# dhansmair/flamingo-mini

Measured on AMD Instinct MI355X. Metric: images/sec (fwd+bwd) flamingo-mini bs=32, higher is better.
Workload: dtype bf16

## Files before the change

flamingo-mini_amd/csrc/ff_api.hip:

```cpp
#include <stdarg.h>
#include <stdio.h>
#include <math.h>
#include <stdlib.h>
#include "ff_common.h"
#include "ff_internal.h"

namespace ff {

static thread_local char g_err[512] = "";
void set_error(const char* fmt, ...) {
    va_list ap;
    va_start(ap, fmt);
    vsnprintf(g_err, sizeof(g_err), fmt, ap);
    va_end(ap);
}
#ifdef FF_DEBUG
int dbg_switch(const char* name, int dflt) {
    const char* e = getenv(name);
    return e ? atoi(e) : dflt;
}
#endif
int check_launch(const char* what) {
    hipError_t e = hipGetLastError();
    if (e != hipSuccess) {
        set_error("%s: launch failed: %s", what, hipGetErrorString(e));
        return FF_ERR_LAUNCH;
    }
    return FF_OK;
}


static LnArgs ln_args(int dtype, int rows, int cols, RowMap x, RowMap y, RowMap dx) {
    LnArgs a;
    a.dtype = dtype; a.rows = rows; a.cols = cols;
    a.x_map = x; a.y_map = y; a.dx_map = dx;
    a.add_rows_per_seg = 0; a.add_div = 0; a.eps = 1e-5f; a.stats_given = 0;
    return a;
}

struct RsDims {
    int dt, Bn, T, v, D, F, q, H, dh, inner, ffi, R, depth, nte, act;
    int Mq, Mkv, Mf;
    size_t es, attn_ws;
    float scale;
    RowMap pD, pI, pF;
    RowMap lat_bcast;
    RowMap kv_media, kv_lat;
    explicit RsDims(const ff_resampler_desc& d) {
        dt = d.dtype; Bn = d.batch; T = d.n_frames; v = d.n_tokens; D = d.dim; F = T * v; q = d.num_latents;
        H = d.heads; dh = d.dim_head; inner = H * dh; ffi = d.ff_mult * D; R = F + q; depth = d.depth;
        nte = d.num_time_embeds; act = d.act; es = dtype_size(dt); scale = 1.0f / sqrtf((float)dh);
        Mq = Bn * q; Mkv = Bn * R; Mf = Bn * F; attn_ws = (size_t)Bn * H * q * 4;
        pD = plain_rows(D); pI = plain_rows(inner); pF = plain_rows(ffi);
        lat_bcast = RowMap{D, 0, q};
        kv_media = RowMap{D, (long long)R * D, F};
        kv_lat = RowMap{D, (long long)R * D, q};
    }
    LnArgs ln_latents() const { return ln_args(dt, Mq, D, pD, pD, pD); }
    LnArgs ln_media(RowMap y) const {
        LnArgs a = ln_args(dt, Mf, D, pD, y, pD);
        a.add_rows_per_seg = F; a.add_div = v;
        return a;
    }
    template <typename P> P* kv_latent_rows(P* kv) const { return (P*)((char*)kv + (size_t)F * D * es); }
};
struct RsLayerSaved {
    void *x_in, *kv_in, *Qs, *K, *V, *O, *x_mid, *xn_f, *Hpre, *Aact;
    float *mean_l, *rstd_l, *lse, *mean_f, *rstd_f;
};
constexpr int kMaxDepth = 64;
struct RsSaved {
    float *mean_m, *rstd_m, *mean_o, *rstd_o;
    void* x_last;
    RsLayerSaved L[kMaxDepth];
};
static void rs_take_layer_saved(const RsDims& s, Arena& a, RsLayerSaved& L) {
    const size_t rows_q = s.Mq, rows_kv = s.Mkv;
    L.mean_l = a.take<float>(rows_q * 4);
    L.rstd_l = a.take<float>(rows_q * 4);
    L.kv_in = a.take(rows_kv * s.D * s.es);
    L.Qs = a.take(rows_q * s.inner * s.es);
    L.K = a.take(rows_kv * s.inner * s.es);
    L.V = a.take(rows_kv * s.inner * s.es);
    L.lse = a.take<float>((size_t)s.Bn * s.H * s.q * 4);
    L.O = a.take(rows_q * s.inner * s.es);
    L.x_mid = a.take(rows_q * s.D * s.es);
    L.mean_f = a.take<float>(rows_q * 4);
    L.rstd_f = a.take<float>(rows_q * 4);
    L.xn_f = a.take(rows_q * s.D * s.es);
    L.Hpre = a.take(rows_q * s.ffi * s.es);
    L.Aact = a.take(rows_q * s.ffi * s.es);
}
static size_t rs_saved_layout(const RsDims& s, void* base, size_t cap, RsSaved& o) {
    Arena a(base, cap);
    const size_t rows_q = s.Mq;
    o.mean_m = a.take<float>((size_t)s.Mf * 4);
    o.rstd_m = a.take<float>((size_t)s.Mf * 4);
    for (int l = 0; l < s.depth; l++) {
        o.L[l].x_in = l == 0 ? nullptr : a.take(rows_q * s.D * s.es);
        rs_take_layer_saved(s, a, o.L[l]);
    }
    o.x_last = a.take(rows_q * s.D * s.es);
    o.mean_o = a.take<float>(rows_q * 4);
    o.rstd_o = a.take<float>(rows_q * 4);
    return align_up(a.used);
}

static size_t rs_ws_bytes(const RsDims& s) {
    size_t w = 0;
    auto g = [&](int M, int N, int K, int nz) { w = std::max(w, gemm_workspace_bytes(s.dt, M, N, K, nz, 0)); };
    g(s.Mq, s.inner, s.D, 1); g(s.Mkv, s.inner, s.D, 2); g(s.Mq, s.D, s.inner, 1); g(s.Mq, s.ffi, s.D, 1); g(s.Mq, s.D, s.ffi, 1);
    for (int nz = 1; nz <= 4; nz++) {
        g(s.D, s.ffi, s.Mq, nz); g(s.ffi, s.D, s.Mq, nz); g(s.D, s.inner, s.Mq, nz); g(s.inner, s.D, s.Mq, nz); g(s.inner, s.D, s.Mkv, nz);
    }
    g(s.Mkv, s.D, s.inner, 1);
    w = std::max(w, layernorm_bwd_workspace(s.Mf, s.D));
    w = std::max(w, layernorm_bwd_workspace(s.Mq, s.D));
    w = std::max(w, rows_reduce_workspace(s.Mq, s.D, s.q, 1));
    w = std::max(w, rows_reduce_workspace(s.Mf, s.D, s.F, s.v));
    return align_up(w) + align_up(s.attn_ws);
}
struct RsChain {
    void *ws, *dxn, *dO, *dkv, *dln;
    size_t ws_bytes, gws;
    float* attn_ws;
};
struct RsLayerGrads {
    void *dx_mid, *dH, *dQs, *dK, *dV;
};
static void rs_take_ws(const RsDims& s, Arena& a, RsChain& c) {
    c.ws_bytes = rs_ws_bytes(s);
    c.ws = a.take(c.ws_bytes);
    c.gws = c.ws_bytes - align_up(s.attn_ws);
    c.attn_ws = c.ws ? (float*)((char*)c.ws + c.gws) : nullptr;
}
static void rs_take_chain(const RsDims& s, Arena& a, RsChain& c) {
    c.dxn = a.take((size_t)s.Mq * s.D * s.es);
    c.dO = a.take((size_t)s.Mq * s.inner * s.es);
    c.dkv = a.take((size_t)s.Mkv * s.D * s.es);
    c.dln = a.take((size_t)s.Mq * s.D * s.es);
}
static void rs_take_layer_grads(const RsDims& s, Arena& a, RsLayerGrads& g) {
    g.dx_mid = a.take((size_t)s.Mq * s.D * s.es);
    g.dH = a.take((size_t)s.Mq * s.ffi * s.es);
    g.dQs = a.take((size_t)s.Mq * s.inner * s.es);
    g.dK = a.take((size_t)s.Mkv * s.inner * s.es);
    g.dV = a.take((size_t)s.Mkv * s.inner * s.es);
}
static void rs_take_ln_partials(const RsDims& s, Arena& a, bool deferrable, float** lnp) {
    for (int i = 0; i < 3; i++) lnp[i] = deferrable ? a.take<float>(layernorm_bwd_partial_bytes(i == 2 ? s.Mf : s.Mq, s.D)) : nullptr;
}

struct RsScratch {
    RsChain c;
    void *dx0, *dxf;
    void* dx_out[kMaxDepth];
    RsLayerGrads L[kMaxDepth];
    float* lnp[3 * kMaxDepth + 1];
};
static size_t rs_scratch_layout(const RsDims& s, void* base, size_t cap, bool bwd, RsScratch& o) {
    Arena a(base, cap);
    rs_take_ws(s, a, o.c);
    if (bwd) {
        o.dx0 = a.take((size_t)s.Mq * s.D * s.es);
        rs_take_chain(s, a, o.c);
        o.dxf = a.take((size_t)s.Mf * s.D * s.es);
        for (int l = 0; l < s.depth; l++) {
            o.dx_out[l] = a.take((size_t)s.Mq * s.D * s.es);
            rs_take_layer_grads(s, a, o.L[l]);
        }
        static const int defer_ln = dbg_switch("FF_DEFER_LN", 1);
        const bool lnd = defer_ln != 0 && layernorm_bwd_deferrable(s.dt, s.D);
        for (int l = 0; l < s.depth; l++) rs_take_ln_partials(s, a, lnd, o.lnp + 3 * l);
        o.lnp[3 * s.depth] = lnd ? a.take<float>(layernorm_bwd_partial_bytes(s.Mq, s.D)) : nullptr;
    }
    return align_up(a.used);
}

static int rs_check(const ff_resampler_desc* d) {
    FF_CHECK(d, FF_ERR_SHAPE, "resampler: null descriptor");
    FF_CHECK(d->dtype == FF_DTYPE_F32 || d->dtype == FF_DTYPE_BF16, FF_ERR_UNSUPPORTED, "resampler: dtype %d", d->dtype);
    FF_CHECK(d->batch > 0 && d->n_frames > 0 && d->n_tokens > 0 && d->dim > 0 && d->depth > 0 && d->depth <= kMaxDepth && d->heads > 0 &&
                 d->dim_head > 0 && d->num_latents > 0 && d->ff_mult > 0,
             FF_ERR_SHAPE, "resampler: bad dimensions");
    FF_CHECK(d->n_frames <= d->num_time_embeds, FF_ERR_SHAPE, "resampler: %d frames > num_time_embeds %d (perceiver_resampler.py:166)",
             d->n_frames, d->num_time_embeds);
    FF_CHECK(d->act >= FF_ACT_GELU && d->act <= FF_ACT_RELU, FF_ERR_SHAPE, "resampler: act %d", d->act);
    return FF_OK;
}

static ff_attn_desc rs_attn_desc(const RsDims& s) {
    ff_attn_desc a = {};
    a.dtype = s.dt; a.batch = s.Bn; a.heads = s.H; a.dim_head = s.dh; a.n_q = s.q; a.n_kv = s.R; a.mode = FF_ATTN_DENSE;
    const ff_strides sq = {(long long)s.q * s.inner, s.inner, s.dh}, sk = {(long long)s.R * s.inner, s.inner, s.dh};
    a.q = sq; a.o = sq; a.dq = sq; a.dout = sq;
    a.k = sk; a.v = sk; a.dk = sk; a.dv = sk;
    return a;
}

static int rs_media_stats(const RsDims& s, const void* x_f, const void* tpe, float* mean_m, float* rstd_m, hipStream_t st) {
    return layernorm_fwd(s.ln_media(s.pD), x_f, tpe, nullptr, nullptr, nullptr, mean_m, rstd_m, st);
}

static int rs_layer_forward(const RsDims& s, const void* const* p, const void* x_f, const void* tpe, float* mean_m, float* rstd_m, const void* x_in,
                            RowMap x_map, void* x_out, const RsLayerSaved& L, void* ws, size_t ws_bytes, hipStream_t st) {
    const RowMap pD = s.pD, pI = s.pI, pF = s.pF;
    void* kv_lat_base = s.kv_latent_rows(L.kv_in);
    {
        LnArgs a = s.ln_media(s.kv_media);
        a.stats_given = 1;
        FF_TRY(layernorm_fwd(a, x_f, tpe, p[0], p[1], L.kv_in, mean_m, rstd_m, st));
    }
    FF_TRY(layernorm_fwd(ln_args(s.dt, s.Mq, s.D, x_map, s.kv_lat, pD), x_in, nullptr, p[2], p[3], kv_lat_base, L.mean_l, L.rstd_l, st));
    FF_TRY(Gemm(s.dt, s.Mq, s.inner, s.D).a(0, s.kv_lat).b(0, pD).c(pI).scale(s.scale).problem(kv_lat_base, p[4], L.Qs).run(ws, ws_bytes, st));
    FF_TRY(Gemm(s.dt, s.Mkv, s.inner, s.D).a(0, pD).b(0, pD).c(pI).problem(L.kv_in, p[5], L.K).problem(L.kv_in, p[6], L.V).run(ws, ws_bytes, st));
    FF_TRY(attention_fwd(rs_attn_desc(s), L.Qs, L.K, L.V, nullptr, L.O, L.lse, st));
    FF_TRY(Gemm(s.dt, s.Mq, s.D, s.inner).a(0, pI).b(0, pI).c(pD).res_map(x_map).problem(L.O, p[7], L.x_mid, nullptr, nullptr, x_in).run(ws, ws_bytes, st));
    FF_TRY(layernorm_fwd(s.ln_latents(), L.x_mid, nullptr, p[8], p[9], L.xn_f, L.mean_f, L.rstd_f, st));
    FF_TRY(Gemm(s.dt, s.Mq, s.ffi, s.D).a(0, pD).b(0, pD).c(pF).act(s.act).problem(L.xn_f, p[10], L.Aact, L.Hpre).run(ws, ws_bytes, st));
    return Gemm(s.dt, s.Mq, s.D, s.ffi).a(0, pF).b(0, pF).c(pD).problem(L.Aact, p[11], x_out, nullptr, nullptr, L.x_mid).run(ws, ws_bytes, st);
}

static int rs_final_norm(const RsDims& s, const void* x_last, const void* gamma, const void* beta, void* out, float* mean, float* rstd, hipStream_t st) {
    return layernorm_fwd(s.ln_latents(), x_last, nullptr, gamma, beta, out, mean, rstd, st);
}

static int rs_ln_bwd(const RsChain& W, float* partial, LnPending* pending, const LnArgs& a, const void* dy, const void* x, const void* add,
                     const void* gamma, const float* mean, const float* rstd, void* dx, const void* dx_res, void* dg, void* db, hipStream_t st) {
    if (partial)
        return layernorm_bwd(a, dy, x, add, gamma, mean, rstd, dx, dx_res, dg, db, partial, layernorm_bwd_partial_bytes(a.rows, a.cols), st, nullptr, pending);
    return layernorm_bwd(a, dy, x, add, gamma, mean, rstd, dx, dx_res, dg, db, W.ws, W.gws, st);
}

static int rs_layer_backward(const RsDims& s, const void* const* p, void* const* g, const void* x_f, const void* tpe, const float* mean_m,
                             const float* rstd_m, const void* x_in, RowMap x_map, const RsLayerSaved& L, const void* dx_out, void* dx_in,
                             void* dx_f, const void* dx_f_res, const RsChain& W, const RsLayerGrads& T, float* const* lnp, LnPending* ln_sets,
                             hipStream_t st) {
    const RowMap pD = s.pD, pI = s.pI, pF = s.pF;
    FF_TRY(Gemm(s.dt, s.Mq, s.ffi, s.D).a(0, pD).b(1, pF).c(pF).act_bwd(s.act).problem(dx_out, p[11], T.dH, nullptr, L.Hpre).run(W.ws, W.gws, st));
    FF_TRY(Gemm(s.dt, s.Mq, s.D, s.ffi).a(0, pF).b(1, pD).c(pD).problem(T.dH, p[10], W.dxn).run(W.ws, W.gws, st));
    FF_TRY(rs_ln_bwd(W, lnp[0], &ln_sets[0], s.ln_latents(), W.dxn, L.x_mid, nullptr, p[8], L.mean_f, L.rstd_f, T.dx_mid, dx_out, g[8], g[9], st));
    FF_TRY(Gemm(s.dt, s.Mq, s.inner, s.D).a(0, pD).b(1, pI).c(pI).problem(T.dx_mid, p[7], W.dO).run(W.ws, W.gws, st));
    FF_TRY(attention_bwd(rs_attn_desc(s), L.Qs, L.K, L.V, nullptr, L.O, W.dO, L.lse, T.dQs, T.dK, T.dV, W.attn_ws, s.attn_ws, st));
    FF_TRY(Gemm(s.dt, s.Mkv, s.D, s.inner).a(0, pI).b(1, pD).c(pD).problem(T.dK, p[5], W.dkv).run(W.ws, W.gws, st));
    FF_TRY(Gemm(s.dt, s.Mkv, s.D, s.inner).a(0, pI).b(1, pD).c(pD).problem(T.dV, p[6], W.dkv, nullptr, nullptr, W.dkv).run(W.ws, W.gws, st));
    FF_TRY(Gemm(s.dt, s.Mq, s.D, s.inner).a(0, pI).b(1, pD).c(pD).res_map(s.kv_lat).scale(s.scale)
               .problem(T.dQs, p[4], W.dln, nullptr, nullptr, s.kv_latent_rows(W.dkv)).run(W.ws, W.gws, st));
    FF_TRY(rs_ln_bwd(W, lnp[1], &ln_sets[1], ln_args(s.dt, s.Mq, s.D, x_map, pD, pD), W.dln, x_in, nullptr, p[2], L.mean_l, L.rstd_l, dx_in, T.dx_mid, g[2],
                     g[3], st));
    return rs_ln_bwd(W, lnp[2], &ln_sets[2], s.ln_media(s.kv_media), W.dkv, x_f, tpe, p[0], mean_m, rstd_m, dx_f, dx_f_res, g[0], g[1], st);
}

static int rs_input_grads(const RsDims& s, const void* dx0, const void* dxf, void* d_latents, void* d_tpe, void* ws, size_t ws_bytes, hipStream_t st) {
    FF_TRY(rows_reduce(s.dt, s.Mq, s.D, s.pD, s.q, 1, dx0, d_latents, ws, ws_bytes, st));
    if (s.nte > s.T) FF_TRY(zero_bytes((char*)d_tpe + (size_t)s.T * s.D * s.es, (size_t)(s.nte - s.T) * s.D * s.es, st));
    return rows_reduce(s.dt, s.Mf, s.D, s.pD, s.F, s.v, dxf, d_tpe, ws, ws_bytes, st);
}

static int resampler_fwd(const ff_resampler_desc* d, const void* x_f, const void* const* P, void* out, void* saved, size_t saved_bytes,
                         void* scratch, size_t scratch_bytes, hipStream_t st) {
    FF_TRY(rs_check(d));
    FF_CHECK(x_f && P && out && saved && scratch, FF_ERR_SHAPE, "resampler_fwd: null argument");
    const RsDims s(*d);
    RsSaved S;
    RsScratch W;
    FF_CHECK(rs_saved_layout(s, saved, saved_bytes, S) <= saved_bytes, FF_ERR_WORKSPACE, "resampler_fwd: saved buffer too small");
    FF_CHECK(rs_scratch_layout(s, scratch, scratch_bytes, false, W) <= scratch_bytes, FF_ERR_WORKSPACE, "resampler_fwd: scratch too small");
    const void *latents = P[0], *tpe = P[1];
    FF_TRY(rs_media_stats(s, x_f, tpe, S.mean_m, S.rstd_m, st));
    for (int l = 0; l < s.depth; l++) {
        const void* const* p = P + FF_RESAMPLER_GLOBAL_PARAMS + FF_RESAMPLER_LAYER_PARAMS * l;
        void* x_next = l + 1 < s.depth ? S.L[l + 1].x_in : S.x_last;
        FF_TRY(rs_layer_forward(s, p, x_f, tpe, S.mean_m, S.rstd_m, l == 0 ? latents : S.L[l].x_in, l == 0 ? s.lat_bcast : s.pD, x_next, S.L[l], W.c.ws,
                                W.c.ws_bytes, st));
    }
    return rs_final_norm(s, S.x_last, P[2], P[3], out, S.mean_o, S.rstd_o, st);
}

static int resampler_bwd(const ff_resampler_desc* d, const void* x_f, const void* const* P, const void* dout, const void* saved,
                         size_t saved_bytes, void* const* G, void* dx_f, void* scratch, size_t scratch_bytes, hipStream_t st) {
    FF_TRY(rs_check(d));
    FF_CHECK(x_f && P && dout && saved && G && scratch, FF_ERR_SHAPE, "resampler_bwd: null argument");
    const RsDims s(*d);
    RsSaved S;
    RsScratch W;
    FF_CHECK(rs_saved_layout(s, (void*)saved, saved_bytes, S) <= saved_bytes, FF_ERR_WORKSPACE, "resampler_bwd: saved buffer too small");
    FF_CHECK(rs_scratch_layout(s, scratch, scratch_bytes, true, W) <= scratch_bytes, FF_ERR_WORKSPACE, "resampler_bwd: scratch too small");
    const RowMap pD = s.pD, pI = s.pI, pF = s.pF;
    const void *latents = P[0], *tpe = P[1];
    void* dxf = dx_f ? dx_f : W.dxf;
    void* const ws = W.c.ws;
    const size_t gws = W.c.gws;

    LnPending ln_sets[3 * kMaxDepth + 1];
    FF_TRY(rs_ln_bwd(W.c, W.lnp[3 * s.depth], &ln_sets[3 * s.depth], s.ln_latents(), dout, S.x_last, nullptr, P[2], S.mean_o, S.rstd_o,
                     W.dx_out[s.depth - 1], nullptr, G[2], G[3], st));
    for (int l = s.depth - 1; l >= 0; l--) {
        const void* const* p = P + FF_RESAMPLER_GLOBAL_PARAMS + FF_RESAMPLER_LAYER_PARAMS * l;
        void* const* g = G + FF_RESAMPLER_GLOBAL_PARAMS + FF_RESAMPLER_LAYER_PARAMS * l;
        void* dx_below = l == 0 ? W.dx0 : W.dx_out[l - 1];
        FF_TRY(rs_layer_backward(s, p, g, x_f, tpe, S.mean_m, S.rstd_m, l == 0 ? latents : S.L[l].x_in, l == 0 ? s.lat_bcast : pD, S.L[l], W.dx_out[l],
                                 dx_below, dxf, l == s.depth - 1 ? nullptr : dxf, W.c, W.L[l], W.lnp + 3 * l, ln_sets + 3 * l, st));
    }
    FF_TRY(layernorm_bwd_finish(s.dt, ln_sets, 3 * s.depth + 1, st));
    constexpr int kRsGroup = 4;
    for (int l0 = 0; l0 < s.depth; l0 += kRsGroup) {
        const int l1 = std::min(s.depth, l0 + kRsGroup);
        Gemm g3(s.dt, s.D, s.ffi, s.Mq), g1(s.dt, s.ffi, s.D, s.Mq), go(s.dt, s.D, s.inner, s.Mq), gq(s.dt, s.inner, s.D, s.Mq);
        g3.a(1, pD).b(1, pF).c(pF);
        g1.a(1, pF).b(1, pD).c(pD);
        go.a(1, pD).b(1, pI).c(pI);
        gq.a(1, pI).b(1, s.kv_lat).c(pD).scale(s.scale);
        for (int l = l0; l < l1; l++) {
            void* const* g = G + FF_RESAMPLER_GLOBAL_PARAMS + FF_RESAMPLER_LAYER_PARAMS * l;
            const RsLayerSaved& L = S.L[l];
            const RsLayerGrads& T = W.L[l];
            g3.problem(W.dx_out[l], L.Aact, g[11]);
            g1.problem(T.dH, L.xn_f, g[10]);
            go.problem(T.dx_mid, L.O, g[7]);
            gq.problem(T.dQs, s.kv_latent_rows(L.kv_in), g[4]);
        }
        FF_TRY(g3.run(ws, gws, st));
        FF_TRY(g1.run(ws, gws, st));
        FF_TRY(go.run(ws, gws, st));
        FF_TRY(gq.run(ws, gws, st));
    }
    {
        Gemm gkv(s.dt, s.inner, s.D, s.Mkv);
        gkv.a(1, pI).b(1, pD).c(pD);
        for (int l = 0; l < s.depth; l++) {
            void* const* g = G + FF_RESAMPLER_GLOBAL_PARAMS + FF_RESAMPLER_LAYER_PARAMS * l;
            gkv.problem(W.L[l].dK, S.L[l].kv_in, g[5]);
            gkv.problem(W.L[l].dV, S.L[l].kv_in, g[6]);
            if (gkv.P.nz == kRsGroup || l == s.depth - 1) {
                FF_TRY(gkv.run(ws, gws, st));
                gkv.P.nz = 0;
            }
        }
    }
    return rs_input_grads(s, W.dx0, dxf, G[0], G[1], ws, gws, st);
}

struct RsProSaved { float *mean_m, *rstd_m; };
static size_t rs_pro_layout(const RsDims& s, void* base, size_t cap, RsProSaved& o) {
    Arena a(base, cap);
    o.mean_m = a.take<float>((size_t)s.Mf * 4);
    o.rstd_m = a.take<float>((size_t)s.Mf * 4);
    return align_up(a.used);
}
static size_t rs_layer_saved_layout(const RsDims& s, void* base, size_t cap, RsLayerSaved& L) {
    Arena a(base, cap);
    L.x_in = nullptr;
    rs_take_layer_saved(s, a, L);
    return align_up(a.used);
}
struct RsLayerScratch {
    RsChain c;
    RsLayerGrads g;
    float* lnp[3];
};
static size_t rs_layer_scratch_layout(const RsDims& s, void* base, size_t cap, RsLayerScratch& o) {
    Arena a(base, cap);
    rs_take_ws(s, a, o.c);
    rs_take_chain(s, a, o.c);
    rs_take_layer_grads(s, a, o.g);
    rs_take_ln_partials(s, a, layernorm_bwd_deferrable(s.dt, s.D), o.lnp);
    return align_up(a.used);
}

static int rs_prologue_fwd(const ff_resampler_desc* d, const void* x_f, const void* tpe, void* pro, size_t pro_bytes, hipStream_t st) {
    FF_TRY(rs_check(d));
    FF_CHECK(x_f && tpe && pro, FF_ERR_SHAPE, "resampler_prologue_fwd: null argument");
    const RsDims s(*d);
    RsProSaved S;
    FF_CHECK(rs_pro_layout(s, pro, pro_bytes, S) <= pro_bytes, FF_ERR_WORKSPACE, "resampler_prologue_fwd: saved buffer too small");
    return rs_media_stats(s, x_f, tpe, S.mean_m, S.rstd_m, st);
}

static int rs_layer_fwd(const ff_resampler_desc* d, const void* x_f, const void* tpe, const void* pro, size_t pro_bytes, const void* x_in,
                        int x_is_latents, const void* const* p, void* x_out, void* saved, size_t saved_bytes, void* scratch, size_t scratch_bytes,
                        hipStream_t st) {
    FF_TRY(rs_check(d));
    FF_CHECK(x_f && tpe && pro && x_in && p && x_out && saved && scratch, FF_ERR_SHAPE, "resampler_layer_fwd: null argument");
    const RsDims s(*d);
    RsProSaved Pr;
    RsLayerSaved L;
    RsLayerScratch W;
    FF_CHECK(rs_pro_layout(s, (void*)pro, pro_bytes, Pr) <= pro_bytes, FF_ERR_WORKSPACE, "resampler_layer_fwd: prologue buffer too small");
    FF_CHECK(rs_layer_saved_layout(s, saved, saved_bytes, L) <= saved_bytes, FF_ERR_WORKSPACE, "resampler_layer_fwd: saved buffer too small");
    FF_CHECK(rs_layer_scratch_layout(s, scratch, scratch_bytes, W) <= scratch_bytes, FF_ERR_WORKSPACE, "resampler_layer_fwd: scratch too small");
    return rs_layer_forward(s, p, x_f, tpe, Pr.mean_m, Pr.rstd_m, x_in, x_is_latents ? s.lat_bcast : s.pD, x_out, L, W.c.ws, W.c.ws_bytes, st);
}

static int rs_layer_bwd(const ff_resampler_desc* d, const void* x_f, const void* tpe, const void* pro, size_t pro_bytes, const void* x_in,
                        int x_is_latents, const void* const* p, const void* dx_out, const void* saved, size_t saved_bytes, void* const* g,
                        void* dx_in, void* dx_f, int dx_f_accumulate, void* scratch, size_t scratch_bytes, hipStream_t st) {
    FF_TRY(rs_check(d));
    FF_CHECK(x_f && tpe && pro && x_in && p && dx_out && saved && g && dx_in && dx_f && scratch, FF_ERR_SHAPE, "resampler_layer_bwd: null argument");
    const RsDims s(*d);
    RsProSaved Pr;
    RsLayerSaved L;
    RsLayerScratch W;
    FF_CHECK(rs_pro_layout(s, (void*)pro, pro_bytes, Pr) <= pro_bytes, FF_ERR_WORKSPACE, "resampler_layer_bwd: prologue buffer too small");
    FF_CHECK(rs_layer_saved_layout(s, (void*)saved, saved_bytes, L) <= saved_bytes, FF_ERR_WORKSPACE, "resampler_layer_bwd: saved buffer too small");
    FF_CHECK(rs_layer_scratch_layout(s, scratch, scratch_bytes, W) <= scratch_bytes, FF_ERR_WORKSPACE, "resampler_layer_bwd: scratch too small");
    const RowMap pD = s.pD, pI = s.pI, pF = s.pF;
    void* const ws = W.c.ws;
    const size_t gws = W.c.gws;
    LnPending ln_sets[3];
    FF_TRY(rs_layer_backward(s, p, g, x_f, tpe, Pr.mean_m, Pr.rstd_m, x_in, x_is_latents ? s.lat_bcast : pD, L, dx_out, dx_in, dx_f,
                             dx_f_accumulate ? dx_f : nullptr, W.c, W.g, W.lnp, ln_sets, st));
    FF_TRY(layernorm_bwd_finish(s.dt, ln_sets, 3, st));
    FF_TRY(Gemm(s.dt, s.D, s.ffi, s.Mq).a(1, pD).b(1, pF).c(pF).problem(dx_out, L.Aact, g[11]).run(ws, gws, st));
    FF_TRY(Gemm(s.dt, s.ffi, s.D, s.Mq).a(1, pF).b(1, pD).c(pD).problem(W.g.dH, L.xn_f, g[10]).run(ws, gws, st));
    FF_TRY(Gemm(s.dt, s.D, s.inner, s.Mq).a(1, pD).b(1, pI).c(pI).problem(W.g.dx_mid, L.O, g[7]).run(ws, gws, st));
    FF_TRY(Gemm(s.dt, s.inner, s.D, s.Mq).a(1, pI).b(1, s.kv_lat).c(pD).scale(s.scale).problem(W.g.dQs, s.kv_latent_rows(L.kv_in), g[4]).run(ws, gws, st));
    return Gemm(s.dt, s.inner, s.D, s.Mkv).a(1, pI).b(1, pD).c(pD).problem(W.g.dK, L.kv_in, g[5]).problem(W.g.dV, L.kv_in, g[6]).run(ws, gws, st);
}

static int rs_prologue_bwd(const ff_resampler_desc* d, const void* dx0, const void* dx_f, void* d_latents, void* d_tpe, void* scratch,
                           size_t scratch_bytes, hipStream_t st) {
    FF_TRY(rs_check(d));
    FF_CHECK(dx0 && dx_f && d_latents && d_tpe && scratch, FF_ERR_SHAPE, "resampler_prologue_bwd: null argument");
    const RsDims s(*d);
    RsLayerScratch W;
    FF_CHECK(rs_layer_scratch_layout(s, scratch, scratch_bytes, W) <= scratch_bytes, FF_ERR_WORKSPACE, "resampler_prologue_bwd: scratch too small");
    return rs_input_grads(s, dx0, dx_f, d_latents, d_tpe, W.c.ws, W.c.ws_bytes, st);
}

static int rs_epilogue_fwd(const ff_resampler_desc* d, const void* x_last, const void* gamma, const void* beta, void* out, void* epi, size_t epi_bytes,
                           hipStream_t st) {
    FF_TRY(rs_check(d));
    FF_CHECK(x_last && gamma && beta && out && epi, FF_ERR_SHAPE, "resampler_epilogue_fwd: null argument");
    const RsDims s(*d);
    const size_t rows_q = s.Mq;
    FF_CHECK(epi_bytes >= 2 * align_up(rows_q * 4), FF_ERR_WORKSPACE, "resampler_epilogue_fwd: saved buffer too small");
    return rs_final_norm(s, x_last, gamma, beta, out, (float*)epi, (float*)((char*)epi + align_up(rows_q * 4)), st);
}
static int rs_epilogue_bwd(const ff_resampler_desc* d, const void* dout, const void* x_last, const void* gamma, const void* epi, size_t epi_bytes,
                           void* dx_last, void* dgamma, void* dbeta, void* scratch, size_t scratch_bytes, hipStream_t st) {
    FF_TRY(rs_check(d));
    FF_CHECK(dout && x_last && gamma && epi && dx_last && dgamma && dbeta && scratch, FF_ERR_SHAPE, "resampler_epilogue_bwd: null argument");
    const RsDims s(*d);
    const size_t rows_q = s.Mq;
    FF_CHECK(epi_bytes >= 2 * align_up(rows_q * 4), FF_ERR_WORKSPACE, "resampler_epilogue_bwd: saved buffer too small");
    RsLayerScratch W;
    FF_CHECK(rs_layer_scratch_layout(s, scratch, scratch_bytes, W) <= scratch_bytes, FF_ERR_WORKSPACE, "resampler_epilogue_bwd: scratch too small");
    const float* mean = (const float*)epi;
    const float* rstd = (const float*)((const char*)epi + align_up(rows_q * 4));
    return layernorm_bwd(s.ln_latents(), dout, x_last, nullptr, gamma, mean, rstd, dx_last, nullptr, dgamma, dbeta, W.c.ws, W.c.ws_bytes, st);
}

struct XaDims {
    int dt, b, L, d, dv, Nm, nv, Nk, H, dh, inner, ffi, act;
    size_t es;
    float scale;
    bool ext_kv;
    explicit XaDims(const ff_xattn_desc& x) {
        ext_kv = x.cached_k.sr != 0;
        dt = x.dtype; b = x.batch; L = x.n_tokens; d = x.dim; dv = x.dim_visual; Nm = x.n_media; nv = x.n_visual; Nk = Nm * nv;
        H = x.heads; dh = x.dim_head; inner = H * dh; ffi = x.ff_mult * d; act = x.act; es = dtype_size(dt);
        scale = 1.0f / sqrtf((float)dh);
    }
};
struct XaSaved {
    float *mean_a, *rstd_a, *lse, *mean_f, *rstd_f;
    void *yn, *Qs, *KV, *O, *attn_out, *y1, *xn_f, *Hpre, *Aact, *ffw_out;
    size_t kv_offset;
};
static size_t xa_saved_layout(const XaDims& s, void* base, size_t cap, XaSaved& o) {
    Arena a(base, cap);
    const size_t M = (size_t)s.b * s.L;
    o.KV = s.ext_kv ? nullptr : a.take((size_t)s.b * s.Nk * 2 * s.inner * s.es);
    o.kv_offset = 0;
    o.mean_a = a.take<float>(M * 4);
    o.rstd_a = a.take<float>(M * 4);
    o.yn = a.take(M * s.d * s.es);
    o.Qs = a.take(M * s.inner * s.es);
    o.lse = a.take<float>((size_t)s.b * s.H * s.L * 4);
    o.O = a.take(M * s.inner * s.es);
    o.attn_out = a.take(M * s.d * s.es);
    o.y1 = a.take(M * s.d * s.es);
    o.mean_f = a.take<float>(M * 4);
    o.rstd_f = a.take<float>(M * 4);
    o.xn_f = a.take(M * s.d * s.es);
    o.Hpre = a.take(M * s.ffi * s.es);
    o.Aact = a.take(M * s.ffi * s.es);
    o.ffw_out = a.take(M * s.d * s.es);
    return align_up(a.used);
}
struct XaScratch {
    void *dy1, *dH, *dxn, *dO, *dQs, *dKV, *dyn, *ws;
    size_t ws_bytes;
    float* lnx;
};
struct XaStash {
    void *dy1, *dH, *dQs;
    float *lnp_f = nullptr, *lnp_a = nullptr;
};
static bool xa_ln_deferrable(const XaDims& s) {
    static const int on = dbg_switch("FF_DEFER_LN", 1);
    return on != 0 && layernorm_bwd_deferrable(s.dt, s.d);
}
static size_t xa_stash_layout(const XaDims& s, void* base, size_t cap, XaStash& o) {
    Arena a(base, cap);
    const size_t M = (size_t)s.b * s.L;
    o.dy1 = a.take(M * s.d * s.es);
    o.dH = a.take(M * s.ffi * s.es);
    o.dQs = a.take(M * s.inner * s.es);
    if (xa_ln_deferrable(s)) {
        o.lnp_f = a.take<float>(layernorm_bwd_partial_bytes((int)M, s.d));
        o.lnp_a = a.take<float>(layernorm_bwd_partial_bytes((int)M, s.d));
    }
    return align_up(a.used);
}
static size_t xa_ws_bytes(const XaDims& s) {
    const int M = s.b * s.L, Mk = s.b * s.Nk;
    size_t w = 0;
    auto g = [&](int m, int n, int k) { w = std::max(w, gemm_workspace_bytes(s.dt, m, n, k, 1, 0)); };
    g(M, s.inner, s.d); g(Mk, 2 * s.inner, s.dv); g(M, s.d, s.inner); g(M, s.ffi, s.d); g(M, s.d, s.ffi);
    g(s.d, s.ffi, M); g(s.ffi, s.d, M); g(s.d, s.inner, M); g(s.inner, s.d, M); g(2 * s.inner, s.dv, Mk); g(Mk, s.dv, 2 * s.inner);
    w = std::max(w, layernorm_bwd_workspace(M, s.d));
    w = std::max(w, gate_grad_workspace(M, s.d));
    if (decode_ffw_supported(s.dt, M, s.d, s.ffi)) w = std::max(w, decode_ffw_workspace_bytes(s.d, s.ffi));
    return align_up(w) + align_up((size_t)s.b * s.H * s.L * 4);
}
static size_t xa_scratch_layout(const XaDims& s, void* base, size_t cap, bool bwd, XaScratch& o) {
    Arena a(base, cap);
    const size_t M = (size_t)s.b * s.L;
    o.ws_bytes = xa_ws_bytes(s);
    o.ws = a.take(o.ws_bytes);
    o.lnx = a.take<float>(xa_ln3_part_bytes(s.b, s.H));
    if (bwd) {
        o.dy1 = a.take(M * s.d * s.es);
        o.dH = a.take(M * s.ffi * s.es);
        o.dxn = a.take(M * s.d * s.es);
        o.dO = a.take(M * s.inner * s.es);
        o.dQs = a.take(M * s.inner * s.es);
        o.dKV = s.ext_kv ? nullptr : a.take((size_t)s.b * s.Nk * 2 * s.inner * s.es);
        o.dyn = a.take(M * s.d * s.es);
    }
    return align_up(a.used);
}
static int xa_check(const ff_xattn_desc* d) {
    FF_CHECK(d, FF_ERR_SHAPE, "xattn: null descriptor");
    FF_CHECK(d->dtype == FF_DTYPE_F32 || d->dtype == FF_DTYPE_BF16, FF_ERR_UNSUPPORTED, "xattn: dtype %d", d->dtype);
    FF_CHECK(d->batch > 0 && d->n_tokens > 0 && d->dim > 0 && d->dim_visual > 0 && d->n_media > 0 && d->n_visual > 0 && d->heads > 0 &&
                 d->dim_head > 0 && d->ff_mult > 0,
             FF_ERR_SHAPE, "xattn: bad dimensions");
    FF_CHECK(d->act >= FF_ACT_GELU && d->act <= FF_ACT_RELU, FF_ERR_SHAPE, "xattn: act %d", d->act);
    return FF_OK;
}
static ff_attn_desc xa_attn_desc(const ff_xattn_desc& x, const XaDims& s, bool cached) {
    ff_attn_desc a = {};
    a.dtype = s.dt; a.batch = s.b; a.heads = s.H; a.dim_head = s.dh; a.n_q = s.L; a.n_kv = s.Nk;
    a.mode = FF_ATTN_MEDIA; a.n_visual = s.nv; a.tt_stride = x.tt_stride; a.tt_offset = x.tt_offset;
    const ff_strides sq = {(long long)s.L * s.inner, s.inner, s.dh};
    const ff_strides sk = {(long long)s.Nk * 2 * s.inner, 2LL * s.inner, s.dh};
    a.q = sq; a.o = sq; a.dq = sq; a.dout = sq;
    a.k = cached ? x.cached_k : sk;
    a.v = cached ? x.cached_v : sk;
    a.dk = sk; a.dv = sk;
    return a;
}

static bool xa_fused_enabled() {
    static const int v = dbg_switch("FF_XATTN_FUSED", 1);
    return v != 0;
}
static bool xa_ln3_enabled() {
    static const int v = dbg_switch("FF_XATTN_LN3", 1);
    return v != 0;
}
static XaFusedArgs xa_fused_args(const ff_xattn_desc& x, const XaDims& s, bool ext_kv) {
    XaFusedArgs a = {};
    a.batch = s.b; a.heads = s.H; a.n_q = s.L; a.n_kv = s.Nk; a.n_visual = s.nv; a.tt_stride = x.tt_stride; a.tt_offset = x.tt_offset;
    a.dim = s.d; a.inner = s.inner; a.scale = s.scale; a.eps = 1e-5f;
    static const int xcd_split = dbg_switch("FF_XATTN_XCD_SPLIT", 0);
    a.xcd_split = xcd_split;
    const ff_strides sk = {(long long)s.Nk * 2 * s.inner, 2LL * s.inner, s.dh};
    a.k = ext_kv ? x.cached_k : sk;
    a.v = ext_kv ? x.cached_v : sk;
    a.dk = sk; a.dv = sk;
    return a;
}

static bool xa_ln3_in_bwd(const ff_xattn_desc& x, const XaDims& s) {
    if (!xa_ln3_enabled() || !xa_fused_enabled() || !xa_fused_supported(s.dt, s.dh, s.d, s.inner) || x.sync == nullptr) return false;
    const XaFusedArgs fa = xa_fused_args(x, s, s.ext_kv);
    const int M = s.b * s.L;
    return xa_out_fusable(fa, s.dt, s.dh) && s.b <= layernorm_bwd_partial_blocks(M) && (size_t)s.b * (2 * (size_t)s.d + 2) * sizeof(float) <= layernorm_bwd_workspace(M, s.d);
}
static int xattn_fwd(const ff_xattn_desc* d, const void* y, const void* vf, const int* tt, const void* const* P, const void* ck,
                     const void* cv, void* y_out, void* saved, size_t saved_bytes, void* scratch, size_t scratch_bytes, hipStream_t st) {
    FF_TRY(xa_check(d));
    const bool cached = ck != nullptr;
    FF_CHECK(y && tt && P && y_out && saved && scratch && (cached ? cv != nullptr : vf != nullptr), FF_ERR_SHAPE, "xattn_fwd: null argument");
    const XaDims s(*d);
    FF_CHECK(s.ext_kv == cached, FF_ERR_SHAPE, "xattn_fwd: external K / V need their strides in the descriptor (cached_k / cached_v) and vice versa");
    XaSaved S;
    XaScratch W;
    FF_CHECK(xa_saved_layout(s, saved, saved_bytes, S) <= saved_bytes, FF_ERR_WORKSPACE, "xattn_fwd: saved buffer too small");
    FF_CHECK(xa_scratch_layout(s, scratch, scratch_bytes, false, W) <= scratch_bytes, FF_ERR_WORKSPACE, "xattn_fwd: scratch too small");
    const int M = s.b * s.L, Mk = s.b * s.Nk;
    const RowMap pd = plain_rows(s.d), pI = plain_rows(s.inner), pF = plain_rows(s.ffi), pV = plain_rows(s.dv), pKV = plain_rows(2 * s.inner);
    const void *Kp, *Vp;
    if (!cached) {
        FF_TRY(Gemm(s.dt, Mk, 2 * s.inner, s.dv).a(0, pV).b(0, pV).c(pKV).problem(vf, P[5], S.KV).run(W.ws, W.ws_bytes, st));
        Kp = S.KV;
        Vp = (const char*)S.KV + (size_t)s.inner * s.es;
    } else {
        Kp = ck; Vp = cv;
    }
    bool out_fused = false, ln_fused = false;
    if (xa_fused_enabled() && xa_fused_supported(s.dt, s.dh, s.d, s.inner)) {
        const XaFusedArgs fa = xa_fused_args(*d, s, cached);
        XaOutArgs oa = {(const bf16*)P[6], (const bf16*)P[0], (bf16*)S.y1, (bf16*)S.attn_out, (unsigned*)d->sync};
        out_fused = d->sync != nullptr && xa_out_fusable(fa, s.dt, s.dh) && !decode_ffw_supported(s.dt, M, s.d, s.ffi);
        if (out_fused && xa_ln3_enabled()) {
            oa.ln_g = (const bf16*)P[7]; oa.ln_b = (const bf16*)P[8]; oa.ln_out = (bf16*)S.xn_f; oa.ln_mean = S.mean_f; oa.ln_rstd = S.rstd_f;
            oa.ln_part = W.lnx;
            ln_fused = true;
        }
        FF_TRY(xa_qattn_fwd(fa, s.dt, s.dh, y, P[2], P[3], P[4], Kp, Vp, tt, S.yn, S.Qs, S.O, S.mean_a, S.rstd_a, S.lse, st, out_fused ? &oa : nullptr));
    } else {
        FF_TRY(layernorm_fwd(ln_args(s.dt, M, s.d, pd, pd, pd), y, nullptr, P[2], P[3], S.yn, S.mean_a, S.rstd_a, st));
        FF_TRY(Gemm(s.dt, M, s.inner, s.d).a(0, pd).b(0, pd).c(pI).scale(s.scale).problem(S.yn, P[4], S.Qs).run(W.ws, W.ws_bytes, st));
        FF_TRY(attention_fwd(xa_attn_desc(*d, s, cached), S.Qs, Kp, Vp, tt, S.O, S.lse, st));
    }
    if (!out_fused) FF_TRY(Gemm(s.dt, M, s.d, s.inner).a(0, pI).b(0, pI).c(pd).problem(S.O, P[6], S.y1, S.attn_out, nullptr, y, P[0]).run(W.ws, W.ws_bytes, st));
    if (decode_ffw_supported(s.dt, M, s.d, s.ffi))
        return decode_ffw(M, s.d, s.ffi, s.act, 1e-5f, S.y1, P[7], P[8], P[9], P[10], P[1], S.xn_f, S.mean_f, S.rstd_f, S.Hpre, S.Aact, S.ffw_out, y_out,
                          W.ws, W.ws_bytes, st);
    if (!ln_fused) FF_TRY(layernorm_fwd(ln_args(s.dt, M, s.d, pd, pd, pd), S.y1, nullptr, P[7], P[8], S.xn_f, S.mean_f, S.rstd_f, st));
    FF_TRY(Gemm(s.dt, M, s.ffi, s.d).a(0, pd).b(0, pd).c(pF).act(s.act).problem(S.xn_f, P[9], S.Aact, S.Hpre).run(W.ws, W.ws_bytes, st));
    return Gemm(s.dt, M, s.d, s.ffi).a(0, pF).b(0, pF).c(pd).problem(S.Aact, P[10], y_out, S.ffw_out, nullptr, S.y1, P[1]).run(W.ws, W.ws_bytes, st);
}

static int xattn_bwd(const ff_xattn_desc* d, const void* y, const void* vf, const int* tt, const void* const* P, const void* dy2,
                     const void* saved, size_t saved_bytes, void* const* G, void* dy, void* dvf, void* scratch, size_t scratch_bytes,
                     hipStream_t st, const void* ext_k = nullptr, const void* ext_v = nullptr, void* dkv_out = nullptr,
                     void* stash = nullptr, size_t stash_bytes = 0) {
    FF_TRY(xa_check(d));
    const bool hoisted = ext_k != nullptr;
    FF_CHECK(y && tt && P && dy2 && saved && G && dy && scratch && (hoisted ? (ext_v && dkv_out) : vf != nullptr), FF_ERR_SHAPE,
             "xattn_bwd: null argument");
    const XaDims s(*d);
    FF_CHECK(s.ext_kv == hoisted, FF_ERR_SHAPE, "xattn_bwd: external K / V need their strides in the descriptor (cached_k / cached_v) and vice versa");
    XaSaved S;
    XaScratch W;
    FF_CHECK(xa_saved_layout(s, (void*)saved, saved_bytes, S) <= saved_bytes, FF_ERR_WORKSPACE, "xattn_bwd: saved buffer too small");
    FF_CHECK(xa_scratch_layout(s, scratch, scratch_bytes, true, W) <= scratch_bytes, FF_ERR_WORKSPACE, "xattn_bwd: scratch too small");
    XaStash T{W.dy1, W.dH, W.dQs};
    const bool defer = stash != nullptr;
    if (defer) FF_CHECK(xa_stash_layout(s, stash, stash_bytes, T) <= stash_bytes, FF_ERR_WORKSPACE, "xattn_bwd: stash too small");
    const bool defer_ln = defer && xa_ln_deferrable(s);
    if (defer_ln)
        FF_CHECK(((uintptr_t)y | (uintptr_t)dy | (uintptr_t)dy2 | (uintptr_t)P[2] | (uintptr_t)P[7]) % 16 == 0, FF_ERR_SHAPE,
                 "xattn_bwd (deferred weight gradients): y, d y_out, d y and the LayerNorm weights must be 16-byte aligned");
    LnPending pend_f, pend_a;
    const int M = s.b * s.L, Mk = s.b * s.Nk;
    const RowMap pd = plain_rows(s.d), pI = plain_rows(s.inner), pF = plain_rows(s.ffi), pV = plain_rows(s.dv), pKV = plain_rows(2 * s.inner);
    const size_t attn_ws_bytes = align_up((size_t)s.b * s.H * s.L * 4);
    const size_t gws = W.ws_bytes - attn_ws_bytes;
    float* attn_ws = (float*)((char*)W.ws + gws);

    if (!defer) FF_TRY(Gemm(s.dt, s.d, s.ffi, M).a(1, pd).b(1, pF).c(pF).problem(dy2, S.Aact, G[10], nullptr, nullptr, nullptr, P[1]).run(W.ws, gws, st));
    FF_TRY(Gemm(s.dt, M, s.ffi, s.d).a(0, pd).b(1, pF).c(pF).act_bwd(s.act).problem(dy2, P[10], T.dH, nullptr, S.Hpre, nullptr, P[1]).run(W.ws, gws, st));
    if (!defer) FF_TRY(Gemm(s.dt, s.ffi, s.d, M).a(1, pF).b(1, pd).c(pd).problem(T.dH, S.xn_f, G[9]).run(W.ws, gws, st));
// ... 339 lines not shown
```

flamingo-mini_amd/csrc/ff_gemm.hip:

```cpp
#include <atomic>
#include <type_traits>
#include "ff_common.h"
#include <stdlib.h>
#include "ff_internal.h"
#include "ff_gemm_tiles.h"

namespace ff {

template <typename T>
FF_DEV void epilogue4(const GemmParams& P, const GemmProblem& pr, int m, int n, float (&v)[4]) {
    typedef __attribute__((ext_vector_type(4))) T vec4;
    const long long off = P.c_map.off(m) + n;
    const bool full = (n + 3 < P.N);
#pragma unroll
    for (int r = 0; r < 4; r++) v[r] *= P.scale;
    auto load4 = [&](const void* base, long long at, float (&o)[4]) {
        const T* p = (const T*)base + at;
        if (full) {
            vec4 t = *(const vec4*)p;
#pragma unroll
            for (int r = 0; r < 4; r++) o[r] = to_f32(t[r]);
        } else {
#pragma unroll
            for (int r = 0; r < 4; r++) o[r] = (n + r < P.N) ? to_f32(p[r]) : 0.f;
// ... 55 lines not shown
                for (int e = 0; e < VN; e++) { o[e] = a[e]; o[e + 4] = b[e]; }
            }
        } else {
#pragma unroll
            for (int e = 0; e < 8; e++) o[e] = e < nv ? to_f32(p[e]) : 0.f;
        }
    };
    auto store8 = [&](void* base, long long at, const float (&o)[8]) {
        T* p = (T*)base + at;
        if (vec) {
            if constexpr (VN == 8) Vec<T>::store(p, o);
            else {
                float a[VN], b[VN];
#pragma unroll
                for (int e = 0; e < VN; e++) { a[e] = o[e]; b[e] = o[e + 4]; }
                Vec<T>::store(p, a); Vec<T>::store(p + VN, b);
            }
        } else {
#pragma unroll
            for (int e = 0; e < 8; e++)
                if (e < nv) p[e] = from_f32<T>(o[e]);
        }
    };
#pragma unroll
    for (int e = 0; e < 8; e++) v[e] *= P.scale;
    const long long off = P.c_map.off(m) + n;
    if (has_aux) store8(pr.aux_out, off, v);
    if (has_gate) {
#pragma unroll
        for (int e = 0; e < 8; e++) v[e] *= gate;
    }
    if (has_act) {
#pragma unroll
        for (int e = 0; e < 8; e++) v[e] = act_fwd_t<T>(v[e], P.act);
    }
    if (has_act_bwd) {
        float h[8];
        load8(pr.aux_in, off, h);
#pragma unroll
        for (int e = 0; e < 8; e++) v[e] *= act_grad_t<T>(h[e], P.act_bwd);
    }
    if (has_res) {
        float q[8];
        load8(pr.residual, P.r_map.off(m) + n, q);
#pragma unroll
        for (int e = 0; e < 8; e++) v[e] += q[e];
    }
    store8(pr.C, off, v);
}

template <int BN> struct CtSwz { static constexpr int kMask = (BN / 4) % 16 == 0 ? 15 : 7; };
template <int BM, int BN, int NTHR = 256>
FF_DEV void tile_epilogue_bf16(const GemmParams& P, const GemmProblem& pr, const float* ct, int m_base, int n_base) {
    constexpr int TPR = BN / 8, RPP = NTHR / TPR;
    const int t = threadIdx.x, tr = t / TPR, col = (t % TPR) * 8, n = n_base + col;
    if (t >= TPR * RPP || n >= P.N) return;
    const int nv = min(8, P.N - n);
    const bool vec = P.c_vec8 && nv == 8;
    const float gate = pr.gate ? tanhf(to_f32(*(const bf16*)pr.gate)) : 1.f;
    auto rows = [&](auto feat) {
        constexpr int F = decltype(feat)::value;
        constexpr int UNROLL = (F < 0 || (F & (kEpiAct | kEpiActBwd))) ? 2 : 4;
        const int nrows = min(BM, P.M - m_base);
#pragma unroll UNROLL
        for (int r = tr; r < nrows; r += RPP) {
            const int m = m_base + r;
            const int ch = col >> 2, sw = r & CtSwz<BN>::kMask;
            const f32x4 lo = *(const f32x4*)(ct + r * BN + ((ch ^ sw) << 2)), hi = *(const f32x4*)(ct + r * BN + (((ch + 1) ^ sw) << 2));
            float v[8] = {lo[0], lo[1], lo[2], lo[3], hi[0], hi[1], hi[2], hi[3]};
            epilogue8<bf16, F>(P, pr, m, n, nv, vec, gate, v);
        }
    };
    const int feat = (pr.aux_out ? kEpiAux : 0) | (pr.gate ? kEpiGate : 0) | (P.act >= 0 ? kEpiAct : 0) | (P.act_bwd >= 0 ? kEpiActBwd : 0) |
                     (pr.residual ? kEpiRes : 0);
    if (feat == 0) rows(std::integral_constant<int, 0>());
    else if (feat == kEpiRes) rows(std::integral_constant<int, kEpiRes>());
    else if (feat == (kEpiRes | kEpiGate)) rows(std::integral_constant<int, kEpiRes | kEpiGate>());
    else if (feat == (kEpiAux | kEpiAct)) rows(std::integral_constant<int, kEpiAux | kEpiAct>());
    else if (feat == kEpiActBwd) rows(std::integral_constant<int, kEpiActBwd>());
    else if (feat == (kEpiActBwd | kEpiGate)) rows(std::integral_constant<int, kEpiActBwd | kEpiGate>());
    else rows(std::integral_constant<int, -1>());
}

#define FF_PIN(x) asm volatile("" : "+s"(x))
#define FF_GEMM_ARGS(Q, pr, P)                                                                                                        \
    GemmParams Q;                                                                                                                     \
    Q.M = P.M; Q.N = P.N; Q.K = P.K; Q.split_k = P.split_k; Q.k_per_split = P.k_per_split; Q.nz = P.nz;                              \
    Q.xcd_ms = P.xcd_ms; Q.xcd_ns = P.xcd_ns; Q.a_map = P.a_map; Q.b_map = P.b_map; Q.c_map = P.c_map; Q.r_map = P.r_map;             \
    Q.scale = P.scale; Q.act = P.act; Q.act_bwd = P.act_bwd; Q.c_vec8 = P.c_vec8; Q.partial = P.partial;                              \
    GemmProblem pr = P.p[0];                                                                                                          \
    FF_PIN(Q.M); FF_PIN(Q.N); FF_PIN(Q.K); FF_PIN(Q.split_k); FF_PIN(Q.k_per_split); FF_PIN(Q.nz); FF_PIN(Q.xcd_ms); FF_PIN(Q.xcd_ns); \
    FF_PIN(Q.a_map.ld); FF_PIN(Q.a_map.seg_stride); FF_PIN(Q.a_map.rows_per_seg);                                                     \
    FF_PIN(Q.b_map.ld); FF_PIN(Q.b_map.seg_stride); FF_PIN(Q.b_map.rows_per_seg);                                                     \
    FF_PIN(Q.c_map.ld); FF_PIN(Q.c_map.seg_stride); FF_PIN(Q.c_map.rows_per_seg);                                                     \
    FF_PIN(Q.r_map.ld); FF_PIN(Q.r_map.seg_stride); FF_PIN(Q.r_map.rows_per_seg);                                                     \
    FF_PIN(Q.scale); FF_PIN(Q.act); FF_PIN(Q.act_bwd); FF_PIN(Q.c_vec8); FF_PIN(Q.partial);                                           \
    FF_PIN(pr.A); FF_PIN(pr.B); FF_PIN(pr.C); FF_PIN(pr.aux_out); FF_PIN(pr.aux_in); FF_PIN(pr.residual); FF_PIN(pr.gate)


struct TileCoord {
    int z, split, tm, tn;
};
FF_DEV int fast_div(int a, int b) {
    int q = (int)(__fdividef((float)a, (float)b));
    if (q * b > a) q--;
    else if ((q + 1) * b <= a) q++;
    return q;
}
FF_DEV TileCoord tile_coord(int nz, int split_k, int ms, int ns, int tiles_m, int tiles_n) {
    const int per_z = tiles_m * tiles_n;
    int bid = xcd_remap(blockIdx.x, per_z * split_k * nz);
    TileCoord c;
    c.z = 0; c.split = 0;
    if (nz > 1) { c.z = fast_div(bid, per_z * split_k); bid -= c.z * per_z * split_k; }
    if (split_k > 1) { c.split = fast_div(bid, per_z); bid -= c.split * per_z; }
    int p = bid;
    const int lm = __builtin_ctz(ms), ln = __builtin_ctz(ns);
    c.tm = 0; c.tn = 0;
    for (int sgrid = 0; sgrid < ms * ns; sgrid++) {
        const int sm = sgrid >> ln, sn = sgrid & (ns - 1);
        const int r0 = (sm * tiles_m) >> lm, r1 = ((sm + 1) * tiles_m) >> lm;
        const int c0 = (sn * tiles_n) >> ln, c1 = ((sn + 1) * tiles_n) >> ln;
        const int cw = c1 - c0, cnt = (r1 - r0) * cw;
        if (p < cnt) {
            const int q = fast_div(p, cw);
            c.tm = r0 + q;
            c.tn = c0 + p - q * cw;
            break;
        }
        p -= cnt;
    }
    return c;
}

#ifdef FF_GEMM_TIMELINE
__device__ unsigned long long g_timeline[16384 * 8];
#define FF_TL(i) do { if (threadIdx.x == 0 && blockIdx.x < 16384) g_timeline[blockIdx.x * 8 + (i)] = __builtin_amdgcn_s_memrealtime(); } while (0)
#else
#define FF_TL(i) do { } while (0)
#endif


template <int BM, int BN, int AL, int BL, int NS>
__global__ __launch_bounds__(256) void gemm_bf16_dma_kernel(const void* hA, const void* hB, int hM, int hN, int hK, int h_split, int h_kps,
                                                            int h_nz, int h_xcd, int h_ald, int h_bld, int h_seg, const GemmParams P) {
    extern __shared__ __attribute__((aligned(16))) unsigned char smem_raw[];
    bf16* smem = (bf16*)smem_raw;
    FF_TL(0);
    constexpr int A_ELEMS = BM * kBK, B_ELEMS = BN * kBK, STAGE = A_ELEMS + B_ELEMS;
    constexpr int WM = BM / 2, WN = BN / 2, MT = WM / 16, NT = WN / 16;
    constexpr int PER_TILE = BM / 32 + BN / 32;
    static_assert(PER_TILE * (NS - 1) <= 63, "vmcnt overflow");

    RowMap a_map{h_ald, 0, 0}, b_map{h_bld, 0, 0};
    if (h_seg) { a_map = P.a_map; b_map = P.b_map; }
    const void* opA = hA;
    const void* opB = hB;
    const int tiles_m = (hM + BM - 1) / BM, tiles_n = (hN + BN - 1) / BN;
    const TileCoord tc = tile_coord(h_nz, h_split, h_xcd & 255, h_xcd >> 8, tiles_m, tiles_n);
    if (tc.z > 0) { opA = P.p[tc.z].A; opB = P.p[tc.z].B; }
    const int m_base = tc.tm * BM, n_base = tc.tn * BN;
    const int k_begin = tc.split * h_kps;
    const int k_end = min(hK, k_begin + h_kps);
    const int t = threadIdx.x, l = t & 63;
    const int w = __builtin_amdgcn_readfirstlane(t >> 6);
    const int wm = w >> 1, wn = w & 1;
    const __amdgpu_buffer_rsrc_t ra = __builtin_amdgcn_make_buffer_rsrc((void*)opA, 0, 0x7fffffff, 0x00020000);
    const __amdgpu_buffer_rsrc_t rb = __builtin_amdgcn_make_buffer_rsrc((void*)opB, 0, 0x7fffffff, 0x00020000);

    f32x4 acc[MT][NT];
#pragma unroll
    for (int i = 0; i < MT; i++)
#pragma unroll
        for (int j = 0; j < NT; j++) acc[i][j] = f32x4{0.f, 0.f, 0.f, 0.f};

    const int nk = (k_end - k_begin + kBK - 1) / kBK;
    unsigned va[BM / 32], vb[BN / 32];
    dma_prepare<BM, AL>(a_map, m_base, hM, w, l, va);
    dma_prepare<BN, BL>(b_map, n_base, hN, w, l, vb);
    const bool a_plain = AL == 0 || a_map.rows_per_seg <= 0, b_plain = BL == 0 || b_map.rows_per_seg <= 0;
    const unsigned a_step = AL == 0 ? 2u : (unsigned)a_map.ld * 2u, b_step = BL == 0 ? 2u : (unsigned)b_map.ld * 2u;
    auto issue = [&](int tile) {
        bf16* st = smem + (tile % NS) * STAGE;
        const int k0 = k_begin + tile * kBK;
        const bool full = k0 + kBK <= k_end;
        if (full && a_plain) dma_tile_fast<BM, AL>(ra, st, va, (unsigned)k0 * a_step, w);
        else dma_tile<BM, AL>(ra, st, a_map, m_base, hM, k0, k_end, w, l);
        if (full && b_plain) dma_tile_fast<BN, BL>(rb, st + A_ELEMS, vb, (unsigned)k0 * b_step, w);
        else dma_tile<BN, BL>(rb, st + A_ELEMS, b_map, n_base, hN, k0, k_end, w, l);
    };
    FF_TL(1);
#pragma unroll
    for (int s = 0; s < NS - 1; s++)
        if (s < nk) issue(s);
    FF_GEMM_ARGS(Q, pr, P);
    if (tc.z > 0) pr = P.p[tc.z];

    for (int kt = 0; kt < nk; kt++) {
        const int younger = min(nk - 1 - kt, NS - 2);
        if (NS >= 4 && younger == 2) wait_vmcnt<2 * PER_TILE>();
        else if (NS >= 3 && younger >= 1) wait_vmcnt<PER_TILE>();
        else wait_vmcnt<0>();
        __builtin_amdgcn_s_barrier();
#ifdef FF_GEMM_TIMELINE
        if (kt == 0) FF_TL(2);
#endif
        if (kt + NS - 1 < nk) issue(kt + NS - 1);
        const bf16* sA = smem + (kt % NS) * STAGE;
        const bf16* sB = sA + A_ELEMS;
#pragma unroll
        for (int ks = 0; ks < kBK / 32; ks++) {
            bf16x8 fa[MT], fb[NT];
#pragma unroll
            for (int i = 0; i < MT; i++) fa[i] = frag_read2<BM, AL>(sA, wm * WM + i * 16, ks);
#pragma unroll
            for (int j = 0; j < NT; j++) fb[j] = frag_read2<BN, BL>(sB, wn * WN + j * 16, ks);
#pragma unroll
            for (int i = 0; i < MT; i++)
#pragma unroll
                for (int j = 0; j < NT; j++) acc[i][j] = mfma_bf16(fb[j], fa[i], acc[i][j]);
        }
    }

    FF_TL(3);
    const int c = l & 15, g = l >> 4;
    if (Q.split_k > 1) {
#pragma unroll
        for (int i = 0; i < MT; i++) {
            const int m = m_base + wm * WM + i * 16 + c;
            if (m >= Q.M) continue;
#pragma unroll
            for (int j = 0; j < NT; j++) {
                const int n = n_base + wn * WN + j * 16 + g * 4;
                if (n >= Q.N) continue;
                *(f32x4*)(Q.partial + ((long long)(tc.z * Q.split_k + tc.split) * Q.M + m) * Q.N + n) = acc[i][j];
            }
        }
        return;
    }
    static_assert(BM * BN * 4 <= NS * STAGE * 2, "fp32 tile must fit the operand ring");
    __syncthreads();
    float* ct = (float*)smem_raw;
#pragma unroll
    for (int i = 0; i < MT; i++) {
        const int ml = wm * WM + i * 16 + c;
#pragma unroll
        for (int j = 0; j < NT; j++) {
            const int ch = ((wn * WN + j * 16) >> 2) + g;
            *(f32x4*)(ct + ml * BN + ((ch ^ (c & CtSwz<BN>::kMask)) << 2)) = acc[i][j];
        }
    }
    __syncthreads();
    FF_TL(4);
    tile_epilogue_bf16<BM, BN>(Q, pr, ct, m_base, n_base);
    FF_TL(5);
}

template <int BN, int BL, int NW = 4> struct BStage {
    static constexpr bool SPLIT = BN == 160 && (BL == 1 || NW == 8);
    static constexpr int N128 = 128 / (NW * 8);
    static constexpr int PER_WAVE = SPLIT ? N128 + 1 : BN / (NW * 8);
    static FF_DEV void prepare(const RowMap& map, int n_base, int n_lim, int w, int l, unsigned* v) {
        if constexpr (SPLIT) {
            dma_prepare<128, BL, NW>(map, n_base, n_lim, w, l, v);
            dma_prepare<32, BL, 4>(map, n_base + 128, n_lim, w & 3, l, v + N128);
            if (NW == 8 && w >= 4) v[N128] = kOobOffset;
        } else dma_prepare<BN, BL, NW>(map, n_base, n_lim, w, l, v);
    }
    static FF_DEV void fast(__amdgpu_buffer_rsrc_t r, bf16* st, const unsigned* v, unsigned soff, int w, bf16* dummy = nullptr) {
        if constexpr (SPLIT) {
            dma_tile_fast<128, BL, NW>(r, st, v, soff, w);
            if (NW == 8 && w >= 4) dma_tile_fast<32, BL, 4>(r, dummy, v + N128, soff, 0);
            else dma_tile_fast<32, BL, 4>(r, st + 128 * kBK, v + N128, soff, w & 3);
        } else dma_tile_fast<BN, BL, NW>(r, st, v, soff, w);
    }
    static FF_DEV void slow(__amdgpu_buffer_rsrc_t r, bf16* st, const RowMap& map, int n_base, int n_lim, int k0, int k_end, int w, int l, bf16* dummy = nullptr) {
        if constexpr (SPLIT) {
            dma_tile<128, BL, NW>(r, st, map, n_base, n_lim, k0, k_end, w, l);
            if (NW == 8 && w >= 4) dma_tile<32, BL, 4>(r, dummy, map, n_base + 128, 0, k0, k_end, 0, l);
            else dma_tile<32, BL, 4>(r, st + 128 * kBK, map, n_base + 128, n_lim, k0, k_end, w & 3, l);
        } else dma_tile<BN, BL, NW>(r, st, map, n_base, n_lim, k0, k_end, w, l);
    }
    static FF_DEV bf16x8 frag(const bf16* s, int col0, int ks) {
        if constexpr (SPLIT && BL == 1) return col0 < 128 ? frag_read2<128, 1>(s, col0, ks) : frag_read2<32, 1>(s + 128 * kBK, col0 - 128, ks);
        else return frag_read2<BN, BL>(s, col0, ks);
    }
};

template <int BM, int BN, int AL, int BL, int NS, int WPC, int NPW = 4, int NCW = 4>
__global__ __launch_bounds__((NCW + NPW) * 64, WPC * (NCW + NPW) / 4) void gemm_bf16_pc_kernel(const void* hA, const void* hB, int hM, int hN, int hK, int h_split, int h_kps,
                                                           int h_nz, int h_xcd, int h_ald, int h_bld, int h_seg, const GemmParams P) {
    extern __shared__ __attribute__((aligned(16))) unsigned char smem_raw[];
    bf16* smem = (bf16*)smem_raw;
    constexpr int A_ELEMS = BM * kBK, B_ELEMS = BN * kBK, STAGE = A_ELEMS + B_ELEMS;
    constexpr int CM = NCW / 2;
    constexpr int WM = BM / CM, WN = BN / 2, MT = WM / 16, NT = WN / 16;
    static_assert((NCW == 4 || NCW == 8) && WM % 16 == 0, "consumer layout");
    typedef BStage<BN, BL, NPW> BS;
    constexpr int PER_TILE = BM / (NPW * 8) + BS::PER_WAVE;
    static_assert(WN % 16 == 0 && BM % 32 == 0 && BN % 32 == 0, "tile shape");
    static_assert((AL == 0 || BM == 256 || BM == 128 || BM == 64) && (BL == 0 || BN == 128 || BN == 64 || BN == 160), "M-major staging exists for 64 / 128 / 256-wide A tiles and 64 / 128 / 160-wide B tiles only");
    static_assert(PER_TILE * (NS - 1) <= 63, "vmcnt overflow");

    RowMap a_map{h_ald, 0, 0}, b_map{h_bld, 0, 0};
    if (h_seg) { a_map = P.a_map; b_map = P.b_map; }
    const void* opA = hA;
    const void* opB = hB;
    const int tiles_m = (hM + BM - 1) / BM, tiles_n = (hN + BN - 1) / BN;
    const TileCoord tc = tile_coord(h_nz, h_split, h_xcd & 255, h_xcd >> 8, tiles_m, tiles_n);
    if (tc.z > 0) { opA = P.p[tc.z].A; opB = P.p[tc.z].B; }
    const int m_base = tc.tm * BM, n_base = tc.tn * BN;
    const int k_begin = tc.split * h_kps;
    const int k_end = min(hK, k_begin + h_kps);
    const int t = threadIdx.x, l = t & 63;
    const int w = __builtin_amdgcn_readfirstlane(t >> 6);
    const bool producer = w >= NCW;
    const int pw = producer ? w - NCW : w;
    const int wm = (w & (NCW - 1)) >> 1, wn = w & 1;
    bf16* dummy = smem + NS * STAGE + (pw & 3) * 512;
    const __amdgpu_buffer_rsrc_t ra = __builtin_amdgcn_make_buffer_rsrc((void*)opA, 0, 0x7fffffff, 0x00020000);
    const __amdgpu_buffer_rsrc_t rb = __builtin_amdgcn_make_buffer_rsrc((void*)opB, 0, 0x7fffffff, 0x00020000);
    const int nk = (k_end - k_begin + kBK - 1) / kBK;

    f32x4 acc[MT][NT];
#pragma unroll
    for (int i = 0; i < MT; i++)
#pragma unroll
        for (int j = 0; j < NT; j++) acc[i][j] = f32x4{0.f, 0.f, 0.f, 0.f};

    unsigned va[BM / (NPW * 8)], vb[BS::PER_WAVE];
    const bool a_plain = AL == 0 || a_map.rows_per_seg <= 0, b_plain = BL == 0 || b_map.rows_per_seg <= 0;
    const unsigned a_step = AL == 0 ? 2u : (unsigned)a_map.ld * 2u, b_step = BL == 0 ? 2u : (unsigned)b_map.ld * 2u;
    auto issue = [&](int tile) {
        bf16* st = smem + (tile % NS) * STAGE;
        const int k0 = k_begin + tile * kBK;
        const bool full = k0 + kBK <= k_end;
        if (full && a_plain) dma_tile_fast<BM, AL, NPW>(ra, st, va, (unsigned)k0 * a_step, pw);
        else dma_tile<BM, AL, NPW>(ra, st, a_map, m_base, hM, k0, k_end, pw, l);
        if (full && b_plain) BS::fast(rb, st + A_ELEMS, vb, (unsigned)k0 * b_step, pw, dummy);
        else BS::slow(rb, st + A_ELEMS, b_map, n_base, hN, k0, k_end, pw, l, dummy);
    };
    if (producer) {
        dma_prepare<BM, AL, NPW>(a_map, m_base, hM, pw, l, va);
        BS::prepare(b_map, n_base, hN, pw, l, vb);
#pragma unroll
        for (int s = 0; s < NS - 1; s++)
            if (s < nk) issue(s);
    }
    FF_GEMM_ARGS(Q, pr, P);
    if (tc.z > 0) pr = P.p[tc.z];
#ifdef FF_GEMM_PCMODE
    constexpr int pcmode = FF_GEMM_PCMODE;
#else
    constexpr int pcmode = 0;
#endif
    if (producer) {
        for (int kt = 0; kt < nk; kt++) {
            if (pcmode == 2) { __builtin_amdgcn_s_barrier(); continue; }
            const int younger = min(nk - 1 - kt, NS - 2);
            if (NS >= 4 && younger == 2) wait_vmcnt<2 * PER_TILE>();
            else if (NS >= 3 && younger >= 1) wait_vmcnt<PER_TILE>();
            else wait_vmcnt<0>();
            __builtin_amdgcn_s_barrier();
            if (kt + NS - 1 < nk) issue(kt + NS - 1);
        }
    } else {
        for (int kt = 0; kt < nk; kt++) {
            __builtin_amdgcn_s_barrier();
            if (pcmode == 1) continue;
            const bf16* sA = smem + (kt % NS) * STAGE;
            const bf16* sB = sA + A_ELEMS;
#pragma unroll
            for (int ks = 0; ks < kBK / 32; ks++) {
                bf16x8 fa[MT], fb[NT];
                if (pcmode != 4) {
#pragma unroll
                    for (int i = 0; i < MT; i++) fa[i] = frag_read2<BM, AL>(sA, wm * WM + i * 16, ks);
#pragma unroll
                    for (int j = 0; j < NT; j++) fb[j] = BS::frag(sB, wn * WN + j * 16, ks);
                } else {
                    const bf16x8 fixed = __builtin_bit_cast(bf16x8, f32x4{(float)l, 1.f, 2.f, (float)kt});
#pragma unroll
                    for (int i = 0; i < MT; i++) fa[i] = fixed;
#pragma unroll
                    for (int j = 0; j < NT; j++) fb[j] = fixed;
                }
                if (pcmode == 3) {
#pragma unroll
                    for (int i = 0; i < MT; i++) acc[i][0] += __builtin_bit_cast(f32x4, fa[i]);
#pragma unroll
                    for (int j = 0; j < NT; j++) acc[0][j] += __builtin_bit_cast(f32x4, fb[j]);
                    continue;
                }
#pragma unroll
                for (int i = 0; i < MT; i++)
#pragma unroll
                    for (int j = 0; j < NT; j++) acc[i][j] = mfma_bf16(fb[j], fa[i], acc[i][j]);
            }
        }
    }
    const int c = l & 15, g = l >> 4;
    if (Q.split_k > 1) {
        if (producer) return;
#pragma unroll
        for (int i = 0; i < MT; i++) {
            const int m = m_base + wm * WM + i * 16 + c;
            if (m >= Q.M) continue;
#pragma unroll
            for (int j = 0; j < NT; j++) {
                const int n = n_base + wn * WN + j * 16 + g * 4;
                if (n >= Q.N) continue;
                *(f32x4*)(Q.partial + ((long long)(tc.z * Q.split_k + tc.split) * Q.M + m) * Q.N + n) = acc[i][j];
            }
        }
        return;
    }
    static_assert(BM * BN * 4 <= NS * STAGE * 2, "fp32 tile must fit the operand ring");
    __syncthreads();
    float* ct = (float*)smem_raw;
    if (!producer) {
#pragma unroll
        for (int i = 0; i < MT; i++) {
            const int ml = wm * WM + i * 16 + c;
#pragma unroll
            for (int j = 0; j < NT; j++) {
                const int ch = ((wn * WN + j * 16) >> 2) + g;
                *(f32x4*)(ct + ml * BN + ((ch ^ (c & CtSwz<BN>::kMask)) << 2)) = acc[i][j];
            }
        }
    }
    __syncthreads();
    tile_epilogue_bf16<BM, BN, (NCW + NPW) * 64>(Q, pr, ct, m_base, n_base);
}

template <int AL, int BL>
__global__ __launch_bounds__(1024, 4) void gemm_bf16_u16_kernel(const void* hA, const void* hB, int hM, int hN, int hK, int h_split, int h_kps,
                                                                int h_nz, int h_xcd, int h_ald, int h_bld, int h_seg, const GemmParams P) {
    extern __shared__ __attribute__((aligned(16))) unsigned char smem_raw[];
    bf16* smem = (bf16*)smem_raw;
    constexpr int BM = 256, BN = 256, NW = 16;
    constexpr int UNIT = BM * kBK, NU = 5;
    static_assert(BM == BN, "the ring's units hold either operand");
    constexpr int WM = 64, WN = 64, MT = WM / 16, NT = WN / 16;
    constexpr int PA = BM / (NW * 8), PB = BN / (NW * 8);

    RowMap a_map{h_ald, 0, 0}, b_map{h_bld, 0, 0};
    if (h_seg) { a_map = P.a_map; b_map = P.b_map; }
    const void* opA = hA;
    const void* opB = hB;
    const int tiles_m = (hM + BM - 1) / BM, tiles_n = (hN + BN - 1) / BN;
    const TileCoord tc = tile_coord(h_nz, h_split, h_xcd & 255, h_xcd >> 8, tiles_m, tiles_n);
    if (tc.z > 0) { opA = P.p[tc.z].A; opB = P.p[tc.z].B; }
    const int m_base = tc.tm * BM, n_base = tc.tn * BN;
    const int k_begin = tc.split * h_kps;
    const int k_end = min(hK, k_begin + h_kps);
    const int t = threadIdx.x, l = t & 63;
    const int w = __builtin_amdgcn_readfirstlane(t >> 6);
    const int wm = w >> 2, wn = w & 3;
    const __amdgpu_buffer_rsrc_t ra = __builtin_amdgcn_make_buffer_rsrc((void*)opA, 0, 0x7fffffff, 0x00020000);
    const __amdgpu_buffer_rsrc_t rb = __builtin_amdgcn_make_buffer_rsrc((void*)opB, 0, 0x7fffffff, 0x00020000);

    f32x4 acc[MT][NT];
#pragma unroll
    for (int i = 0; i < MT; i++)
#pragma unroll
        for (int j = 0; j < NT; j++) acc[i][j] = f32x4{0.f, 0.f, 0.f, 0.f};

    const int nk = (k_end - k_begin + kBK - 1) / kBK;
    unsigned va[PA], vb[PB];
    dma_prepare<BM, AL, NW>(a_map, m_base, hM, w, l, va);
    dma_prepare<BN, BL, NW>(b_map, n_base, hN, w, l, vb);
    const bool a_plain = AL == 0 || a_map.rows_per_seg <= 0, b_plain = BL == 0 || b_map.rows_per_seg <= 0;
    const unsigned a_step = AL == 0 ? 2u : (unsigned)a_map.ld * 2u, b_step = BL == 0 ? 2u : (unsigned)b_map.ld * 2u;
    auto unit = [&](int kt, int op) { return smem + ((2 * kt + op) % NU) * UNIT; };
    auto issue_a = [&](int tile) {
        const int k0 = k_begin + tile * kBK;
        if (k0 + kBK <= k_end && a_plain) dma_tile_fast<BM, AL, NW>(ra, unit(tile, 0), va, (unsigned)k0 * a_step, w);
        else dma_tile<BM, AL, NW>(ra, unit(tile, 0), a_map, m_base, hM, k0, k_end, w, l);
    };
    auto issue_b = [&](int tile) {
        const int k0 = k_begin + tile * kBK;
        if (k0 + kBK <= k_end && b_plain) dma_tile_fast<BN, BL, NW>(rb, unit(tile, 1), vb, (unsigned)k0 * b_step, w);
        else dma_tile<BN, BL, NW>(rb, unit(tile, 1), b_map, n_base, hN, k0, k_end, w, l);
    };
    if (nk > 0) { issue_a(0); issue_b(0); }
    if (nk > 1) issue_a(1);
    FF_GEMM_ARGS(Q, pr, P);
    if (tc.z > 0) pr = P.p[tc.z];

    auto sync = [&](int kt) {
        if (kt + 1 < nk) wait_vmcnt<PA>();
        else wait_vmcnt<0>();
        __builtin_amdgcn_s_barrier();
        if (kt + 1 < nk) issue_b(kt + 1);
        if (kt + 2 < nk) issue_a(kt + 2);
    };
    bf16x8 fa[MT], fb[NT];
    auto read = [&](int kt, int ks) {
        const bf16* sA = unit(kt, 0);
        const bf16* sB = unit(kt, 1);
#pragma unroll
        for (int i = 0; i < MT; i++) fa[i] = frag_read2<BM, AL>(sA, wm * WM + i * 16, ks);
#pragma unroll
        for (int j = 0; j < NT; j++) fb[j] = frag_read2<BN, BL>(sB, wn * WN + j * 16, ks);
    };
    auto mma = [&]() {
#pragma unroll
        for (int i = 0; i < MT; i++)
#pragma unroll
            for (int j = 0; j < NT; j++) acc[i][j] = mfma_bf16(fb[j], fa[i], acc[i][j]);
    };
    for (int kt = 0; kt < nk; kt++) {
        sync(kt);
        read(kt, 0);
        mma();
        read(kt, 1);
        mma();
    }

    const int c = l & 15, g = l >> 4;
    if (Q.split_k > 1) {
#pragma unroll
        for (int i = 0; i < MT; i++) {
            const int m = m_base + wm * WM + i * 16 + c;
            if (m >= Q.M) continue;
#pragma unroll
            for (int j = 0; j < NT; j++) {
                const int n = n_base + wn * WN + j * 16 + g * 4;
                if (n >= Q.N) continue;
                *(f32x4*)(Q.partial + ((long long)(tc.z * Q.split_k + tc.split) * Q.M + m) * Q.N + n) = acc[i][j];
            }
        }
        return;
    }
    static_assert((BM / 2) * BN * 4 <= NU * UNIT * 2, "half of the fp32 tile must fit the operand ring");
    float* ct = (float*)smem_raw;
    __syncthreads();
#pragma unroll
    for (int half = 0; half < 2; half++) {
        if ((wm >> 1) == half) {
#pragma unroll
            for (int i = 0; i < MT; i++) {
                const int ml = (wm & 1) * WM + i * 16 + c;
#pragma unroll
                for (int j = 0; j < NT; j++) {
                    const int ch = ((wn * WN + j * 16) >> 2) + g;
                    *(f32x4*)(ct + ml * BN + ((ch ^ (c & CtSwz<BN>::kMask)) << 2)) = acc[i][j];
                }
            }
        }
        __syncthreads();
        tile_epilogue_bf16<BM / 2, BN, NW * 64>(Q, pr, ct, m_base + half * (BM / 2), n_base);
        if (half == 0) __syncthreads();
    }
}
template <int AL, int BL> static int launch_bf16_u16(const GemmParams& P, hipStream_t st) {
    constexpr size_t lds = (size_t)5 * 256 * kBK * sizeof(bf16);
    static bool attr_done[64] = {};
    int dev = 0;
    (void)hipGetDevice(&dev);
    if (dev < 0 || dev >= 64 || !attr_done[dev]) {
        hipError_t e = hipFuncSetAttribute((const void*)gemm_bf16_u16_kernel<AL, BL>, hipFuncAttributeMaxDynamicSharedMemorySize, (int)lds);
        FF_CHECK(e == hipSuccess, FF_ERR_LAUNCH, "hipFuncSetAttribute(gemm u16 lds=%zu): %s", lds, hipGetErrorString(e));
        if (dev >= 0 && dev < 64) attr_done[dev] = true;
    }
    const int grid = cdiv(P.M, 256) * cdiv(P.N, 256) * P.split_k * P.nz;
    const int seg = P.a_map.rows_per_seg > 0 || P.b_map.rows_per_seg > 0 || P.a_map.ld >= (1LL << 31) || P.b_map.ld >= (1LL << 31);
    gemm_bf16_u16_kernel<AL, BL><<<dim3(grid), dim3(1024), lds, st>>>(P.p[0].A, P.p[0].B, P.M, P.N, P.K, P.split_k, P.k_per_split, P.nz,
                                                                      P.xcd_ms | (P.xcd_ns << 8), (int)P.a_map.ld, (int)P.b_map.ld, seg, P);
    return check_launch("gemm_bf16_u16");
}

template <int NW>
__global__ __launch_bounds__(NW * 64) void gemm_bf16_rows32_kernel(const GemmParams P) {
    __shared__ f32x4 red[NW][2][64];
    const int t = threadIdx.x, l = t & 63, c = l & 15, g = l >> 4;
    const int w = __builtin_amdgcn_readfirstlane(t >> 6);
    const int n0 = blockIdx.x * 16;
    const GemmProblem& pr = P.p[0];
    const int steps = P.K / 32, spw = (steps + NW - 1) / NW;
    const int s_begin = w * spw, s_end = min(steps, s_begin + spw);
    const __amdgpu_buffer_rsrc_t ra = __builtin_amdgcn_make_buffer_rsrc((void*)pr.A, 0, 0x7fffffff, 0x00020000);
    const __amdgpu_buffer_rsrc_t rb = __builtin_amdgcn_make_buffer_rsrc((void*)pr.B, 0, 0x7fffffff, 0x00020000);
    const int gk = g * 8;
    const unsigned b_off = n0 + c < P.N ? (unsigned)(P.b_map.off(n0 + c) + gk) * 2u : kOobOffset;
    const unsigned a0_off = c < P.M ? (unsigned)(P.a_map.off(c) + gk) * 2u : kOobOffset;
    const unsigned a1_off = 16 + c < P.M ? (unsigned)(P.a_map.off(16 + c) + gk) * 2u : kOobOffset;
    constexpr int SB = 4;
    bf16x8 fb0[SB], fa00[SB], fa10[SB], fb1[SB], fa01[SB], fa11[SB];
    f32x4 acc0 = {0.f, 0.f, 0.f, 0.f}, acc1 = {0.f, 0.f, 0.f, 0.f};
    auto ld = [&](__amdgpu_buffer_rsrc_t r, unsigned off, unsigned soff, bool in) {
        return __builtin_bit_cast(bf16x8, __builtin_amdgcn_raw_buffer_load_b128(r, in ? off : kOobOffset, soff, 0));
    };
    auto load = [&](bf16x8* fb, bf16x8* fa0, bf16x8* fa1, int s0) {
#pragma unroll
        for (int i = 0; i < SB; i++) {
            const bool in = s0 + i < s_end;
            const int st = s0 + i;
            const unsigned soff = in ? (unsigned)st * 64u : 0u;
            fb[i] = ld(rb, b_off, soff, in);
            fa0[i] = ld(ra, a0_off, soff, in);
            fa1[i] = ld(ra, a1_off, soff, in);
        }
    };
    auto mma = [&](const bf16x8* fb, const bf16x8* fa0, const bf16x8* fa1, int s0) {
#pragma unroll
        for (int i = 0; i < SB; i++)
            if (s0 + i < s_end) {
                acc0 = mfma_bf16(fb[i], fa0[i], acc0);
                acc1 = mfma_bf16(fb[i], fa1[i], acc1);
            }
    };
    load(fb0, fa00, fa10, s_begin);
    for (int s0 = s_begin; s0 < s_end; s0 += 2 * SB) {
        load(fb1, fa01, fa11, s0 + SB);
        mma(fb0, fa00, fa10, s0);
        load(fb0, fa00, fa10, s0 + 2 * SB);
        mma(fb1, fa01, fa11, s0 + SB);
    }
    red[w][0][l] = acc0;
    red[w][1][l] = acc1;
    __syncthreads();
    if (t < 128) {
        const int i = t >> 6;
        f32x4 sum = red[0][i][l];
#pragma unroll
        for (int ww = 1; ww < NW; ww++) sum += red[ww][i][l];
        const int m = i * 16 + c, n = n0 + g * 4;
        if (m < P.M && n < P.N) {
            float v[4] = {sum[0], sum[1], sum[2], sum[3]};
            epilogue4<bf16>(P, pr, m, n, v);
        }
    }
}
static int launch_bf16_rows32(const GemmParams& P, hipStream_t st) {
    const int steps = P.K / 32, grid = cdiv(P.N, 16);
    if (steps <= 40) hipLaunchKernelGGL(gemm_bf16_rows32_kernel<4>, dim3(grid), dim3(256), 0, st, P);
    else if (steps <= 80) hipLaunchKernelGGL(gemm_bf16_rows32_kernel<8>, dim3(grid), dim3(512), 0, st, P);
    else hipLaunchKernelGGL(gemm_bf16_rows32_kernel<16>, dim3(grid), dim3(1024), 0, st, P);
    return check_launch("gemm_bf16_rows32");
}

constexpr int kFBM = 64, kFBK = 16, kFLd = 80;
// ... 4 lines not shown
    const int t = threadIdx.x;
    if (LAYOUT == 0) {
        const int row = row_base + (t >> 2), k = k0 + (t & 3) * 4;
        reg[0] = reg[1] = reg[2] = reg[3] = 0.f;
        if (row < row_lim) {
            const float* p = base + map.off(row) + k;
            if (vec_ok && k + 3 < k_end) {
                f32x4 v = *(const f32x4*)p;
                reg[0] = v[0]; reg[1] = v[1]; reg[2] = v[2]; reg[3] = v[3];
            } else {
#pragma unroll
                for (int j = 0; j < 4; j++)
                    if (k + j < k_end) reg[j] = p[j];
            }
        }
    } else {
        const int k = k0 + (t >> 4), row = row_base + (t & 15) * 4;
        reg[0] = reg[1] = reg[2] = reg[3] = 0.f;
        if (k < k_end) {
            const float* p = base + map.off(k) + row;
            if (vec_ok && row + 3 < row_lim) {
                f32x4 v = *(const f32x4*)p;
                reg[0] = v[0]; reg[1] = v[1]; reg[2] = v[2]; reg[3] = v[3];
            } else {
#pragma unroll
                for (int j = 0; j < 4; j++)
                    if (row + j < row_lim) reg[j] = p[j];
            }
        }
    }
}
template <int LAYOUT> FF_DEV void f32_tile_store(float* s, const float (&reg)[4]) {
    const int t = threadIdx.x;
    if (LAYOUT == 0) {
        const int row = t >> 2, k = (t & 3) * 4;
#pragma unroll
        for (int j = 0; j < 4; j++) s[(k + j) * kFLd + row] = reg[j];
    } else {
        const int k = t >> 4, row = (t & 15) * 4;
        *(f32x4*)(s + k * kFLd + row) = f32x4{reg[0], reg[1], reg[2], reg[3]};
    }
}

template <int AL, int BL> __global__ __launch_bounds__(256) void gemm_f32_kernel(const GemmParams P) {
    __shared__ __attribute__((aligned(16))) float sA[kFBK * kFLd];
    __shared__ __attribute__((aligned(16))) float sB[kFBK * kFLd];
    const int tiles_m = (P.M + kFBM - 1) / kFBM, tiles_n = (P.N + kFBM - 1) / kFBM;
    const TileCoord tc = tile_coord(P.nz, P.split_k, P.xcd_ms, P.xcd_ns, tiles_m, tiles_n);
    const GemmProblem& pr = P.p[tc.z];
    const int m_base = tc.tm * kFBM, n_base = tc.tn * kFBM;
    const int k_begin = tc.split * P.k_per_split;
    const int k_end = min(P.K, k_begin + P.k_per_split);
    const float* A = (const float*)pr.A;
    const float* B = (const float*)pr.B;
    const int t = threadIdx.x, w = t >> 6, l = t & 63, c = l & 15, g = l >> 4;
    const int wm = w >> 1, wn = w & 1;
    const bool a_vec = P.a_vec_ok, b_vec = P.b_vec_ok;

    f32x4 acc[2][2];
#pragma unroll
    for (int i = 0; i < 2; i++)
#pragma unroll
        for (int j = 0; j < 2; j++) acc[i][j] = f32x4{0.f, 0.f, 0.f, 0.f};

    for (int k0 = k_begin; k0 < k_end; k0 += kFBK) {
        float ra[4], rb[4];
        f32_tile_load<AL>(A, P.a_map, m_base, P.M, k0, k_end, a_vec, ra);
        f32_tile_load<BL>(B, P.b_map, n_base, P.N, k0, k_end, b_vec, rb);
        __syncthreads();
        f32_tile_store<AL>(sA, ra);
        f32_tile_store<BL>(sB, rb);
        __syncthreads();
#pragma unroll
        for (int ks = 0; ks < kFBK / 4; ks++) {
            float fa[2], fb[2];
#pragma unroll
            for (int i = 0; i < 2; i++) fa[i] = sA[(ks * 4 + g) * kFLd + wm * 32 + i * 16 + c];
#pragma unroll
            for (int j = 0; j < 2; j++) fb[j] = sB[(ks * 4 + g) * kFLd + wn * 32 + j * 16 + c];
#pragma unroll
            for (int i = 0; i < 2; i++)
#pragma unroll
                for (int j = 0; j < 2; j++) acc[i][j] = mfma_f32(fb[j], fa[i], acc[i][j]);
        }
    }
#pragma unroll
    for (int i = 0; i < 2; i++) {
        const int m = m_base + wm * 32 + i * 16 + c;
        if (m >= P.M) continue;
#pragma unroll
        for (int j = 0; j < 2; j++) {
            const int n = n_base + wn * 32 + j * 16 + g * 4;
            if (n >= P.N) continue;
            float v[4] = {acc[i][j][0], acc[i][j][1], acc[i][j][2], acc[i][j][3]};
            if (P.split_k > 1) {
                float* dst = P.partial + ((long long)(tc.z * P.split_k + tc.split) * P.M + m) * P.N + n;
#pragma unroll
                for (int r = 0; r < 4; r++)
                    if (n + r < P.N) dst[r] = v[r];
            } else {
                epilogue4<float>(P, pr, m, n, v);
            }
        }
    }
}

template <typename T> __global__ __launch_bounds__(256) void gemm_splitk_epilogue_kernel(const GemmParams P) {
    FF_GEMM_ARGS(Q, pr, P);
    const unsigned n8 = (unsigned)(Q.N + 7) / 8u;
    const unsigned idx = blockIdx.x * 256u + threadIdx.x;
    const unsigned row = idx / n8, nq = idx - row * n8;
    if (row >= (unsigned)(Q.nz * Q.M)) return;
    const int z = Q.nz > 1 ? (int)(row / (unsigned)Q.M) : 0, m = (int)row - z * Q.M, n = (int)nq * 8;
    if (z > 0) pr = P.p[z];
    const int nv = min(8, Q.N - n);
    float v[8] = {0.f, 0.f, 0.f, 0.f, 0.f, 0.f, 0.f, 0.f};
    const float* src = Q.partial + ((long long)z * Q.split_k * Q.M + m) * Q.N + n;
    const long long slab = (long long)Q.M * Q.N;
    int sp = 0;
    for (; sp + 3 < Q.split_k; sp += 4) {
        f32x4 lo[4], hi[4];
#pragma unroll
        for (int u = 0; u < 4; u++) {
            lo[u] = *(const f32x4*)(src + (sp + u) * slab);
            hi[u] = f32x4{0.f, 0.f, 0.f, 0.f};
            if (nv == 8) hi[u] = *(const f32x4*)(src + (sp + u) * slab + 4);
        }
#pragma unroll
        for (int u = 0; u < 4; u++)
#pragma unroll
            for (int e = 0; e < 4; e++) { v[e] += lo[u][e]; v[e + 4] += hi[u][e]; }
    }
    for (; sp + 1 < Q.split_k; sp += 2) {
        const f32x4 a0 = *(const f32x4*)(src + sp * slab), b0 = *(const f32x4*)(src + (sp + 1) * slab);
        f32x4 a1 = {0.f, 0.f, 0.f, 0.f}, b1 = a1;
        if (nv == 8) { a1 = *(const f32x4*)(src + sp * slab + 4); b1 = *(const f32x4*)(src + (sp + 1) * slab + 4); }
#pragma unroll
        for (int e = 0; e < 4; e++) { v[e] += a0[e]; v[e + 4] += a1[e]; }
#pragma unroll
        for (int e = 0; e < 4; e++) { v[e] += b0[e]; v[e + 4] += b1[e]; }
    }
    if (sp < Q.split_k) {
        const f32x4 a0 = *(const f32x4*)(src + sp * slab);
        f32x4 a1 = {0.f, 0.f, 0.f, 0.f};
        if (nv == 8) a1 = *(const f32x4*)(src + sp * slab + 4);
#pragma unroll
        for (int e = 0; e < 4; e++) { v[e] += a0[e]; v[e + 4] += a1[e]; }
    }
    const float gate = pr.gate ? tanhf(to_f32(*(const T*)pr.gate)) : 1.f;
    epilogue8<T>(Q, pr, m, n, nv, Q.c_vec8 && nv == 8, gate, v);
}

static int dispatch_f32(const GemmParams& P, hipStream_t st) {
    const int grid = cdiv(P.M, kFBM) * cdiv(P.N, kFBM) * P.split_k * P.nz;
#define FF_F32_LAUNCH(AL, BL) hipLaunchKernelGGL((gemm_f32_kernel<AL, BL>), dim3(grid), dim3(256), 0, st, P)
    if (P.a_layout == 0 && P.b_layout == 0) FF_F32_LAUNCH(0, 0);
    else if (P.a_layout == 0 && P.b_layout == 1) FF_F32_LAUNCH(0, 1);
    else if (P.a_layout == 1 && P.b_layout == 0) FF_F32_LAUNCH(1, 0);
    else FF_F32_LAUNCH(1, 1);
#undef FF_F32_LAUNCH
    return check_launch("gemm_f32");
}


namespace {
struct ProfState {
    std::atomic<bool> on{false};
    int cap = 0;
    std::atomic<int> n{0};
    hipEvent_t* ev = nullptr;
    ff_gemm_profile_record* rec = nullptr;
} g_prof;
}
int profile_begin(int dtype, int tile, int a_layout, int b_layout, int M, int N, int K, int nz, int split_k, hipStream_t st) {
    if (!g_prof.on.load(std::memory_order_relaxed)) return -1;
    const int i = g_prof.n.fetch_add(1);
    if (i >= g_prof.cap) return -1;
    ff_gemm_profile_record& r = g_prof.rec[i];
    r.dtype = dtype; r.tile = tile; r.a_layout = a_layout; r.b_layout = b_layout;
    r.M = M; r.N = N; r.K = K; r.nz = nz; r.split_k = split_k; r.ms = 0.f;
    hipEventRecord(g_prof.ev[2 * i], st);
    return i;
}
void profile_end(int i, hipStream_t st) {
    if (i >= 0) hipEventRecord(g_prof.ev[2 * i + 1], st);
}
static int prof_begin(const GemmParams& P, int dtype, int bm, hipStream_t st) {
    return profile_begin(dtype, bm, P.a_layout, P.b_layout, P.M, P.N, P.K, P.nz, P.split_k, st);
}
static void prof_end(int i, hipStream_t st) { profile_end(i, st); }

static int env_int(const char* name, int dflt) { return dbg_switch(name, dflt); }

struct TilePlan { int tile, split; };
static TilePlan plan_bf16(int M, int N, int K, int nz, int want_split, int a_layout = 0, int b_layout = 0, int ft = 0) {
    const long long t128 = (long long)cdiv(M, 128) * cdiv(N, 128) * nz, t64 = (long long)cdiv(M, 64) * cdiv(N, 64) * nz;
    TilePlan p;
    static const int env_tile = env_int("FF_GEMM_TILE", 0);
    if (ft == 0) ft = env_tile;
    static const int pc_bl1 = env_int("FF_GEMM_PC_BL1", 1);
    const bool pc_ok = a_layout == 0 && (b_layout == 0 || (pc_bl1 && N % 8 == 0));
    const bool skinny_ok = a_layout == 0 && b_layout == 0;
    const bool rows_ok = skinny_ok && M <= 32 && nz == 1 && K % 32 == 0;
    if (ft == 3216 && rows_ok) return TilePlan{3216, 1};
    if (ft == 128168) ft = 128160;
    const long long t256 = (long long)cdiv(M, 256) * cdiv(N, 128) * nz;
    if (ft == 128 || ft == 64 || ft == 64002 || ft == 6412 || ft == 128002 || (ft == 128160 && pc_ok) || (ft == 3264 && skinny_ok) || ft == 256128 || (ft == 256256 && skinny_ok)) {
        p.tile = ft;
        if (want_split > 0) { p.split = want_split; return p; }
        const long long t = ft == 128 || ft == 128002 ? t128 : ft == 64 || ft == 64002 ? t64 : ft == 128160 ? (long long)cdiv(M, 128) * cdiv(N, 160) * nz
                            : ft == 3264 ? (long long)cdiv(M, 32) * cdiv(N, 64) * nz : ft == 256128 ? t256 : ft == 256256 ? (long long)cdiv(M, 256) * cdiv(N, 256) * nz
                            : (long long)cdiv(M, 64) * cdiv(N, 128) * nz;
        p.split = (t >= 128 || K < 1024) ? 1 : std::max(1, std::min(std::min((int)(256 / t), K / 512), 16));
        return p;
    }
    static const int pc_on = env_int("FF_GEMM_PC", 1);
    static const int skinny_on = env_int("FF_GEMM_SKINNY", 1);
    static const int rows_on = env_int("FF_GEMM_ROWS32", 1);
    if (rows_on && rows_ok && K <= 1024 && want_split <= 1) return TilePlan{3216, 1};
    if (skinny_on && skinny_ok && M <= 32 && nz == 1) {
        const int t = cdiv(N, 64);
        int sp = 1;
        if (K >= 2048) {
            sp = std::min(8, std::max(1, 160 / t));
            while (sp > 1 && K / (64 * sp) < 8) sp--;
        }
        p = TilePlan{3264, want_split > 0 ? want_split : sp};
        return p;
    }
    static const int u16_on = env_int("FF_GEMM_U16", 1);
    const long long t256sq = (long long)cdiv(M, 256) * cdiv(N, 256) * nz;
    if (u16_on && a_layout == 0 && b_layout == 0 && M >= 4096 && K >= 2048 && t256sq >= 256 && want_split <= 1) return TilePlan{256256, 1};
    static const int t256_on = env_int("FF_GEMM_T256", 1);
    if (t256_on && a_layout == 0 && M >= 4096 && N >= 1024 && K >= 1024 && t256 >= 256 && N % 8 == 0 && want_split <= 1) return TilePlan{256128, 1};
    const long long t160 = (long long)cdiv(M, 128) * cdiv(N, 160) * nz;
    int pc_split = 0;
    if (pc_on && pc_ok && N % 160 == 0 && K % 64 == 0 && t160 <= 256)
        for (int sp = 1; sp <= 8 && !pc_split; sp++)
            if (t160 * sp >= 224 && t160 * sp <= 256 && K / sp >= 1024 && K % (64 * sp) == 0) pc_split = sp;
    if (pc_split) p = TilePlan{128160, pc_split};
    else if (t128 >= 200 && t128 < 450 && a_layout == 0 && (long long)cdiv(M, 64) * cdiv(N, 128) * nz >= 400) p = TilePlan{6412, 1};
    else if (t128 >= 200) p = TilePlan{128, 1};
    else if (K >= 2048) {
        int s = (int)std::min<long long>(8, std::max<long long>(2, cdiv(384, t128)));
        while (s > 1 && K / (64 * s) < 8) s--;
        p = TilePlan{128, s};
    } else if (t64 >= 200) p = TilePlan{64, 1};
    else {
        int s = (int)std::min<long long>(4, cdiv(256, t64));
        while (s > 1 && K / (64 * s) < 4) s--;
        p = TilePlan{64, s};
    }
    if (want_split > 0) p.split = want_split;
    static const int pc128 = env_int("FF_GEMM_PC128", 2);
    if (pc128 && p.tile == 128) p.tile = 128002;
    if (pc128 >= 2 && p.tile == 6412) p.tile = 128002;
    static const int pc64 = env_int("FF_GEMM_PC64", 1);
    if (pc64 && p.tile == 64) p.tile = 64002;
    return p;
}

template <int BM, int BN, int AL, int BL, int NS> static int launch_bf16_dma(const GemmParams& P, hipStream_t st) {
    constexpr size_t lds = (size_t)NS * (BM + BN) * kBK * sizeof(bf16);
    if (lds > 64 * 1024) {
        static bool attr_done[64] = {};
        int dev = 0;
        (void)hipGetDevice(&dev);
        if (dev < 0 || dev >= 64 || !attr_done[dev]) {
            hipError_t e = hipFuncSetAttribute((const void*)gemm_bf16_dma_kernel<BM, BN, AL, BL, NS>,
                                               hipFuncAttributeMaxDynamicSharedMemorySize, (int)lds);
            FF_CHECK(e == hipSuccess, FF_ERR_LAUNCH, "hipFuncSetAttribute(gemm dma lds=%zu): %s", lds, hipGetErrorString(e));
            if (dev >= 0 && dev < 64) attr_done[dev] = true;
        }
    }
    const int grid = cdiv(P.M, BM) * cdiv(P.N, BN) * P.split_k * P.nz;
    const int seg = P.a_map.rows_per_seg > 0 || P.b_map.rows_per_seg > 0 || P.a_map.ld >= (1LL << 31) || P.b_map.ld >= (1LL << 31);
    gemm_bf16_dma_kernel<BM, BN, AL, BL, NS><<<dim3(grid), dim3(256), lds, st>>>(P.p[0].A, P.p[0].B, P.M, P.N, P.K, P.split_k, P.k_per_split, P.nz,
                                                                           P.xcd_ms | (P.xcd_ns << 8), (int)P.a_map.ld, (int)P.b_map.ld, seg, P);
    return check_launch("gemm_bf16_dma");
}
template <int BM, int BN, int NS> static int dispatch_bf16_dma(const GemmParams& P, hipStream_t st) {
    if (P.a_layout == 0 && P.b_layout == 0) return launch_bf16_dma<BM, BN, 0, 0, NS>(P, st);
    if (P.a_layout == 0 && P.b_layout == 1) return launch_bf16_dma<BM, BN, 0, 1, NS>(P, st);
    if (P.a_layout == 1 && P.b_layout == 0) return launch_bf16_dma<BM, BN, 1, 0, NS>(P, st);
    return launch_bf16_dma<BM, BN, 1, 1, NS>(P, st);
}
template <int BM, int BN> static int run_bf16_dma_tile(const GemmParams& P, int ns, hipStream_t st) {
    return ns == 2 ? dispatch_bf16_dma<BM, BN, 2>(P, st) : ns == 4 ? dispatch_bf16_dma<BM, BN, 4>(P, st) : dispatch_bf16_dma<BM, BN, 3>(P, st);
}
template <int BM, int BN, int AL, int BL, int NS, int WPC, int NPW = 4, int NCW = 4> static int launch_bf16_pc(const GemmParams& P, hipStream_t st) {
    constexpr size_t lds = (size_t)NS * (BM + BN) * kBK * sizeof(bf16) + (NPW == 8 && BN == 160 ? 4096 : 0);
    static bool attr_done[64] = {};
    int dev = 0;
    (void)hipGetDevice(&dev);
    if (dev < 0 || dev >= 64 || !attr_done[dev]) {
        hipError_t e = hipFuncSetAttribute((const void*)gemm_bf16_pc_kernel<BM, BN, AL, BL, NS, WPC, NPW, NCW>, hipFuncAttributeMaxDynamicSharedMemorySize, (int)lds);
        FF_CHECK(e == hipSuccess, FF_ERR_LAUNCH, "hipFuncSetAttribute(gemm pc lds=%zu): %s", lds, hipGetErrorString(e));
        if (dev >= 0 && dev < 64) attr_done[dev] = true;
    }
    const int grid = cdiv(P.M, BM) * cdiv(P.N, BN) * P.split_k * P.nz;
    const int seg = P.a_map.rows_per_seg > 0 || P.b_map.rows_per_seg > 0 || P.a_map.ld >= (1LL << 31) || P.b_map.ld >= (1LL << 31);
    gemm_bf16_pc_kernel<BM, BN, AL, BL, NS, WPC, NPW, NCW><<<dim3(grid), dim3((NCW + NPW) * 64), lds, st>>>(P.p[0].A, P.p[0].B, P.M, P.N, P.K, P.split_k, P.k_per_split,
                                                                                 P.nz, P.xcd_ms | (P.xcd_ns << 8), (int)P.a_map.ld,
                                                                                 (int)P.b_map.ld, seg, P);
    return check_launch("gemm_bf16_pc");
}
template <int NS> static int dispatch_bf16_pc128(const GemmParams& P, hipStream_t st) {
    if (P.a_layout == 0 && P.b_layout == 0) return launch_bf16_pc<128, 128, 0, 0, NS, 2>(P, st);
    if (P.a_layout == 0 && P.b_layout == 1) return launch_bf16_pc<128, 128, 0, 1, NS, 2>(P, st);
    if (P.a_layout == 1 && P.b_layout == 0) return launch_bf16_pc<128, 128, 1, 0, NS, 2>(P, st);
    return launch_bf16_pc<128, 128, 1, 1, NS, 2>(P, st);
}
static int run_bf16_dma(const GemmParams& P, hipStream_t st) {
    static const int ns_env = env_int("FF_GEMM_STAGES", 0);
    const int ns = P.force_stages > 0 ? P.force_stages : ns_env > 0 ? ns_env : 2;
    if (P.tile == 128160) {
        static const int npw_full = env_int("FF_GEMM_NPW", 8), npw_split = env_int("FF_GEMM_NPW_SPLIT", 4);
        const int npw = P.split_k > 1 ? npw_split : npw_full;
        const int pns = P.force_stages > 0 ? P.force_stages : ns_env > 0 ? ns_env : npw == 8 ? 4 : 3;
        static const int ncw_env = env_int("FF_GEMM_NCW", 4), ncw_split_env = env_int("FF_GEMM_NCW_SPLIT", 4);
        const int ncw = P.force_tile == 128168 ? 8 : (P.split_k > 1 ? ncw_split_env : ncw_env);
        if (ncw == 8) {
            if (P.b_layout == 0) return pns == 3 ? launch_bf16_pc<128, 160, 0, 0, 3, 1, 4, 8>(P, st) : launch_bf16_pc<128, 160, 0, 0, 4, 1, 4, 8>(P, st);
            return pns == 3 ? launch_bf16_pc<128, 160, 0, 1, 3, 1, 4, 8>(P, st) : launch_bf16_pc<128, 160, 0, 1, 4, 1, 4, 8>(P, st);
        }
        if (npw == 8) {
            if (P.b_layout == 0) return pns == 4 ? launch_bf16_pc<128, 160, 0, 0, 4, 1, 8>(P, st) : launch_bf16_pc<128, 160, 0, 0, 3, 1, 8>(P, st);
            return pns == 4 ? launch_bf16_pc<128, 160, 0, 1, 4, 1, 8>(P, st) : launch_bf16_pc<128, 160, 0, 1, 3, 1, 8>(P, st);
        }
        if (P.b_layout == 0) return pns == 4 ? launch_bf16_pc<128, 160, 0, 0, 4, 1>(P, st) : launch_bf16_pc<128, 160, 0, 0, 3, 1>(P, st);
        return pns == 4 ? launch_bf16_pc<128, 160, 0, 1, 4, 1>(P, st) : launch_bf16_pc<128, 160, 0, 1, 3, 1>(P, st);
    }
    if (P.tile == 128002) return dispatch_bf16_pc128<2>(P, st);
    if (P.tile == 256128) {
        static const int npw256 = env_int("FF_GEMM_NPW256", 8);
        if (P.a_layout == 1)
            return P.b_layout == 0 ? launch_bf16_pc<256, 128, 1, 0, 3, 1, 4, 8>(P, st) : launch_bf16_pc<256, 128, 1, 1, 3, 1, 4, 8>(P, st);
        if (npw256 == 8) return P.b_layout == 0 ? launch_bf16_pc<256, 128, 0, 0, 3, 1, 8, 8>(P, st) : launch_bf16_pc<256, 128, 0, 1, 3, 1, 8, 8>(P, st);
        return P.b_layout == 0 ? launch_bf16_pc<256, 128, 0, 0, 3, 1, 4, 8>(P, st) : launch_bf16_pc<256, 128, 0, 1, 3, 1, 4, 8>(P, st);
    }
    if (P.tile == 256256) return launch_bf16_u16<0, 0>(P, st);
    if (P.tile == 3216) return launch_bf16_rows32(P, st);
    if (P.tile == 3264) return launch_bf16_pc<32, 64, 0, 0, 4, 2>(P, st);
    if (P.tile == 128) return run_bf16_dma_tile<128, 128>(P, ns, st);
    if (P.tile == 6412) return run_bf16_dma_tile<64, 128>(P, ns, st);
    if (P.tile == 64002) {
        if (P.a_layout == 0 && P.b_layout == 0) return launch_bf16_pc<64, 64, 0, 0, 3, 2>(P, st);
        if (P.a_layout == 0 && P.b_layout == 1) return launch_bf16_pc<64, 64, 0, 1, 3, 2>(P, st);
        if (P.a_layout == 1 && P.b_layout == 0) return launch_bf16_pc<64, 64, 1, 0, 3, 2>(P, st);
        return launch_bf16_pc<64, 64, 1, 1, 3, 2>(P, st);
    }
    return run_bf16_dma_tile<64, 64>(P, P.force_stages > 0 ? P.force_stages : ns_env > 0 ? ns_env : 3, st);
}

int gemm_pick_split(int dtype, int M, int N, int K, int nz) {
    if (dtype == FF_DTYPE_BF16)
        return std::max(plan_bf16(M, N, K, nz, 0, 0, 0).split, plan_bf16(M, N, K, nz, 0, 0, 1).split);
    const long long tiles = (long long)cdiv(M, kFBM) * cdiv(N, kFBM) * nz;
    if (tiles >= 128 || K < 1024) return 1;
    int s = (int)(256 / tiles);
    s = std::min(s, K / 512);
    s = std::min(s, 16);
    return std::max(s, 1);
}

size_t gemm_workspace_bytes(int dtype, int M, int N, int K, int nz, int split_k) {
    if (split_k <= 0) split_k = gemm_pick_split(dtype, M, N, K, nz);
    return split_k > 1 ? (size_t)split_k * nz * M * N * sizeof(float) : 0;
}

int gemm_launch(GemmParams P, int dtype, void* workspace, size_t ws_bytes, hipStream_t st, int* leave_partial) {
    if (leave_partial) *leave_partial = 1;
    FF_CHECK(P.M > 0 && P.N > 0 && P.K > 0 && P.nz >= 1 && P.nz <= kGemmMaxZ, FF_ERR_SHAPE, "gemm: bad shape M=%d N=%d K=%d nz=%d",
             P.M, P.N, P.K, P.nz);
    P.tile = kFBM;
    if (dtype == FF_DTYPE_BF16) {
        const TilePlan plan = plan_bf16(P.M, P.N, P.K, P.nz, P.split_k, P.a_layout, P.b_layout, P.force_tile);
        P.tile = plan.tile;
        P.split_k = plan.split;
    } else if (P.split_k <= 0) P.split_k = gemm_pick_split(dtype, P.M, P.N, P.K, P.nz);
    const int kq = dtype == FF_DTYPE_BF16 ? kBK : kFBK;
    P.k_per_split = cdiv(cdiv(P.K, P.split_k), kq) * kq;
    P.split_k = cdiv(P.K, P.k_per_split);
    P.partial = nullptr;
    if (P.split_k > 1) {
        const size_t need = gemm_workspace_bytes(dtype, P.M, P.N, P.K, P.nz, P.split_k);
        FF_CHECK(workspace && ws_bytes >= need, FF_ERR_WORKSPACE, "gemm split-K workspace: need %zu have %zu", need, ws_bytes);
        FF_CHECK(P.N % 4 == 0, FF_ERR_UNSUPPORTED, "gemm split-K needs N %% 4 == 0 (N=%d)", P.N);
        P.partial = (float*)workspace;
    }
    {
        const int tm_edge = dtype == FF_DTYPE_BF16 ? (P.tile == 256128 || P.tile == 256256 ? 256 : P.tile == 128 || P.tile == 128160 || P.tile == 128002 ? 128 : P.tile == 3264 || P.tile == 3216 ? 32 : 64) : kFBM;
        const int tn_edge = dtype == FF_DTYPE_BF16 ? (P.tile == 3216 ? 16 : P.tile == 64 || P.tile == 64002 || P.tile == 3264 ? 64 : P.tile == 128160 ? 160 : P.tile == 256256 ? 256 : 128) : kFBM;
        const int tiles_m = cdiv(P.M, tm_edge), tiles_n = cdiv(P.N, tn_edge);
        double best = 1e300;
        P.xcd_ms = 1; P.xcd_ns = 1;
        for (int ms = 1; ms <= 8; ms *= 2) {
            const int ns = 8 / ms;
            if (ms > tiles_m || ns > tiles_n) continue;
            const double cost = (double)P.M / ms + (double)P.N / ns;
            if (cost < best) { best = cost; P.xcd_ms = ms; P.xcd_ns = ns; }
        }
        static const int disable = env_int("FF_GEMM_XCD2D", 1) == 0;
        if (disable) { P.xcd_ms = 1; P.xcd_ns = 1; }
    }
    const int vec = dtype == FF_DTYPE_BF16 ? 8 : 4;
    auto map_ok = [&](const RowMap& m) { return m.ld % vec == 0 && (m.rows_per_seg <= 0 || m.seg_stride % vec == 0); };
    const int a_contig = P.a_layout == 0 ? P.K : P.M, b_contig = P.b_layout == 0 ? P.K : P.N;
    P.a_vec_ok = map_ok(P.a_map) && a_contig % vec == 0;
    P.b_vec_ok = map_ok(P.b_map) && b_contig % vec == 0;
    for (int z = 0; z < P.nz; z++) {
        P.a_vec_ok = P.a_vec_ok && ((uintptr_t)P.p[z].A % 16 == 0);
        P.b_vec_ok = P.b_vec_ok && ((uintptr_t)P.p[z].B % 16 == 0);
    }
    P.c_vec8 = P.N % vec == 0 && map_ok(P.c_map) && map_ok(P.r_map);
    for (int z = 0; z < P.nz; z++)
        P.c_vec8 = P.c_vec8 && ((uintptr_t)P.p[z].C | (uintptr_t)P.p[z].aux_out | (uintptr_t)P.p[z].aux_in | (uintptr_t)P.p[z].residual) % 16 == 0;
    int rc;
    const int prof_id = prof_begin(P, dtype, P.tile, st);
    if (dtype == FF_DTYPE_BF16) {
        FF_CHECK(P.a_vec_ok && P.b_vec_ok, FF_ERR_UNSUPPORTED,
                 "bf16 gemm needs 16-byte aligned operands with contiguous dims %% 8 == 0 (M=%d N=%d K=%d)", P.M, P.N, P.K);
        FF_CHECK(P.N % 4 == 0 && P.c_map.ld % 4 == 0, FF_ERR_UNSUPPORTED, "bf16 gemm needs N %% 4 == 0 (N=%d)", P.N);
        auto span_ok = [&](const RowMap& m, int rows, int contig) {
            const long long last = (m.rows_per_seg > 0 ? (long long)((rows - 1) / m.rows_per_seg) * m.seg_stride + (long long)((rows - 1) % m.rows_per_seg) * m.ld
                                                      : (long long)(rows - 1) * m.ld) + contig;
            return last < (1LL << 30);
        };
        FF_CHECK(span_ok(P.a_map, P.a_layout == 0 ? P.M : P.K, a_contig) && span_ok(P.b_map, P.b_layout == 0 ? P.N : P.K, b_contig),
                 FF_ERR_UNSUPPORTED, "bf16 gemm operands must span < 2^30 elements (M=%d N=%d K=%d)", P.M, P.N, P.K);
        rc = run_bf16_dma(P, st);
    } else {
        rc = dispatch_f32(P, st);
    }
    prof_end(prof_id, st);
    FF_TRY(rc);
    if (P.split_k > 1 && leave_partial && P.nz == 1 && P.scale == 1.f && P.act < 0 && P.act_bwd < 0 && !P.p[0].aux_out && !P.p[0].gate &&
        !P.p[0].residual) {
        *leave_partial = P.split_k;
        return FF_OK;
    }
    if (P.split_k > 1) {
        const long long total = (long long)P.nz * P.M * ((P.N + 7) / 8);
        FF_CHECK(total < (1LL << 31), FF_ERR_UNSUPPORTED, "gemm split-K output too large (M=%d N=%d nz=%d)", P.M, P.N, P.nz);
        const int grid = (int)((total + 255) / 256);
        if (dtype == FF_DTYPE_BF16) hipLaunchKernelGGL(gemm_splitk_epilogue_kernel<bf16>, dim3(grid), dim3(256), 0, st, P);
        else hipLaunchKernelGGL(gemm_splitk_epilogue_kernel<float>, dim3(grid), dim3(256), 0, st, P);
        FF_TRY(check_launch("gemm_splitk_epilogue"));
    }
    return FF_OK;
}

}

#ifdef FF_GEMM_TIMELINE
extern "C" int ff_debug_timeline_read(unsigned long long* out, int n_blocks) {
    return (int)hipMemcpyFromSymbol(out, HIP_SYMBOL(ff::g_timeline), sizeof(unsigned long long) * 8 * n_blocks);
}
#endif

extern "C" size_t ff_gemm_workspace_bytes(const ff_gemm_desc* d) {
    int split = d->split_k;
    if (split <= 0 && d->tile > 0 && d->dtype == FF_DTYPE_BF16) split = ff::plan_bf16(d->M, d->N, d->K, 1, 0, d->a_layout, d->b_layout, d->tile).split;
    return ff::gemm_workspace_bytes(d->dtype, d->M, d->N, d->K, 1, split);
}

extern "C" int ff_gemm(const ff_gemm_desc* d, const void* A, const void* B, void* C, void* aux_out, const void* aux_in,
                       const void* residual, const void* gate, void* workspace, size_t workspace_bytes, ff_stream_t stream) {
    using namespace ff;
    FF_CHECK(d && A && B && C, FF_ERR_SHAPE, "ff_gemm: null argument");
    FF_CHECK(d->dtype == FF_DTYPE_F32 || d->dtype == FF_DTYPE_BF16, FF_ERR_UNSUPPORTED, "ff_gemm: dtype %d", d->dtype);
    FF_CHECK(d->act_bwd < 0 || aux_in, FF_ERR_SHAPE, "ff_gemm: act_bwd needs aux_in");
    GemmParams P = {};
    P.M = d->M; P.N = d->N; P.K = d->K;
    P.a_layout = d->a_layout; P.b_layout = d->b_layout;
    P.a_map = make_rowmap(d->a_map); P.b_map = make_rowmap(d->b_map); P.c_map = make_rowmap(d->c_map); P.r_map = P.c_map;
    P.scale = d->scale; P.act = d->act; P.act_bwd = d->act_bwd; P.split_k = d->split_k;
    P.force_tile = d->tile; P.force_stages = d->stages;
    P.nz = 1;
    P.p[0] = GemmProblem{A, B, C, aux_out, aux_in, residual, gate};
    return gemm_launch(P, d->dtype, workspace, workspace_bytes, (hipStream_t)stream);
}

extern "C" int ff_gemm_profile_enable(int max_records) {
    using namespace ff;
    if (max_records <= 0) { g_prof.on = false; return FF_OK; }
    g_prof.on = false;
    if (max_records > g_prof.cap) {
        hipEvent_t* ev = (hipEvent_t*)realloc(g_prof.ev, sizeof(hipEvent_t) * 2 * max_records);
        ff_gemm_profile_record* rec = (ff_gemm_profile_record*)realloc(g_prof.rec, sizeof(ff_gemm_profile_record) * max_records);
        FF_CHECK(ev && rec, FF_ERR_WORKSPACE, "gemm profile: out of host memory");
        g_prof.ev = ev; g_prof.rec = rec;
        for (int i = 2 * g_prof.cap; i < 2 * max_records; i++) {
            hipError_t e = hipEventCreate(&g_prof.ev[i]);
            FF_CHECK(e == hipSuccess, FF_ERR_LAUNCH, "hipEventCreate: %s", hipGetErrorString(e));
        }
        g_prof.cap = max_records;
    }
    g_prof.n = 0;
    g_prof.on = true;
    return FF_OK;
}
extern "C" int ff_gemm_profile_read(ff_gemm_profile_record* out, int max_records) {
    using namespace ff;
    const int n = std::min(std::min(g_prof.n.load(), g_prof.cap), max_records);
    for (int i = 0; i < n; i++) {
        hipEventSynchronize(g_prof.ev[2 * i + 1]);
        float ms = 0.f;
        hipEventElapsedTime(&ms, g_prof.ev[2 * i], g_prof.ev[2 * i + 1]);
        g_prof.rec[i].ms = ms;
        out[i] = g_prof.rec[i];
    }
    g_prof.n = 0;
    return n;
}

extern "C" int ff_gemm_plan(const ff_gemm_desc* d, int* bm, int* bn, int* split_k) {
    using namespace ff;
    FF_CHECK(d && bm && bn && split_k, FF_ERR_SHAPE, "ff_gemm_plan: null argument");
    if (d->dtype == FF_DTYPE_BF16) {
        const TilePlan p = plan_bf16(d->M, d->N, d->K, 1, d->split_k, d->a_layout, d->b_layout, d->tile);
        *bm = p.tile == 256128 || p.tile == 256256 ? 256 : p.tile == 128 || p.tile == 128160 || p.tile == 128002 ? 128 : p.tile == 3264 || p.tile == 3216 ? 32 : 64;
        *bn = p.tile == 3216 ? 16 : p.tile == 64 || p.tile == 64002 || p.tile == 3264 ? 64 : p.tile == 128160 ? 160 : p.tile == 256256 ? 256 : 128;
        *split_k = p.split;
    } else {
        *bm = *bn = kFBM;
        *split_k = d->split_k > 0 ? d->split_k : gemm_pick_split(d->dtype, d->M, d->N, d->K, 1);
    }
    return FF_OK;
}
```

flamingo-mini_amd/csrc/ff_internal.h:

```cpp
#pragma once
#include <algorithm>
#include "ff_common.h"

namespace ff {

constexpr int kGemmMaxZ = 12;
constexpr int kKvProjGroup = 4;
struct GemmProblem {
    const void* A;
    const void* B;
    void* C;
    void* aux_out;
    const void* aux_in;
    const void* residual;
    const void* gate;
};
struct GemmParams {
    int M, N, K;
    int a_layout, b_layout;
    RowMap a_map, b_map, c_map, r_map;
    float scale;
    int act, act_bwd;
    int split_k, k_per_split;
    int tile;
    int force_tile, force_stages;
    int xcd_ms, xcd_ns;
    float* partial;
    int a_vec_ok, b_vec_ok;
    int c_vec8;
    int nz;
    GemmProblem p[kGemmMaxZ];
};
int gemm_pick_split(int dtype, int M, int N, int K, int nz);
size_t gemm_workspace_bytes(int dtype, int M, int N, int K, int nz, int split_k);
int gemm_launch(GemmParams P, int dtype, void* workspace, size_t ws_bytes, hipStream_t st, int* leave_partial = nullptr);

struct Gemm {
    GemmParams P;
    int dtype;
    Gemm(int dtype_, int M, int N, int K) : dtype(dtype_) {
        P = GemmParams{};
        P.M = M; P.N = N; P.K = K;
        P.scale = 1.f; P.act = FF_ACT_NONE; P.act_bwd = FF_ACT_NONE; P.split_k = 0; P.nz = 0;
        P.a_map = plain_rows(K); P.b_map = plain_rows(K); P.c_map = plain_rows(N); P.r_map = P.c_map;
    }
    Gemm& a(int layout, RowMap m) { P.a_layout = layout; P.a_map = m; return *this; }
    Gemm& b(int layout, RowMap m) { P.b_layout = layout; P.b_map = m; return *this; }
    Gemm& c(RowMap m) { P.c_map = m; P.r_map = m; return *this; }
    Gemm& res_map(RowMap m) { P.r_map = m; return *this; }
    Gemm& scale(float s) { P.scale = s; return *this; }
    Gemm& act(int a) { P.act = a; return *this; }
    Gemm& act_bwd(int a) { P.act_bwd = a; return *this; }
    Gemm& problem(const void* A, const void* B, void* C, void* aux_out = nullptr, const void* aux_in = nullptr,
                  const void* residual = nullptr, const void* gate = nullptr) {
        P.p[P.nz++] = GemmProblem{A, B, C, aux_out, aux_in, residual, gate};
        return *this;
    }
    size_t workspace() const { return gemm_workspace_bytes(dtype, P.M, P.N, P.K, std::max(P.nz, 1), P.split_k); }
    int run(void* ws, size_t ws_bytes, hipStream_t st, int* leave_partial = nullptr) const { return gemm_launch(P, dtype, ws, ws_bytes, st, leave_partial); }
};

int profile_begin(int dtype, int tile, int a_layout, int b_layout, int M, int N, int K, int nz, int split_k, hipStream_t st);
void profile_end(int i, hipStream_t st);

struct LnArgs {
    int dtype;
    int rows, cols;
    RowMap x_map, y_map, dx_map;
    int add_rows_per_seg, add_div;
    float eps;
    int stats_given;
    int dy_splits = 0;
    long long dy_slab = 0;
};
int layernorm_fwd(const LnArgs& a, const void* x, const void* add, const void* gamma, const void* beta, void* y,
                  float* mean, float* rstd, hipStream_t st);
size_t layernorm_bwd_workspace(int rows, int cols);
struct LnDots {
    const void* a = nullptr; const void* alpha_a = nullptr; void* out_a = nullptr;
    const void* b = nullptr; const void* alpha_b = nullptr; void* out_b = nullptr;
};
struct LnPending {
    const float* partial = nullptr;
    int nblk = 0, cols = 0;
    void *dgamma = nullptr, *dbeta = nullptr;
    const void* alpha_a = nullptr; void* out_a = nullptr;
    const void* alpha_b = nullptr; void* out_b = nullptr;
};
constexpr int kLnFinishMax = 8;
bool layernorm_bwd_deferrable(int dtype, int cols);
size_t layernorm_bwd_partial_bytes(int rows, int cols);
int layernorm_bwd_partial_blocks(int rows);
int layernorm_bwd(const LnArgs& a, const void* dy, const void* x, const void* add, const void* gamma, const float* mean,
                  const float* rstd, void* dx, const void* dx_residual, void* dgamma, void* dbeta, void* ws,
                  size_t ws_bytes, hipStream_t st, const LnDots* dots = nullptr, LnPending* pending = nullptr);
int layernorm_bwd_finish(int dtype, const LnPending* sets, int n, hipStream_t st);
size_t rows_reduce_workspace(int rows, int cols, int rows_per_batch, int rows_per_group);
int zero_bytes(void* p, size_t bytes, hipStream_t st);
int rows_reduce(int dtype, int rows, int cols, RowMap x_map, int rows_per_batch, int rows_per_group, const void* x,
                void* out, void* ws, size_t ws_bytes, hipStream_t st);
size_t gate_grad_workspace(int rows, int cols);
int gate_grad(int dtype, int rows, int cols, const void* a, const void* b, const void* alpha, void* dalpha, void* ws,
              size_t ws_bytes, hipStream_t st);
int text_time(int batch, int n_tokens, const void* ml, int elem_bytes, int* out, hipStream_t st);

size_t attention_bwd_workspace(const ff_attn_desc& d);
int attention_fwd(const ff_attn_desc& d, const void* Q, const void* K, const void* V, const int* tt, void* O, float* lse,
                  hipStream_t st);
int attention_bwd(const ff_attn_desc& d, const void* Q, const void* K, const void* V, const int* tt, const void* O,
                  const void* dO, const float* lse, void* dQ, void* dK, void* dV, void* ws, size_t ws_bytes,
                  hipStream_t st);

int attention_bwd_dkv(const ff_attn_desc& d, const void* Q, const void* K, const void* V, const int* tt, const void* dO, const float* lse,
                      const float* Dsum, void* dK, void* dV, hipStream_t st);

struct XaFusedArgs {
    int batch, heads, n_q, n_kv, n_visual, tt_stride, tt_offset;
    int dim, inner;
    float scale, eps;
    int xcd_split;
    ff_strides k, v, dk, dv;
};
struct XaOutArgs {
    const bf16* W;
    const bf16* gate;
    bf16* out;
    bf16* aux;
    unsigned* sync;
    const bf16* ln_g;
    const bf16* ln_b;
    bf16* ln_out;
    float* ln_mean;
    float* ln_rstd;
    const bf16* ln_x;
    const bf16* ln_res;
    float* ln_part;
    float* ln_wpart;
};
size_t xa_ln3_part_bytes(int batch, int heads);
bool xa_out_fusable(const XaFusedArgs& a, int dtype, int dim_head);
bool xa_fused_supported(int dtype, int dim_head, int dim, int inner);
int xa_qattn_fwd(const XaFusedArgs& a, int dtype, int dim_head, const void* y, const void* gamma, const void* beta, const void* Wq, const void* K,
                 const void* V, const int* tt, void* yn, void* Qs, void* O, float* mean, float* rstd, float* lse, hipStream_t st,
                 const XaOutArgs* out = nullptr);
int xa_dattn_bwd(const XaFusedArgs& a, int dtype, int dim_head, const void* dy1, const void* Wo, const void* gate, const void* Qs, const void* K,
                 const void* V, const int* tt, const void* O, const float* lse, void* dO, void* dQ, void* dK, void* dV, float* Dsum,
                 int* single_tile, hipStream_t st, const XaOutArgs* out = nullptr);

bool decode_ffw_supported(int dtype, int M, int d, int ffi);
size_t decode_ffw_workspace_bytes(int d, int ffi);
int decode_ffw(int M, int d, int ffi, int act, float eps, const void* y1, const void* gamma, const void* beta, const void* W1, const void* W3,
               const void* alpha, void* xn, float* mean, float* rstd, void* Hpre, void* Aact, void* ffw_out, void* y_out, void* ws, size_t ws_bytes,
               hipStream_t st);

struct Arena {
    unsigned char* base;
    size_t cap, used;
    Arena(void* p, size_t c) : base((unsigned char*)p), cap(c), used(0) {}
    template <typename T = void> T* take(size_t bytes) {
        size_t at = align_up(used);
        used = at + bytes;
        return (T*)(base ? base + at : nullptr);
    }
    bool ok() const { return used <= cap; }
};

}
```

flamingo-mini_amd/csrc/ff_rowwise.hip:

```cpp
#include "ff_common.h"
#include "ff_internal.h"

namespace ff {

#ifdef FF_XA_TIMELINE
__device__ unsigned long long g_ln_timeline[4096 * 8];
#define FF_LTL(i) do { if (threadIdx.x == 0 && blockIdx.x < 4096) g_ln_timeline[blockIdx.x * 8 + (i)] = __builtin_amdgcn_s_memrealtime(); } while (0)
#else
#define FF_LTL(i) do { } while (0)
#endif

template <typename T, int VEC> FF_DEV void ld(const T* p, float (&o)[VEC]) {
    if constexpr (VEC == 1) o[0] = to_f32(p[0]);
    else Vec<T>::load(p, o);
}
template <typename T, int VEC> FF_DEV void st(T* p, const float (&o)[VEC]) {
    if constexpr (VEC == 1) p[0] = from_f32<T>(o[0]);
    else Vec<T>::store(p, o);
}

template <typename T, int VEC>
__global__ __launch_bounds__(256) void ln_fwd_kernel(const LnArgs a_in, const T* __restrict__ x, const T* __restrict__ add,
                                                     const T* __restrict__ gamma, const T* __restrict__ beta, T* __restrict__ y,
                                                     float* __restrict__ mean, float* __restrict__ rstd) {
    const LnArgs a = fetch_args(a_in);
    pin_args(x, add, gamma, beta, y, mean, rstd);
    const int lane = threadIdx.x & 63;
    const int row = blockIdx.x * 4 + (threadIdx.x >> 6);
    if (row >= a.rows) return;
    const T* xr = x + a.x_map.off(row);
    const T* ar = nullptr;
    if (add) ar = add + (long long)((row % a.add_rows_per_seg) / a.add_div) * a.cols;
    const int nchunk = a.cols / VEC;
    float mu, rs;
    if (nchunk <= 4 * 64 && VEC > 1) {
        float v[4][VEC];
#pragma unroll
        for (int u = 0; u < 4; u++) {
            const int c = lane + 64 * u;
            if (c < nchunk) {
                ld<T, VEC>(xr + c * VEC, v[u]);
                if (ar) {
                    float t[VEC];
                    ld<T, VEC>(ar + c * VEC, t);
#pragma unroll
                    for (int i = 0; i < VEC; i++) v[u][i] += t[i];
                }
            }
        }
        if (a.stats_given) {
            mu = mean[row];
            rs = rstd[row];
        } else {
            float s = 0.f;
#pragma unroll
            for (int u = 0; u < 4; u++)
                if (lane + 64 * u < nchunk)
#pragma unroll
                    for (int i = 0; i < VEC; i++) s += v[u][i];
            mu = wave_sum(s) / (float)a.cols;
            float q = 0.f;
#pragma unroll
            for (int u = 0; u < 4; u++)
                if (lane + 64 * u < nchunk)
#pragma unroll
                    for (int i = 0; i < VEC; i++) q += (v[u][i] - mu) * (v[u][i] - mu);
            rs = rsqrtf(wave_sum(q) / (float)a.cols + a.eps);
            if (lane == 0 && mean) {
                mean[row] = mu;
                rstd[row] = rs;
            }
        }
        if (!y) return;
        T* yr = y + a.y_map.off(row);
#pragma unroll
        for (int u = 0; u < 4; u++) {
            const int c = lane + 64 * u;
            if (c < nchunk) {
                float g[VEC], b[VEC], o[VEC];
                ld<T, VEC>(gamma + c * VEC, g);
                ld<T, VEC>(beta + c * VEC, b);
#pragma unroll
                for (int i = 0; i < VEC; i++) o[i] = (v[u][i] - mu) * rs * g[i] + b[i];
                st<T, VEC>(yr + c * VEC, o);
            }
        }
        return;
    }
    if (a.stats_given) {
        mu = mean[row];
        rs = rstd[row];
    } else {
        float s = 0.f;
        for (int c = lane; c < nchunk; c += 64) {
            float v[VEC];
            ld<T, VEC>(xr + c * VEC, v);
            if (ar) {
                float t[VEC];
                ld<T, VEC>(ar + c * VEC, t);
#pragma unroll
                for (int i = 0; i < VEC; i++) v[i] += t[i];
            }
#pragma unroll
            for (int i = 0; i < VEC; i++) s += v[i];
        }
        mu = wave_sum(s) / (float)a.cols;
        float q = 0.f;
        for (int c = lane; c < nchunk; c += 64) {
            float v[VEC];
            ld<T, VEC>(xr + c * VEC, v);
            if (ar) {
                float t[VEC];
                ld<T, VEC>(ar + c * VEC, t);
#pragma unroll
                for (int i = 0; i < VEC; i++) v[i] += t[i];
            }
#pragma unroll
            for (int i = 0; i < VEC; i++) q += (v[i] - mu) * (v[i] - mu);
        }
        rs = rsqrtf(wave_sum(q) / (float)a.cols + a.eps);
        if (lane == 0 && mean) {
            mean[row] = mu;
            rstd[row] = rs;
        }
    }
    if (!y) return;
    T* yr = y + a.y_map.off(row);
    for (int c = lane; c < nchunk; c += 64) {
        float v[VEC], g[VEC], b[VEC];
        ld<T, VEC>(xr + c * VEC, v);
        if (ar) {
            float t[VEC];
            ld<T, VEC>(ar + c * VEC, t);
#pragma unroll
            for (int i = 0; i < VEC; i++) v[i] += t[i];
        }
        ld<T, VEC>(gamma + c * VEC, g);
        ld<T, VEC>(beta + c * VEC, b);
#pragma unroll
        for (int i = 0; i < VEC; i++) v[i] = (v[i] - mu) * rs * g[i] + b[i];
        st<T, VEC>(yr + c * VEC, v);
    }
}

template <typename T, int VEC>
__global__ __launch_bounds__(256) void ln_bwd_dx_kernel(const LnArgs a_in, const T* __restrict__ dy, const T* __restrict__ x,
                                                        const T* __restrict__ add, const T* __restrict__ gamma,
                                                        const float* __restrict__ mean, const float* __restrict__ rstd, T* dx,
                                                        const T* dx_res) {
    const LnArgs a = fetch_args(a_in);
    pin_args(dy, x, add, gamma, mean, rstd, dx, dx_res);
    const int lane = threadIdx.x & 63;
    const int row = blockIdx.x * 4 + (threadIdx.x >> 6);
    if (row >= a.rows) return;
    const T* xr = x + a.x_map.off(row);
    const T* dyr = dy + a.y_map.off(row);
    const T* ar = nullptr;
    if (add) ar = add + (long long)((row % a.add_rows_per_seg) / a.add_div) * a.cols;
    const float mu = mean[row], rs = rstd[row];
    const int nchunk = a.cols / VEC;
    float s1 = 0.f, s2 = 0.f;
    for (int c = lane; c < nchunk; c += 64) {
        float v[VEC], d[VEC], g[VEC];
        ld<T, VEC>(xr + c * VEC, v);
        if (ar) {
            float t[VEC];
            ld<T, VEC>(ar + c * VEC, t);
#pragma unroll
            for (int i = 0; i < VEC; i++) v[i] += t[i];
        }
        ld<T, VEC>(dyr + c * VEC, d);
        ld<T, VEC>(gamma + c * VEC, g);
#pragma unroll
        for (int i = 0; i < VEC; i++) {
            const float dyh = d[i] * g[i];
            s1 += dyh;
            s2 += dyh * (v[i] - mu) * rs;
        }
    }
    const float m1 = wave_sum(s1) / (float)a.cols, m2 = wave_sum(s2) / (float)a.cols;
    const long long doff = a.dx_map.off(row);
    for (int c = lane; c < nchunk; c += 64) {
        float v[VEC], d[VEC], g[VEC], o[VEC];
        ld<T, VEC>(xr + c * VEC, v);
        if (ar) {
            float t[VEC];
            ld<T, VEC>(ar + c * VEC, t);
#pragma unroll
            for (int i = 0; i < VEC; i++) v[i] += t[i];
        }
        ld<T, VEC>(dyr + c * VEC, d);
        ld<T, VEC>(gamma + c * VEC, g);
#pragma unroll
        for (int i = 0; i < VEC; i++) o[i] = rs * (d[i] * g[i] - m1 - (v[i] - mu) * rs * m2);
        if (dx_res) {
            float q[VEC];
            ld<T, VEC>(dx_res + doff + c * VEC, q);
#pragma unroll
            for (int i = 0; i < VEC; i++) o[i] += q[i];
        }
        st<T, VEC>(dx + doff + c * VEC, o);
    }
}


template <typename T, int VEC, int NCH>
__global__ __launch_bounds__(256) void ln_bwd_fused_kernel(const LnArgs a_in, const T* __restrict__ dy, const T* __restrict__ x,
                                                           const T* __restrict__ add, const T* __restrict__ gamma,
                                                           const float* __restrict__ mean, const float* __restrict__ rstd, T* dx,
                                                           const T* dx_res, const T* __restrict__ dot_a, const T* __restrict__ dot_b,
                                                           float* __restrict__ partial, int rows_per_block) {
    FF_LTL(0);
    const LnArgs a = fetch_args(a_in);
    pin_args(dy, x, add, gamma, mean, rstd, dx, dx_res, dot_a, dot_b, partial, rows_per_block);
    extern __shared__ __attribute__((aligned(16))) float sacc[];
    FF_LTL(1);
    __shared__ float red[4];
    const int lane = threadIdx.x & 63, w = threadIdx.x >> 6;
    const int nchunk = a.cols / VEC;
    float accg[NCH][VEC], accb[NCH][VEC];
#pragma unroll
    for (int i = 0; i < NCH; i++)
#pragma unroll
        for (int e = 0; e < VEC; e++) accg[i][e] = accb[i][e] = 0.f;
    float da = 0.f, db = 0.f;
    const int row_end = min(a.rows, (int)(blockIdx.x + 1) * rows_per_block);
    auto load_dy = [&](int row, const T* dyr, int c, float (&d)[VEC]) {
        if (a.dy_splits > 0) {
            const float* pp = (const float*)dy + (long long)row * a.cols + c * VEC;
#pragma unroll
            for (int e = 0; e < VEC; e++) d[e] = 0.f;
            for (int sp = 0; sp < a.dy_splits; sp++) {
#pragma unroll
                for (int e = 0; e < VEC; e += 4) {
                    const f32x4 q = *(const f32x4*)(pp + (long long)sp * a.dy_slab + e);
                    d[e] += q[0]; d[e + 1] += q[1]; d[e + 2] += q[2]; d[e + 3] += q[3];
                }
            }
        } else ld<T, VEC>(dyr + c * VEC, d);
    };
    for (int row = blockIdx.x * rows_per_block + w; row < row_end; row += 4) {
        const T* xr = x + a.x_map.off(row);
        const T* dyr = a.dy_splits > 0 ? dy : dy + a.y_map.off(row);
        const T* ar = add ? add + (long long)((row % a.add_rows_per_seg) / a.add_div) * a.cols : nullptr;
        const float mu = mean[row], rs = rstd[row];
        float s1 = 0.f, s2 = 0.f;
        constexpr bool KEEP = NCH <= 4;
        constexpr bool HOIST = KEEP && VEC > 1;
        float xk[KEEP ? NCH : 1][VEC], dk[KEEP ? NCH : 1][VEC];
        uint4 rq[HOIST ? NCH : 1], ra[HOIST ? NCH : 1], rb[HOIST ? NCH : 1];
        const long long doff = a.dx_map.off(row);
#pragma unroll
        for (int i = 0; i < NCH; i++) {
            const int c = lane + 64 * i;
            if (c < nchunk) {
                float v[VEC], d[VEC], g[VEC];
                ld<T, VEC>(xr + c * VEC, v);
                if (ar) {
                    float t[VEC];
                    ld<T, VEC>(ar + c * VEC, t);
#pragma unroll
                    for (int e = 0; e < VEC; e++) v[e] += t[e];
                }
                load_dy(row, dyr, c, d);
                ld<T, VEC>(gamma + c * VEC, g);
                if constexpr (HOIST) {
                    if (dx_res) rq[i] = *(const uint4*)(dx_res + doff + c * VEC);
                    if (dot_a) ra[i] = *(const uint4*)(dot_a + doff + c * VEC);
                    if (dot_b) rb[i] = *(const uint4*)(dot_b + doff + c * VEC);
                }
#pragma unroll
                for (int e = 0; e < VEC; e++) {
                    const float dyh = d[e] * g[e], xh = (v[e] - mu) * rs;
                    s1 += dyh;
                    s2 += dyh * xh;
                    if (KEEP) { xk[i][e] = xh; dk[i][e] = d[e]; }
                }
            }
        }
        const float m1 = wave_sum(s1) / (float)a.cols, m2 = wave_sum(s2) / (float)a.cols;
        auto unpack = [](const uint4& r, float (&o)[VEC]) {
            if constexpr (VEC > 1) {
                typedef typename Vec<T>::raw raw_t;
                const raw_t x = __builtin_bit_cast(raw_t, r);
#pragma unroll
                for (int e = 0; e < VEC; e++) o[e] = to_f32(x[e]);
            }
        };
#pragma unroll
        for (int i = 0; i < NCH; i++) {
            const int c = lane + 64 * i;
            if (c < nchunk) {
                float xh[VEC], d[VEC], g[VEC], o[VEC];
                if (KEEP) {
#pragma unroll
                    for (int e = 0; e < VEC; e++) { xh[e] = xk[i][e]; d[e] = dk[i][e]; }
                } else {
                    float v[VEC];
                    ld<T, VEC>(xr + c * VEC, v);
                    if (ar) {
                        float t[VEC];
                        ld<T, VEC>(ar + c * VEC, t);
#pragma unroll
                        for (int e = 0; e < VEC; e++) v[e] += t[e];
                    }
                    load_dy(row, dyr, c, d);
#pragma unroll
                    for (int e = 0; e < VEC; e++) xh[e] = (v[e] - mu) * rs;
                }
                ld<T, VEC>(gamma + c * VEC, g);
#pragma unroll
                for (int e = 0; e < VEC; e++) {
                    o[e] = rs * (d[e] * g[e] - m1 - xh[e] * m2);
                    accg[i][e] += d[e] * xh[e];
                    accb[i][e] += d[e];
                }
                if (dx_res) {
                    float q[VEC];
                    if constexpr (HOIST) unpack(rq[i], q);
                    else ld<T, VEC>(dx_res + doff + c * VEC, q);
                    if (dot_a) {
                        float u[VEC];
                        if constexpr (HOIST) unpack(ra[i], u);
                        else ld<T, VEC>(dot_a + doff + c * VEC, u);
#pragma unroll
                        for (int e = 0; e < VEC; e++) da += q[e] * u[e];
                    }
#pragma unroll
                    for (int e = 0; e < VEC; e++) o[e] += q[e];
                }
                if (dx) {
                    float r[VEC];
#pragma unroll
                    for (int e = 0; e < VEC; e++) r[e] = to_f32(from_f32<T>(o[e]));
                    if (dot_b) {
                        float u[VEC];
                        if constexpr (HOIST) unpack(rb[i], u);
                        else ld<T, VEC>(dot_b + doff + c * VEC, u);
#pragma unroll
                        for (int e = 0; e < VEC; e++) db += r[e] * u[e];
                    }
                    st<T, VEC>(dx + doff + c * VEC, o);
                }
            }
        }
    }
    FF_LTL(2);
    {
        float* mine = sacc + (size_t)w * 2 * a.cols;
#pragma unroll
        for (int i = 0; i < NCH; i++) {
            const int c = lane + 64 * i;
            if (c < nchunk) {
#pragma unroll
                for (int e = 0; e < VEC; e += 4) {
                    *(f32x4*)(mine + c * VEC + e) = f32x4{accg[i][e], accg[i][e + 1], accg[i][e + 2], accg[i][e + 3]};
                    *(f32x4*)(mine + a.cols + c * VEC + e) = f32x4{accb[i][e], accb[i][e + 1], accb[i][e + 2], accb[i][e + 3]};
                }
            }
        }
    }
    __syncthreads();
    FF_LTL(3);
    const long long P = 2LL * a.cols + 2;
    float* out = partial + (long long)blockIdx.x * P;
    for (int i = threadIdx.x * 4; i < 2 * a.cols; i += 256 * 4) {
        const f32x4 s0 = *(const f32x4*)(sacc + i), s1 = *(const f32x4*)(sacc + 2 * a.cols + i);
        const f32x4 s2 = *(const f32x4*)(sacc + 4 * a.cols + i), s3 = *(const f32x4*)(sacc + 6 * a.cols + i);
        float* o = out + i;
        o[0] = (s0[0] + s1[0]) + (s2[0] + s3[0]); o[1] = (s0[1] + s1[1]) + (s2[1] + s3[1]);
        o[2] = (s0[2] + s1[2]) + (s2[2] + s3[2]); o[3] = (s0[3] + s1[3]) + (s2[3] + s3[3]);
    }
    da = block_sum<4>(da, red);
    db = block_sum<4>(db, red);
    if (threadIdx.x == 0) { out[2 * a.cols] = da; out[2 * a.cols + 1] = db; }
    FF_LTL(4);
}

template <typename T>
FF_DEV void ln_final_body(int nblk, int cols, const float* __restrict__ partial, T* dgamma, T* dbeta, const T* alpha_a, T* out_a, const T* alpha_b,
                          T* out_b) {
    __shared__ float red[16][17];
    const int P = 2 * cols + 2;
    const int tx = threadIdx.x & 15, ty = threadIdx.x >> 4;
    const int idx = blockIdx.x * 16 + tx;
    float v[8] = {0.f, 0.f, 0.f, 0.f, 0.f, 0.f, 0.f, 0.f};
    if (idx < P) {
        int b = ty;
        for (; b + 7 * 16 < nblk; b += 8 * 16) {
#pragma unroll
            for (int u = 0; u < 8; u++) v[u] += partial[(long long)(b + 16 * u) * P + idx];
        }
        for (; b < nblk; b += 16) v[0] += partial[(long long)b * P + idx];
    }
    red[ty][tx] = ((v[0] + v[1]) + (v[2] + v[3])) + ((v[4] + v[5]) + (v[6] + v[7]));
    __syncthreads();
    if (ty == 0 && idx < P) {
        float s = 0.f;
#pragma unroll
        for (int u = 0; u < 16; u++) s += red[u][tx];
        const float v = s;
        if (idx < cols) { if (dgamma) dgamma[idx] = from_f32<T>(v); }
        else if (idx < 2 * cols) { if (dbeta) dbeta[idx - cols] = from_f32<T>(v); }
        else if (idx == 2 * cols) {
            if (out_a) { const float t = tanhf(to_f32(alpha_a[0])); out_a[0] = from_f32<T>(v * (1.f - t * t)); }
        } else if (out_b) { const float t = tanhf(to_f32(alpha_b[0])); out_b[0] = from_f32<T>(v * (1.f - t * t)); }
    }
}
template <typename T>
__global__ __launch_bounds__(256) void ln_bwd_final_kernel(int nblk, int cols, const float* __restrict__ partial, T* dgamma, T* dbeta,
                                                           const T* alpha_a, T* out_a, const T* alpha_b, T* out_b) {
    pin_args(nblk, cols, partial, dgamma, dbeta, alpha_a, out_a, alpha_b, out_b);
    ln_final_body<T>(nblk, cols, partial, dgamma, dbeta, alpha_a, out_a, alpha_b, out_b);
}
struct LnFinishTable {
    LnPending s[kLnFinishMax];
};
template <typename T>
__global__ __launch_bounds__(256) void ln_bwd_final_multi_kernel(const LnFinishTable t) {
    const LnPending& e = t.s[blockIdx.y];
    if ((int)blockIdx.x * 16 >= 2 * e.cols + 2) return;
    ln_final_body<T>(e.nblk, e.cols, e.partial, (T*)e.dgamma, (T*)e.dbeta, (const T*)e.alpha_a, (T*)e.out_a, (const T*)e.alpha_b, (T*)e.out_b);
}

struct ColReduceArgs {
    int rows, cols;
    RowMap x_map, y_map;
    int rows_per_batch, rows_per_group, n_batch;
    int add_rows_per_seg, add_div;
    int rows_per_split, nsplit, ngroups;
};

template <typename T, int VEC, int MODE>
__global__ __launch_bounds__(256) void col_reduce_kernel(const ColReduceArgs a_in, const T* __restrict__ x, const T* __restrict__ dy,
                                                         const T* __restrict__ add, const float* __restrict__ mean,
                                                         const float* __restrict__ rstd, float* __restrict__ partial) {
    const ColReduceArgs a = fetch_args(a_in);
    pin_args(x, dy, add, mean, rstd, partial);
    constexpr int NS = MODE == 1 ? 2 : 1;
    __shared__ float red[4][NS][64 * VEC];
    const int tx = threadIdx.x & 63, ty = threadIdx.x >> 6;
    const int col = (blockIdx.x * 64 + tx) * VEC;
    const int g = blockIdx.y, split = blockIdx.z;
    float acc[NS][VEC];
#pragma unroll
    for (int s = 0; s < NS; s++)
#pragma unroll
        for (int i = 0; i < VEC; i++) acc[s][i] = 0.f;
    if (col < a.cols) {
        const int n_g = a.n_batch * a.rows_per_group;
        const int i_end = min(n_g, (split + 1) * a.rows_per_split);
        for (int i = split * a.rows_per_split + ty; i < i_end; i += 4) {
            const int bi = i / a.rows_per_group, j = i - bi * a.rows_per_group;
            const int row = bi * a.rows_per_batch + g * a.rows_per_group + j;
            if (row >= a.rows) continue;
            float v[VEC];
            ld<T, VEC>(x + a.x_map.off(row) + col, v);
            if (MODE == 0) {
#pragma unroll
                for (int e = 0; e < VEC; e++) acc[0][e] += v[e];
            } else {
                if (add) {
                    float t[VEC];
                    ld<T, VEC>(add + (long long)((row % a.add_rows_per_seg) / a.add_div) * a.cols + col, t);
#pragma unroll
                    for (int e = 0; e < VEC; e++) v[e] += t[e];
                }
                float d[VEC];
                ld<T, VEC>(dy + a.y_map.off(row) + col, d);
                const float mu = mean[row], rs = rstd[row];
#pragma unroll
                for (int e = 0; e < VEC; e++) {
                    acc[0][e] += d[e] * (v[e] - mu) * rs;
                    acc[1][e] += d[e];
                }
            }
        }
    }
#pragma unroll
    for (int s = 0; s < NS; s++)
#pragma unroll
        for (int e = 0; e < VEC; e++) red[ty][s][tx * VEC + e] = acc[s][e];
    __syncthreads();
    if (ty == 0 && col < a.cols) {
#pragma unroll
        for (int s = 0; s < NS; s++)
#pragma unroll
            for (int e = 0; e < VEC; e++) {
                const float v = red[0][s][tx * VEC + e] + red[1][s][tx * VEC + e] + red[2][s][tx * VEC + e] + red[3][s][tx * VEC + e];
                partial[(((long long)split * a.ngroups + g) * NS + s) * a.cols + col + e] = v;
            }
    }
}

template <typename T>
__global__ __launch_bounds__(256) void col_reduce_final_kernel(int nsplit, int ngroups, int nslots, int cols,
                                                               const float* __restrict__ partial, T* out0, T* out1) {
    pin_args(nsplit, ngroups, nslots, cols, partial, out0, out1);
    const long long total = (long long)ngroups * nslots * cols;
    for (long long idx = (long long)blockIdx.x * 256 + threadIdx.x; idx < total; idx += (long long)gridDim.x * 256) {
        float v0 = 0.f, v1 = 0.f, v2 = 0.f, v3 = 0.f;
        int s = 0;
        for (; s + 4 <= nsplit; s += 4) {
            v0 += partial[(long long)s * total + idx];
            v1 += partial[(long long)(s + 1) * total + idx];
            v2 += partial[(long long)(s + 2) * total + idx];
            v3 += partial[(long long)(s + 3) * total + idx];
        }
        for (; s < nsplit; s++) v0 += partial[(long long)s * total + idx];
        const float v = (v0 + v1) + (v2 + v3);
        const int c = (int)(idx % cols);
        const long long gs = idx / cols;
        const int slot = (int)(gs % nslots), g = (int)(gs / nslots);
        T* out = slot == 0 ? out0 : out1;
        out[(long long)g * cols + c] = from_f32<T>(v);
    }
}

template <typename T, int VEC>
__global__ __launch_bounds__(256) void dot_partial_kernel(long long n, const T* __restrict__ a, const T* __restrict__ b,
                                                          float* __restrict__ partial) {
    pin_args(n, a, b, partial);
    __shared__ float red[4];
    float s = 0.f;
    const long long nchunk = n / VEC;
    for (long long c = (long long)blockIdx.x * 256 + threadIdx.x; c < nchunk; c += (long long)gridDim.x * 256) {
        float u[VEC], v[VEC];
        ld<T, VEC>(a + c * VEC, u);
        ld<T, VEC>(b + c * VEC, v);
#pragma unroll
        for (int i = 0; i < VEC; i++) s += u[i] * v[i];
    }
    s = block_sum<4>(s, red);
    if (threadIdx.x == 0) partial[blockIdx.x] = s;
}
template <typename T>
__global__ __launch_bounds__(256) void gate_grad_final_kernel(int nblk, const float* __restrict__ partial, const T* alpha, T* dalpha) {
    pin_args(nblk, partial, alpha, dalpha);
    __shared__ float red[4];
    float s = 0.f;
    for (int i = threadIdx.x; i < nblk; i += 256) s += partial[i];
    s = block_sum<4>(s, red);
    if (threadIdx.x == 0) {
        const float t = tanhf(to_f32(alpha[0]));
        dalpha[0] = from_f32<T>(s * (1.f - t * t));
    }
}

template <typename I> __global__ void text_time_kernel(int batch, int n, const I* __restrict__ ml, int* __restrict__ out) {
    const int b = blockIdx.x * blockDim.x + threadIdx.x;
    if (b >= batch) return;
    int acc = 0;
    for (int i = 0; i < n; i++) {
        acc += (int)ml[(long long)b * n + i];
        out[(long long)b * n + i] = acc;
    }
}

int gate_grad(int dtype, int rows, int cols, const void* a, const void* b, const void* alpha, void* dalpha, void* ws,
              size_t ws_bytes, hipStream_t st_);

static bool vec_ok(int dtype, int cols, std::initializer_list<RowMap> maps, std::initializer_list<const void*> ptrs) {
    const int n = dtype == FF_DTYPE_BF16 ? 8 : 4;
    if (cols % n) return false;
    for (const RowMap& m : maps)
        if (m.ld % n || (m.rows_per_seg > 0 && m.seg_stride % n)) return false;
    for (const void* p : ptrs)
        if (p && (uintptr_t)p % 16) return false;
    return true;
}

#define FF_DISPATCH_T_VEC(dtype, vec, ...)                 \
    do {                                                    \
        if ((dtype) == FF_DTYPE_BF16) {                     \
            typedef bf16 T;                                 \
            if (vec) { constexpr int VEC = 8; __VA_ARGS__; }       \
            else { constexpr int VEC = 1; __VA_ARGS__; }           \
        } else {                                            \
            typedef float T;                                \
            if (vec) { constexpr int VEC = 4; __VA_ARGS__; }       \
            else { constexpr int VEC = 1; __VA_ARGS__; }           \
        }                                                   \
    } while (0)

int layernorm_fwd(const LnArgs& a, const void* x, const void* add, const void* gamma, const void* beta, void* y, float* mean,
                  float* rstd, hipStream_t st_) {
    FF_CHECK(a.rows > 0 && a.cols > 0 && x, FF_ERR_SHAPE, "layernorm_fwd: bad shape rows=%d cols=%d", a.rows, a.cols);
    FF_CHECK(!a.stats_given || (mean && rstd), FF_ERR_SHAPE, "layernorm_fwd: stats_given without statistics");
    FF_CHECK(!y || (gamma && beta), FF_ERR_SHAPE, "layernorm_fwd: gamma/beta missing");
    FF_CHECK(!add || (a.add_rows_per_seg > 0 && a.add_div > 0), FF_ERR_SHAPE, "layernorm_fwd: addend needs add_rows_per_seg/add_div");
    const bool v = vec_ok(a.dtype, a.cols, {a.x_map, a.y_map}, {x, add, gamma, beta, y});
    const int grid = cdiv(a.rows, 4);
    FF_DISPATCH_T_VEC(a.dtype, v, ln_fwd_kernel<T, VEC><<<dim3(grid), dim3(256), 0, st_>>>(a, (const T*)x, (const T*)add, (const T*)gamma, (const T*)beta, (T*)y, mean, rstd));
    return check_launch("ln_fwd");
}

static void split_plan(int n_rows_in_group, int col_blocks, int ngroups, int& rows_per_split, int& nsplit) {
    int target = std::max(1, 512 / std::max(1, col_blocks * ngroups));
    nsplit = std::max(1, std::min(std::min(target, 32), cdiv(n_rows_in_group, 32)));
    rows_per_split = cdiv(n_rows_in_group, nsplit);
    nsplit = cdiv(n_rows_in_group, rows_per_split);
}

static size_t col_reduce_ws(int n_rows_in_group, int cols, int ngroups, int nslots) {
    int rps, ns;
    split_plan(n_rows_in_group, 1, ngroups, rps, ns);
    return (size_t)ns * ngroups * nslots * cols * sizeof(float);
}


static int ln_fused_blocks(int rows, int& rows_per_block) {
    rows_per_block = std::max(4, (cdiv(rows, 256) + 3) / 4 * 4);
    return cdiv(rows, rows_per_block);
}
static bool ln_fused_ok(int dtype, int cols, bool vec) {
    if (!vec) return false;
    const int n = dtype == FF_DTYPE_BF16 ? 8 : 4;
    return cdiv(cols / n, 64) <= 8 && (size_t)8 * cols * sizeof(float) <= 150 * 1024;
}
size_t layernorm_bwd_workspace(int rows, int cols) {
    int rpb;
    const size_t fused = (size_t)ln_fused_blocks(rows, rpb) * (2 * (size_t)cols + 2) * sizeof(float);
    return std::max(fused, col_reduce_ws(rows, cols, 1, 2));
}

bool layernorm_bwd_deferrable(int dtype, int cols) { return cols % (dtype == FF_DTYPE_BF16 ? 8 : 4) == 0 && ln_fused_ok(dtype, cols, true); }
int layernorm_bwd_partial_blocks(int rows) {
    int rpb;
    return ln_fused_blocks(rows, rpb);
}
size_t layernorm_bwd_partial_bytes(int rows, int cols) { return (size_t)layernorm_bwd_partial_blocks(rows) * (2 * (size_t)cols + 2) * sizeof(float); }

template <typename T, int VEC>
static int launch_ln_fused(const LnArgs& a, const void* dy, const void* x, const void* add, const void* gamma, const float* mean,
                           const float* rstd, void* dx, const void* dx_res, const LnDots& dots, void* dgamma, void* dbeta, float* partial,
                           hipStream_t st_, LnPending* pending) {
    int rpb;
    const int nblk = ln_fused_blocks(a.rows, rpb);
    const int nch = cdiv(a.cols / VEC, 64);
    const size_t lds = (size_t)8 * a.cols * sizeof(float);
#define FF_LN_LAUNCH(NCH)                                                                                                                 \
    do {                                                                                                                                  \
        if (lds > 48 * 1024) {                                                                                                            \
            static bool attr[64] = {};                                                                                                    \
            int dev = 0;                                                                                                                  \
            (void)hipGetDevice(&dev);                                                                                                     \
            if (dev < 0 || dev >= 64 || !attr[dev]) {                                                                                     \
                hipFuncSetAttribute((const void*)ln_bwd_fused_kernel<T, VEC, NCH>, hipFuncAttributeMaxDynamicSharedMemorySize, 150 * 1024); \
                if (dev >= 0 && dev < 64) attr[dev] = true;                                                                               \
            }                                                                                                                             \
        }                                                                                                                                 \
        ln_bwd_fused_kernel<T, VEC, NCH><<<dim3(nblk), dim3(256), lds, st_>>>(a, (const T*)dy, (const T*)x, (const T*)add, (const T*)gamma, \
                                                                              mean, rstd, (T*)dx, (const T*)dx_res, (const T*)dots.a,     \
                                                                              (const T*)dots.b, partial, rpb);                            \
    } while (0)
    if (nch <= 2) FF_LN_LAUNCH(2);
    else if (nch <= 4) FF_LN_LAUNCH(4);
    else FF_LN_LAUNCH(8);
#undef FF_LN_LAUNCH
    FF_TRY(check_launch("ln_bwd_fused"));
    if (pending) {
        pending->partial = partial; pending->nblk = nblk; pending->cols = a.cols; pending->dgamma = dgamma; pending->dbeta = dbeta;
        pending->alpha_a = dots.alpha_a; pending->out_a = dots.out_a; pending->alpha_b = dots.alpha_b; pending->out_b = dots.out_b;
        return FF_OK;
    }
    const int P = 2 * a.cols + 2;
    ln_bwd_final_kernel<T><<<dim3(cdiv(P, 16)), dim3(256), 0, st_>>>(nblk, a.cols, partial, (T*)dgamma, (T*)dbeta, (const T*)dots.alpha_a,
                                                                     (T*)dots.out_a, (const T*)dots.alpha_b, (T*)dots.out_b);
    return check_launch("ln_bwd_final");
}

int layernorm_bwd(const LnArgs& a, const void* dy, const void* x, const void* add, const void* gamma, const float* mean,
                  const float* rstd, void* dx, const void* dx_residual, void* dgamma, void* dbeta, void* ws, size_t ws_bytes,
                  hipStream_t st_, const LnDots* dots_in, LnPending* pending) {
    FF_CHECK(a.rows > 0 && a.cols > 0 && dy && x && gamma && mean && rstd, FF_ERR_SHAPE, "layernorm_bwd: null/shape");
    if (pending) *pending = LnPending{};
    FF_CHECK(!add || (a.add_rows_per_seg > 0 && a.add_div > 0), FF_ERR_SHAPE, "layernorm_bwd: addend needs add_rows_per_seg/add_div");
    const LnDots dots = dots_in ? *dots_in : LnDots{};
    FF_CHECK(!dots.a || dx_residual, FF_ERR_SHAPE, "layernorm_bwd: dot_a is taken against dx_residual");
    FF_CHECK(!dots.b || dx, FF_ERR_SHAPE, "layernorm_bwd: dot_b is taken against dx");
    const bool v = vec_ok(a.dtype, a.cols, {a.x_map, a.y_map, a.dx_map}, {x, add, gamma, dy, dx, dx_residual, dots.a, dots.b});
    FF_CHECK(a.dy_splits == 0 || (ln_fused_ok(a.dtype, a.cols, v) && (dgamma || dots.a || dots.b) && a.cols % 4 == 0), FF_ERR_UNSUPPORTED,
             "layernorm_bwd: summing split-K slabs needs the one-pass kernel");
    if (ln_fused_ok(a.dtype, a.cols, v) && (dgamma || dots.a || dots.b)) {
        FF_CHECK(!dgamma == !dbeta, FF_ERR_SHAPE, "layernorm_bwd: dgamma and dbeta come together");
        int rpb;
        const size_t need = (size_t)ln_fused_blocks(a.rows, rpb) * (2 * (size_t)a.cols + 2) * sizeof(float);
        FF_CHECK(ws && ws_bytes >= need, FF_ERR_WORKSPACE, "layernorm_bwd workspace: need %zu have %zu", need, ws_bytes);
        if (a.dtype == FF_DTYPE_BF16) return launch_ln_fused<bf16, 8>(a, dy, x, add, gamma, mean, rstd, dx, dx_residual, dots, dgamma, dbeta, (float*)ws, st_, pending);
        return launch_ln_fused<float, 4>(a, dy, x, add, gamma, mean, rstd, dx, dx_residual, dots, dgamma, dbeta, (float*)ws, st_, pending);
    }
    if (dots.a) FF_TRY(gate_grad(a.dtype, a.rows, a.cols, dx_residual, dots.a, dots.alpha_a, dots.out_a, ws, ws_bytes, st_));
    if (dx) {
        const int grid = cdiv(a.rows, 4);
        FF_DISPATCH_T_VEC(a.dtype, v, ln_bwd_dx_kernel<T, VEC><<<dim3(grid), dim3(256), 0, st_>>>(a, (const T*)dy, (const T*)x, (const T*)add, (const T*)gamma, mean, rstd, (T*)dx, (const T*)dx_residual));
        FF_TRY(check_launch("ln_bwd_dx"));
    }
    if (dgamma || dbeta) {
        FF_CHECK(dgamma && dbeta, FF_ERR_SHAPE, "layernorm_bwd: dgamma and dbeta come together");
        const int vecn = v ? (a.dtype == FF_DTYPE_BF16 ? 8 : 4) : 1;
        ColReduceArgs c = {};
        c.rows = a.rows; c.cols = a.cols; c.x_map = a.x_map; c.y_map = a.y_map;
        c.rows_per_batch = a.rows; c.rows_per_group = a.rows; c.n_batch = 1; c.ngroups = 1;
        c.add_rows_per_seg = a.add_rows_per_seg; c.add_div = a.add_div;
        const int col_blocks = cdiv(a.cols, 64 * vecn);
        split_plan(a.rows, col_blocks, 1, c.rows_per_split, c.nsplit);
        const size_t need = (size_t)c.nsplit * 2 * a.cols * sizeof(float);
        FF_CHECK(ws && ws_bytes >= need, FF_ERR_WORKSPACE, "layernorm_bwd workspace: need %zu have %zu", need, ws_bytes);
        FF_DISPATCH_T_VEC(a.dtype, v, col_reduce_kernel<T, VEC, 1><<<dim3(col_blocks, 1, c.nsplit), dim3(256), 0, st_>>>(c, (const T*)x, (const T*)dy, (const T*)add, mean, rstd, (float*)ws));
        FF_TRY(check_launch("ln_bwd_param_partial"));
        const int grid = std::min(cdiv(2LL * a.cols, 256), 1024);
        if (a.dtype == FF_DTYPE_BF16)
            hipLaunchKernelGGL(col_reduce_final_kernel<bf16>, dim3(grid), dim3(256), 0, st_, c.nsplit, 1, 2, a.cols, (const float*)ws, (bf16*)dgamma, (bf16*)dbeta);
        else
            hipLaunchKernelGGL(col_reduce_final_kernel<float>, dim3(grid), dim3(256), 0, st_, c.nsplit, 1, 2, a.cols, (const float*)ws, (float*)dgamma, (float*)dbeta);
        FF_TRY(check_launch("ln_bwd_param_final"));
    }
    if (dots.b) FF_TRY(gate_grad(a.dtype, a.rows, a.cols, dx, dots.b, dots.alpha_b, dots.out_b, ws, ws_bytes, st_));
    return FF_OK;
}

int layernorm_bwd_finish(int dtype, const LnPending* sets, int n, hipStream_t st_) {
    for (int i0 = 0; i0 < n; i0 += kLnFinishMax) {
        LnFinishTable t = {};
        int cnt = 0, pmax = 0;
        for (int i = i0; i < n && i < i0 + kLnFinishMax; i++)
            if (sets[i].partial) {
                t.s[cnt++] = sets[i];
                pmax = std::max(pmax, 2 * sets[i].cols + 2);
            }
        if (!cnt) continue;
        const dim3 grid(cdiv(pmax, 16), cnt);
        if (dtype == FF_DTYPE_BF16) ln_bwd_final_multi_kernel<bf16><<<grid, dim3(256), 0, st_>>>(t);
        else ln_bwd_final_multi_kernel<float><<<grid, dim3(256), 0, st_>>>(t);
        FF_TRY(check_launch("ln_bwd_final_multi"));
    }
    return FF_OK;
}

size_t rows_reduce_workspace(int rows, int cols, int rows_per_batch, int rows_per_group) {
    if (rows_per_batch <= 0 || rows_per_group <= 0) return 0;
    const int ngroups = cdiv(rows_per_batch, rows_per_group);
    const int n_batch = cdiv(rows, rows_per_batch);
    return col_reduce_ws(n_batch * rows_per_group, cols, ngroups, 1);
}

int rows_reduce(int dtype, int rows, int cols, RowMap x_map, int rows_per_batch, int rows_per_group, const void* x, void* out,
                void* ws, size_t ws_bytes, hipStream_t st_) {
    FF_CHECK(rows > 0 && cols > 0 && rows_per_batch > 0 && rows_per_group > 0 && x && out, FF_ERR_SHAPE, "rows_reduce: bad arguments");
    FF_CHECK(rows % rows_per_batch == 0 && rows_per_batch % rows_per_group == 0, FF_ERR_SHAPE,
             "rows_reduce: rows=%d rows_per_batch=%d rows_per_group=%d do not nest", rows, rows_per_batch, rows_per_group);
    const bool v = vec_ok(dtype, cols, {x_map}, {x, out});
    const int vecn = v ? (dtype == FF_DTYPE_BF16 ? 8 : 4) : 1;
    ColReduceArgs c = {};
    c.rows = rows; c.cols = cols; c.x_map = x_map; c.y_map = x_map;
    c.rows_per_batch = rows_per_batch; c.rows_per_group = rows_per_group;
    c.n_batch = rows / rows_per_batch; c.ngroups = rows_per_batch / rows_per_group;
    const int col_blocks = cdiv(cols, 64 * vecn);
    split_plan(c.n_batch * rows_per_group, col_blocks, c.ngroups, c.rows_per_split, c.nsplit);
    const size_t need = (size_t)c.nsplit * c.ngroups * cols * sizeof(float);
    FF_CHECK(ws && ws_bytes >= need, FF_ERR_WORKSPACE, "rows_reduce workspace: need %zu have %zu", need, ws_bytes);
    FF_DISPATCH_T_VEC(dtype, v, col_reduce_kernel<T, VEC, 0><<<dim3(col_blocks, c.ngroups, c.nsplit), dim3(256), 0, st_>>>(c, (const T*)x, (const T*)nullptr, (const T*)nullptr, (const float*)nullptr, (const float*)nullptr, (float*)ws));
    FF_TRY(check_launch("rows_reduce_partial"));
    const int grid = std::min(cdiv((long long)c.ngroups * cols, 256), 1024);
    if (dtype == FF_DTYPE_BF16)
        hipLaunchKernelGGL(col_reduce_final_kernel<bf16>, dim3(grid), dim3(256), 0, st_, c.nsplit, c.ngroups, 1, cols, (const float*)ws, (bf16*)out, (bf16*)nullptr);
    else
        hipLaunchKernelGGL(col_reduce_final_kernel<float>, dim3(grid), dim3(256), 0, st_, c.nsplit, c.ngroups, 1, cols, (const float*)ws, (float*)out, (float*)nullptr);
    return check_launch("rows_reduce_final");
}

__global__ __launch_bounds__(256) void zero_bytes_kernel(unsigned char* __restrict__ p, size_t n) {
    for (size_t i = (size_t)blockIdx.x * 256 + threadIdx.x; i < n; i += (size_t)gridDim.x * 256) p[i] = 0;
}

int zero_bytes(void* p, size_t bytes, hipStream_t st) {
    if (bytes == 0) return 0;
    FF_CHECK(p, FF_ERR_SHAPE, "zero_bytes: null pointer");
    const int grid = (int)std::min<size_t>(1024, (bytes + 255) / 256);
    hipLaunchKernelGGL(zero_bytes_kernel, dim3(grid), dim3(256), 0, st, (unsigned char*)p, bytes);
    return check_launch("zero_bytes");
}

static int gate_blocks(long long n) { return (int)std::max<long long>(1, std::min<long long>(512, n / 4096)); }
size_t gate_grad_workspace(int rows, int cols) { return (size_t)gate_blocks((long long)rows * cols) * sizeof(float); }

int gate_grad(int dtype, int rows, int cols, const void* a, const void* b, const void* alpha, void* dalpha, void* ws,
              size_t ws_bytes, hipStream_t st_) {
    const long long n = (long long)rows * cols;
    FF_CHECK(n > 0 && a && b && alpha && dalpha, FF_ERR_SHAPE, "gate_grad: bad arguments");
    const int nblk = gate_blocks(n);
    FF_CHECK(ws && ws_bytes >= nblk * sizeof(float), FF_ERR_WORKSPACE, "gate_grad workspace too small");
    const bool v = vec_ok(dtype, cols, {}, {a, b});
    FF_DISPATCH_T_VEC(dtype, v, dot_partial_kernel<T, VEC><<<dim3(nblk), dim3(256), 0, st_>>>(n, (const T*)a, (const T*)b, (float*)ws));
    FF_TRY(check_launch("gate_grad_partial"));
    if (dtype == FF_DTYPE_BF16)
        hipLaunchKernelGGL(gate_grad_final_kernel<bf16>, dim3(1), dim3(256), 0, st_, nblk, (const float*)ws, (const bf16*)alpha, (bf16*)dalpha);
    else
        hipLaunchKernelGGL(gate_grad_final_kernel<float>, dim3(1), dim3(256), 0, st_, nblk, (const float*)ws, (const float*)alpha, (float*)dalpha);
    return check_launch("gate_grad_final");
}

int text_time(int batch, int n_tokens, const void* ml, int elem_bytes, int* out, hipStream_t st_) {
    FF_CHECK(batch > 0 && n_tokens > 0 && ml && out, FF_ERR_SHAPE, "text_time: bad arguments");
    const int grid = cdiv(batch, 64);
    if (elem_bytes == 8) hipLaunchKernelGGL(text_time_kernel<long long>, dim3(grid), dim3(64), 0, st_, batch, n_tokens, (const long long*)ml, out);
    else if (elem_bytes == 4) hipLaunchKernelGGL(text_time_kernel<int>, dim3(grid), dim3(64), 0, st_, batch, n_tokens, (const int*)ml, out);
    else if (elem_bytes == 1) hipLaunchKernelGGL(text_time_kernel<unsigned char>, dim3(grid), dim3(64), 0, st_, batch, n_tokens, (const unsigned char*)ml, out);
    else FF_CHECK(false, FF_ERR_UNSUPPORTED, "text_time: media_locations element size %d", elem_bytes);
    return check_launch("text_time");
}

}

static ff::LnArgs to_args(const ff_ln_desc* d) {
    ff::LnArgs a;
    a.dtype = d->dtype; a.rows = d->rows; a.cols = d->cols;
    a.x_map = ff::make_rowmap(d->x_map); a.y_map = ff::make_rowmap(d->y_map); a.dx_map = ff::make_rowmap(d->dx_map);
    a.add_rows_per_seg = d->add_rows_per_seg; a.add_div = d->add_div;
    a.eps = d->eps; a.stats_given = d->stats_given;
    return a;
}
extern "C" int ff_layernorm_fwd(const ff_ln_desc* d, const void* x, const void* add, const void* gamma, const void* beta, void* y,
                                float* mean, float* rstd, ff_stream_t stream) {
    return ff::layernorm_fwd(to_args(d), x, add, gamma, beta, y, mean, rstd, (hipStream_t)stream);
}
extern "C" size_t ff_layernorm_bwd_workspace_bytes(const ff_ln_desc* d) { return ff::layernorm_bwd_workspace(d->rows, d->cols); }
extern "C" int ff_layernorm_bwd(const ff_ln_desc* d, const void* dy, const void* x, const void* add, const void* gamma,
                                const float* mean, const float* rstd, void* dx, const void* dx_residual, void* dgamma, void* dbeta,
                                void* workspace, size_t workspace_bytes, ff_stream_t stream) {
    return ff::layernorm_bwd(to_args(d), dy, x, add, gamma, mean, rstd, dx, dx_residual, dgamma, dbeta, workspace, workspace_bytes,
                             (hipStream_t)stream, nullptr);
}
extern "C" size_t ff_rows_reduce_workspace_bytes(const ff_reduce_desc* d) {
    return ff::rows_reduce_workspace(d->rows, d->cols, d->rows_per_batch, d->rows_per_group);
}
extern "C" int ff_rows_reduce(const ff_reduce_desc* d, const void* x, void* out, void* workspace, size_t workspace_bytes,
                              ff_stream_t stream) {
    return ff::rows_reduce(d->dtype, d->rows, d->cols, ff::make_rowmap(d->x_map), d->rows_per_batch, d->rows_per_group, x, out,
                           workspace, workspace_bytes, (hipStream_t)stream);
}
extern "C" size_t ff_gate_grad_workspace_bytes(int rows, int cols) { return ff::gate_grad_workspace(rows, cols); }
extern "C" int ff_gate_grad(int dtype, int rows, int cols, const void* a, const void* b, const void* alpha, void* dalpha,
                            void* workspace, size_t workspace_bytes, ff_stream_t stream) {
    return ff::gate_grad(dtype, rows, cols, a, b, alpha, dalpha, workspace, workspace_bytes, (hipStream_t)stream);
}
extern "C" int ff_text_time(int batch, int n_tokens, const void* media_locations, int elem_bytes, int* text_time, ff_stream_t stream) {
    return ff::text_time(batch, n_tokens, media_locations, elem_bytes, text_time, (hipStream_t)stream);
}

#ifdef FF_XA_TIMELINE
extern "C" int ff_debug_ln_timeline_read(unsigned long long* out, int n_blocks) {
    return (int)hipMemcpyFromSymbol(out, HIP_SYMBOL(ff::g_ln_timeline), sizeof(unsigned long long) * 8 * n_blocks);
}
#endif
```

Before: 801.0.

## Fuse dK/dV projection GEMMs via K-segments and skip media dx materialization

Merges the two kv-projection backward GEMMs into one K-segmented GEMM whose kernel switches its A/B operand descriptors at segment boundaries, replacing two launches and a read-modify-write of dkv. When T==1, the media layernorm backward no longer writes the full media dx tensor. It accumulates per-block column sums that one final kernel reduces across layers into the time-embedding gradient. It also lets the FFN down-projection leave split-K slabs for the layernorm backward to sum. These changes add more LDS per block and more complex kernel control flow.

```diff
diff --git a/flamingo-mini_amd/csrc/ff_api.hip b/flamingo-mini_amd/csrc/ff_api.hip
--- a/flamingo-mini_amd/csrc/ff_api.hip
+++ b/flamingo-mini_amd/csrc/ff_api.hip
@@ -113,7 +113,7 @@
     for (int nz = 1; nz <= 4; nz++) {
         g(s.D, s.ffi, s.Mq, nz); g(s.ffi, s.D, s.Mq, nz); g(s.D, s.inner, s.Mq, nz); g(s.inner, s.D, s.Mq, nz); g(s.inner, s.D, s.Mkv, nz);
     }
-    g(s.Mkv, s.D, s.inner, 1);
+    g(s.Mkv, s.D, s.inner, 1); g(s.Mkv, s.D, 2 * s.inner, 1);
     w = std::max(w, layernorm_bwd_workspace(s.Mf, s.D));
     w = std::max(w, layernorm_bwd_workspace(s.Mq, s.D));
     w = std::max(w, rows_reduce_workspace(s.Mq, s.D, s.q, 1));
@@ -147,13 +147,15 @@
     g.dK = a.take((size_t)s.Mkv * s.inner * s.es);
     g.dV = a.take((size_t)s.Mkv * s.inner * s.es);
 }
-static void rs_take_ln_partials(const RsDims& s, Arena& a, bool deferrable, float** lnp) {
-    for (int i = 0; i < 3; i++) lnp[i] = deferrable ? a.take<float>(layernorm_bwd_partial_bytes(i == 2 ? s.Mf : s.Mq, s.D)) : nullptr;
+static void rs_take_ln_partials(const RsDims& s, Arena& a, bool deferrable, bool media_sums, float** lnp) {
+    for (int i = 0; i < 2; i++) lnp[i] = deferrable ? a.take<float>(layernorm_bwd_partial_bytes(s.Mq, s.D)) : nullptr;
+    lnp[2] = !deferrable ? nullptr : a.take<float>(media_sums ? layernorm_bwd_colsum_partial_bytes(s.Mf, s.D) : layernorm_bwd_partial_bytes(s.Mf, s.D));
 }
 
 struct RsScratch {
     RsChain c;
     void *dx0, *dxf;
+    bool media_sums;
     void* dx_out[kMaxDepth];
     RsLayerGrads L[kMaxDepth];
     float* lnp[3 * kMaxDepth + 1];
@@ -161,17 +163,19 @@
 static size_t rs_scratch_layout(const RsDims& s, void* base, size_t cap, bool bwd, RsScratch& o) {
     Arena a(base, cap);
     rs_take_ws(s, a, o.c);
+    o.media_sums = false;
     if (bwd) {
         o.dx0 = a.take((size_t)s.Mq * s.D * s.es);
         rs_take_chain(s, a, o.c);
-        o.dxf = a.take((size_t)s.Mf * s.D * s.es);
+        static const int defer_ln = dbg_switch("FF_DEFER_LN", 1);
+        const bool lnd = defer_ln != 0 && layernorm_bwd_deferrable(s.dt, s.D);
+        o.media_sums = lnd && s.T == 1 && layernorm_bwd_colsum_ok(s.dt, s.D);
+        o.dxf = o.media_sums ? nullptr : a.take((size_t)s.Mf * s.D * s.es);
         for (int l = 0; l < s.depth; l++) {
             o.dx_out[l] = a.take((size_t)s.Mq * s.D * s.es);
             rs_take_layer_grads(s, a, o.L[l]);
         }
-        static const int defer_ln = dbg_switch("FF_DEFER_LN", 1);
-        const bool lnd = defer_ln != 0 && layernorm_bwd_deferrable(s.dt, s.D);
-        for (int l = 0; l < s.depth; l++) rs_take_ln_partials(s, a, lnd, o.lnp + 3 * l);
+        for (int l = 0; l < s.depth; l++) rs_take_ln_partials(s, a, lnd, o.media_sums, o.lnp + 3 * l);
         o.lnp[3 * s.depth] = lnd ? a.take<float>(layernorm_bwd_partial_bytes(s.Mq, s.D)) : nullptr;
     }
     return align_up(a.used);
@@ -228,7 +232,8 @@
 static int rs_ln_bwd(const RsChain& W, float* partial, LnPending* pending, const LnArgs& a, const void* dy, const void* x, const void* add,
                      const void* gamma, const float* mean, const float* rstd, void* dx, const void* dx_res, void* dg, void* db, hipStream_t st) {
     if (partial)
-        return layernorm_bwd(a, dy, x, add, gamma, mean, rstd, dx, dx_res, dg, db, partial, layernorm_bwd_partial_bytes(a.rows, a.cols), st, nullptr, pending);
+        return layernorm_bwd(a, dy, x, add, gamma, mean, rstd, dx, dx_res, dg, db, partial,
+                             a.dx_colsum ? layernorm_bwd_colsum_partial_bytes(a.rows, a.cols) : layernorm_bwd_partial_bytes(a.rows, a.cols), st, nullptr, pending);
     return layernorm_bwd(a, dy, x, add, gamma, mean, rstd, dx, dx_res, dg, db, W.ws, W.gws, st);
 }
 
@@ -238,22 +243,28 @@
                              hipStream_t st) {
     const RowMap pD = s.pD, pI = s.pI, pF = s.pF;
     FF_TRY(Gemm(s.dt, s.Mq, s.ffi, s.D).a(0, pD).b(1, pF).c(pF).act_bwd(s.act).problem(dx_out, p[11], T.dH, nullptr, L.Hpre).run(W.ws, W.gws, st));
-    FF_TRY(Gemm(s.dt, s.Mq, s.D, s.ffi).a(0, pF).b(1, pD).c(pD).problem(T.dH, p[10], W.dxn).run(W.ws, W.gws, st));
-    FF_TRY(rs_ln_bwd(W, lnp[0], &ln_sets[0], s.ln_latents(), W.dxn, L.x_mid, nullptr, p[8], L.mean_f, L.rstd_f, T.dx_mid, dx_out, g[8], g[9], st));
+    int dxn_splits = 1;
+    FF_TRY(Gemm(s.dt, s.Mq, s.D, s.ffi).a(0, pF).b(1, pD).c(pD).problem(T.dH, p[10], W.dxn).run(W.ws, W.gws, st, lnp[0] ? &dxn_splits : nullptr));
+    LnArgs lf = s.ln_latents();
+    if (dxn_splits > 1) { lf.dy_splits = dxn_splits; lf.dy_slab = (long long)s.Mq * s.D; }
+    FF_TRY(rs_ln_bwd(W, lnp[0], &ln_sets[0], lf, dxn_splits > 1 ? W.ws : W.dxn, L.x_mid, nullptr, p[8], L.mean_f, L.rstd_f, T.dx_mid, dx_out, g[8], g[9], st));
     FF_TRY(Gemm(s.dt, s.Mq, s.inner, s.D).a(0, pD).b(1, pI).c(pI).problem(T.dx_mid, p[7], W.dO).run(W.ws, W.gws, st));
     FF_TRY(attention_bwd(rs_attn_desc(s), L.Qs, L.K, L.V, nullptr, L.O, W.dO, L.lse, T.dQs, T.dK, T.dV, W.attn_ws, s.attn_ws, st));
-    FF_TRY(Gemm(s.dt, s.Mkv, s.D, s.inner).a(0, pI).b(1, pD).c(pD).problem(T.dK, p[5], W.dkv).run(W.ws, W.gws, st));
-    FF_TRY(Gemm(s.dt, s.Mkv, s.D, s.inner).a(0, pI).b(1, pD).c(pD).problem(T.dV, p[6], W.dkv, nullptr, nullptr, W.dkv).run(W.ws, W.gws, st));
+    FF_TRY(Gemm(s.dt, s.Mkv, s.D, s.inner).a(0, pI).b(1, pD).c(pD).problem(T.dK, p[5], W.dkv).segment(T.dV, p[6]).run(W.ws, W.gws, st));
     FF_TRY(Gemm(s.dt, s.Mq, s.D, s.inner).a(0, pI).b(1, pD).c(pD).res_map(s.kv_lat).scale(s.scale)
                .problem(T.dQs, p[4], W.dln, nullptr, nullptr, s.kv_latent_rows(W.dkv)).run(W.ws, W.gws, st));
     FF_TRY(rs_ln_bwd(W, lnp[1], &ln_sets[1], ln_args(s.dt, s.Mq, s.D, x_map, pD, pD), W.dln, x_in, nullptr, p[2], L.mean_l, L.rstd_l, dx_in, T.dx_mid, g[2],
                      g[3], st));
-    return rs_ln_bwd(W, lnp[2], &ln_sets[2], s.ln_media(s.kv_media), W.dkv, x_f, tpe, p[0], mean_m, rstd_m, dx_f, dx_f_res, g[0], g[1], st);
-}
-
-static int rs_input_grads(const RsDims& s, const void* dx0, const void* dxf, void* d_latents, void* d_tpe, void* ws, size_t ws_bytes, hipStream_t st) {
+    LnArgs lm = s.ln_media(s.kv_media);
+    lm.dx_colsum = dx_f == nullptr;
+    return rs_ln_bwd(W, lnp[2], &ln_sets[2], lm, W.dkv, x_f, tpe, p[0], mean_m, rstd_m, dx_f, dx_f_res, g[0], g[1], st);
+}
+
+static int rs_input_grads(const RsDims& s, const void* dx0, const void* dxf, void* d_latents, void* d_tpe, void* ws, size_t ws_bytes, hipStream_t st,
+                          const float* sums = nullptr, long long sums_stride = 0) {
     FF_TRY(rows_reduce(s.dt, s.Mq, s.D, s.pD, s.q, 1, dx0, d_latents, ws, ws_bytes, st));
     if (s.nte > s.T) FF_TRY(zero_bytes((char*)d_tpe + (size_t)s.T * s.D * s.es, (size_t)(s.nte - s.T) * s.D * s.es, st));
+    if (!dxf) return layernorm_bwd_colsum_finish(s.dt, s.depth, s.Mf, s.D, sums, sums_stride, d_tpe, st);
     return rows_reduce(s.dt, s.Mf, s.D, s.pD, s.F, s.v, dxf, d_tpe, ws, ws_bytes, st);
 }
 
@@ -338,7 +349,7 @@
             }
         }
     }
-    return rs_input_grads(s, W.dx0, dxf, G[0], G[1], ws, gws, st);
+    return rs_input_grads(s, W.dx0, dxf, G[0], G[1], ws, gws, st, W.lnp[2], s.depth > 1 ? W.lnp[5] - W.lnp[2] : 0);
 }
 
 struct RsProSaved { float *mean_m, *rstd_m; };
@@ -364,7 +375,7 @@
     rs_take_ws(s, a, o.c);
     rs_take_chain(s, a, o.c);
     rs_take_layer_grads(s, a, o.g);
-    rs_take_ln_partials(s, a, layernorm_bwd_deferrable(s.dt, s.D), o.lnp);
+    rs_take_ln_partials(s, a, layernorm_bwd_deferrable(s.dt, s.D), false, o.lnp);
     return align_up(a.used);
 }
 
diff --git a/flamingo-mini_amd/csrc/ff_gemm.hip b/flamingo-mini_amd/csrc/ff_gemm.hip
--- a/flamingo-mini_amd/csrc/ff_gemm.hip
+++ b/flamingo-mini_amd/csrc/ff_gemm.hip
@@ -381,8 +381,10 @@
     static_assert((AL == 0 || BM == 256 || BM == 128 || BM == 64) && (BL == 0 || BN == 128 || BN == 64 || BN == 160), "M-major staging exists for 64 / 128 / 256-wide A tiles and 64 / 128 / 160-wide B tiles only");
     static_assert(PER_TILE * (NS - 1) <= 63, "vmcnt overflow");
 
+    constexpr bool KSEG = BM == 128 && BN == 128;
+    const int k_seg = KSEG ? h_seg >> 1 : 0;
     RowMap a_map{h_ald, 0, 0}, b_map{h_bld, 0, 0};
-    if (h_seg) { a_map = P.a_map; b_map = P.b_map; }
+    if (KSEG ? h_seg & 1 : h_seg) { a_map = P.a_map; b_map = P.b_map; }
     const void* opA = hA;
     const void* opB = hB;
     const int tiles_m = (hM + BM - 1) / BM, tiles_n = (hN + BN - 1) / BN;
@@ -397,8 +399,9 @@
     const int pw = producer ? w - NCW : w;
     const int wm = (w & (NCW - 1)) >> 1, wn = w & 1;
     bf16* dummy = smem + NS * STAGE + (pw & 3) * 512;
-    const __amdgpu_buffer_rsrc_t ra = __builtin_amdgcn_make_buffer_rsrc((void*)opA, 0, 0x7fffffff, 0x00020000);
-    const __amdgpu_buffer_rsrc_t rb = __builtin_amdgcn_make_buffer_rsrc((void*)opB, 0, 0x7fffffff, 0x00020000);
+    __amdgpu_buffer_rsrc_t ra = __builtin_amdgcn_make_buffer_rsrc((void*)opA, 0, 0x7fffffff, 0x00020000);
+    __amdgpu_buffer_rsrc_t rb = __builtin_amdgcn_make_buffer_rsrc((void*)opB, 0, 0x7fffffff, 0x00020000);
+    int seg = 0, seg_lo = 0, seg_hi = k_seg > 0 ? k_seg : 0x7fffffff;
     const int nk = (k_end - k_begin + kBK - 1) / kBK;
 
     f32x4 acc[MT][NT];
@@ -412,12 +415,21 @@
     const unsigned a_step = AL == 0 ? 2u : (unsigned)a_map.ld * 2u, b_step = BL == 0 ? 2u : (unsigned)b_map.ld * 2u;
     auto issue = [&](int tile) {
         bf16* st = smem + (tile % NS) * STAGE;
-        const int k0 = k_begin + tile * kBK;
-        const bool full = k0 + kBK <= k_end;
+        int k0 = k_begin + tile * kBK, k_lim = k_end;
+        if constexpr (KSEG) {
+            if (k0 >= seg_hi) {
+                do { seg++; seg_lo = seg_hi; seg_hi += k_seg; } while (k0 >= seg_hi);
+                ra = __builtin_amdgcn_make_buffer_rsrc((void*)P.p[seg].A, 0, 0x7fffffff, 0x00020000);
+                rb = __builtin_amdgcn_make_buffer_rsrc((void*)P.p[seg].B, 0, 0x7fffffff, 0x00020000);
+            }
+            k0 -= seg_lo;
+            k_lim = min(k_end, seg_hi) - seg_lo;
+        }
+        const bool full = k0 + kBK <= k_lim;
         if (full && a_plain) dma_tile_fast<BM, AL, NPW>(ra, st, va, (unsigned)k0 * a_step, pw);
-        else dma_tile<BM, AL, NPW>(ra, st, a_map, m_base, hM, k0, k_end, pw, l);
+        else dma_tile<BM, AL, NPW>(ra, st, a_map, m_base, hM, k0, k_lim, pw, l);
         if (full && b_plain) BS::fast(rb, st + A_ELEMS, vb, (unsigned)k0 * b_step, pw, dummy);
-        else BS::slow(rb, st + A_ELEMS, b_map, n_base, hN, k0, k_end, pw, l, dummy);
+        else BS::slow(rb, st + A_ELEMS, b_map, n_base, hN, k0, k_lim, pw, l, dummy);
     };
     if (producer) {
         dma_prepare<BM, AL, NPW>(a_map, m_base, hM, pw, l, va);
@@ -1028,7 +1040,7 @@
     const int seg = P.a_map.rows_per_seg > 0 || P.b_map.rows_per_seg > 0 || P.a_map.ld >= (1LL << 31) || P.b_map.ld >= (1LL << 31);
     gemm_bf16_pc_kernel<BM, BN, AL, BL, NS, WPC, NPW, NCW><<<dim3(grid), dim3((NCW + NPW) * 64), lds, st>>>(P.p[0].A, P.p[0].B, P.M, P.N, P.K, P.split_k, P.k_per_split,
                                                                                  P.nz, P.xcd_ms | (P.xcd_ns << 8), (int)P.a_map.ld,
-                                                                                 (int)P.b_map.ld, seg, P);
+                                                                                 (int)P.b_map.ld, seg | (P.k_seg << 1), P);
     return check_launch("gemm_bf16_pc");
 }
 template <int NS> static int dispatch_bf16_pc128(const GemmParams& P, hipStream_t st) {
@@ -1099,6 +1111,30 @@
     if (leave_partial) *leave_partial = 1;
     FF_CHECK(P.M > 0 && P.N > 0 && P.K > 0 && P.nz >= 1 && P.nz <= kGemmMaxZ, FF_ERR_SHAPE, "gemm: bad shape M=%d N=%d K=%d nz=%d",
              P.M, P.N, P.K, P.nz);
+    P.k_seg = 0;
+    if (P.nseg > 1) {
+        FF_CHECK(P.nz == 1 && P.nseg <= kGemmMaxZ && P.act < 0 && P.act_bwd < 0 && !P.p[0].aux_out && !P.p[0].gate, FF_ERR_UNSUPPORTED,
+                 "gemm: K-segmented operands go with one problem and a plain / scale / residual epilogue");
+        const int ft = P.force_tile ? P.force_tile : 128002;
+        bool merged = dtype == FF_DTYPE_BF16 && P.K % kBK == 0 && (long long)P.K * P.nseg < (1LL << 30);
+        if (merged) {
+            const TilePlan plan = plan_bf16(P.M, P.N, P.K * P.nseg, 1, P.split_k, P.a_layout, P.b_layout, ft);
+            merged = plan.tile == 128002 && (plan.split <= 1 || (workspace && ws_bytes >= gemm_workspace_bytes(dtype, P.M, P.N, P.K * P.nseg, 1, plan.split)));
+        }
+        if (!merged) {
+            for (int s = 0; s < P.nseg; s++) {
+                GemmParams Q = P;
+                Q.nseg = 0;
+                Q.p[0].A = P.p[s].A; Q.p[0].B = P.p[s].B;
+                if (s > 0) { Q.p[0].residual = P.p[0].C; Q.r_map = P.c_map; }
+                FF_TRY(gemm_launch(Q, dtype, workspace, ws_bytes, st));
+            }
+            return FF_OK;
+        }
+        P.k_seg = P.K; P.K *= P.nseg; P.force_tile = ft;
+    }
+    const int k_pair = P.k_seg ? P.k_seg : P.K;
+    const int n_pairs = P.k_seg ? P.nseg : P.nz;
     P.tile = kFBM;
     if (dtype == FF_DTYPE_BF16) {
         const TilePlan plan = plan_bf16(P.M, P.N, P.K, P.nz, P.split_k, P.a_layout, P.b_layout, P.force_tile);
@@ -1132,10 +1168,10 @@
     }
     const int vec = dtype == FF_DTYPE_BF16 ? 8 : 4;
     auto map_ok = [&](const RowMap& m) { return m.ld % vec == 0 && (m.rows_per_seg <= 0 || m.seg_stride % vec == 0); };
-    const int a_contig = P.a_layout == 0 ? P.K : P.M, b_contig = P.b_layout == 0 ? P.K : P.N;
+    const int a_contig = P.a_layout == 0 ? k_pair : P.M, b_contig = P.b_layout == 0 ? k_pair : P.N;
     P.a_vec_ok = map_ok(P.a_map) && a_contig % vec == 0;
     P.b_vec_ok = map_ok(P.b_map) && b_contig % vec == 0;
-    for (int z = 0; z < P.nz; z++) {
+    for (int z = 0; z < n_pairs; z++) {
         P.a_vec_ok = P.a_vec_ok && ((uintptr_t)P.p[z].A % 16 == 0);
         P.b_vec_ok = P.b_vec_ok && ((uintptr_t)P.p[z].B % 16 == 0);
     }
@@ -1153,7 +1189,7 @@
                                                       : (long long)(rows - 1) * m.ld) + contig;
             return last < (1LL << 30);
         };
-        FF_CHECK(span_ok(P.a_map, P.a_layout == 0 ? P.M : P.K, a_contig) && span_ok(P.b_map, P.b_layout == 0 ? P.N : P.K, b_contig),
+        FF_CHECK(span_ok(P.a_map, P.a_layout == 0 ? P.M : k_pair, a_contig) && span_ok(P.b_map, P.b_layout == 0 ? P.N : k_pair, b_contig),
                  FF_ERR_UNSUPPORTED, "bf16 gemm operands must span < 2^30 elements (M=%d N=%d K=%d)", P.M, P.N, P.K);
         rc = run_bf16_dma(P, st);
     } else {
diff --git a/flamingo-mini_amd/csrc/ff_internal.h b/flamingo-mini_amd/csrc/ff_internal.h
--- a/flamingo-mini_amd/csrc/ff_internal.h
+++ b/flamingo-mini_amd/csrc/ff_internal.h
@@ -29,6 +29,8 @@
     int a_vec_ok, b_vec_ok;
     int c_vec8;
     int nz;
+    int nseg;
+    int k_seg;
     GemmProblem p[kGemmMaxZ];
 };
 int gemm_pick_split(int dtype, int M, int N, int K, int nz);
@@ -56,6 +58,11 @@
         P.p[P.nz++] = GemmProblem{A, B, C, aux_out, aux_in, residual, gate};
         return *this;
     }
+    Gemm& segment(const void* A, const void* B) {
+        if (P.nseg == 0) P.nseg = 1;
+        P.p[P.nseg++] = GemmProblem{A, B, nullptr, nullptr, nullptr, nullptr, nullptr};
+        return *this;
+    }
     size_t workspace() const { return gemm_workspace_bytes(dtype, P.M, P.N, P.K, std::max(P.nz, 1), P.split_k); }
     int run(void* ws, size_t ws_bytes, hipStream_t st, int* leave_partial = nullptr) const { return gemm_launch(P, dtype, ws, ws_bytes, st, leave_partial); }
 };
@@ -71,6 +78,7 @@
     float eps;
     int stats_given;
     int dy_splits = 0;
+    int dx_colsum = 0;
     long long dy_slab = 0;
 };
 int layernorm_fwd(const LnArgs& a, const void* x, const void* add, const void* gamma, const void* beta, void* y,
@@ -82,7 +90,7 @@
 };
 struct LnPending {
     const float* partial = nullptr;
-    int nblk = 0, cols = 0;
+    int nblk = 0, cols = 0, stride = 0;
     void *dgamma = nullptr, *dbeta = nullptr;
     const void* alpha_a = nullptr; void* out_a = nullptr;
     const void* alpha_b = nullptr; void* out_b = nullptr;
@@ -91,6 +99,9 @@
 bool layernorm_bwd_deferrable(int dtype, int cols);
 size_t layernorm_bwd_partial_bytes(int rows, int cols);
 int layernorm_bwd_partial_blocks(int rows);
+bool layernorm_bwd_colsum_ok(int dtype, int cols);
+size_t layernorm_bwd_colsum_partial_bytes(int rows, int cols);
+int layernorm_bwd_colsum_finish(int dtype, int nsets, int rows, int cols, const float* partial, long long set_stride, void* out, hipStream_t st);
 int layernorm_bwd(const LnArgs& a, const void* dy, const void* x, const void* add, const void* gamma, const float* mean,
                   const float* rstd, void* dx, const void* dx_residual, void* dgamma, void* dbeta, void* ws,
                   size_t ws_bytes, hipStream_t st, const LnDots* dots = nullptr, LnPending* pending = nullptr);
diff --git a/flamingo-mini_amd/csrc/ff_rowwise.hip b/flamingo-mini_amd/csrc/ff_rowwise.hip
--- a/flamingo-mini_amd/csrc/ff_rowwise.hip
+++ b/flamingo-mini_amd/csrc/ff_rowwise.hip
@@ -204,7 +204,7 @@
 }
 
 
-template <typename T, int VEC, int NCH>
+template <typename T, int VEC, int NCH, bool DXSUM = false>
 __global__ __launch_bounds__(256) void ln_bwd_fused_kernel(const LnArgs a_in, const T* __restrict__ dy, const T* __restrict__ x,
                                                            const T* __restrict__ add, const T* __restrict__ gamma,
                                                            const float* __restrict__ mean, const float* __restrict__ rstd, T* dx,
@@ -218,11 +218,14 @@
     __shared__ float red[4];
     const int lane = threadIdx.x & 63, w = threadIdx.x >> 6;
     const int nchunk = a.cols / VEC;
-    float accg[NCH][VEC], accb[NCH][VEC];
+    float accg[NCH][VEC], accb[NCH][VEC], accx[DXSUM ? NCH : 1][VEC];
 #pragma unroll
     for (int i = 0; i < NCH; i++)
 #pragma unroll
-        for (int e = 0; e < VEC; e++) accg[i][e] = accb[i][e] = 0.f;
+        for (int e = 0; e < VEC; e++) {
+            accg[i][e] = accb[i][e] = 0.f;
+            if constexpr (DXSUM) accx[i][e] = 0.f;
+        }
     float da = 0.f, db = 0.f;
     const int row_end = min(a.rows, (int)(blockIdx.x + 1) * rows_per_block);
     auto load_dy = [&](int row, const T* dyr, int c, float (&d)[VEC]) {
@@ -314,6 +317,7 @@
                     o[e] = rs * (d[e] * g[e] - m1 - xh[e] * m2);
                     accg[i][e] += d[e] * xh[e];
                     accb[i][e] += d[e];
+                    if constexpr (DXSUM) accx[i][e] += o[e];
                 }
                 if (dx_res) {
                     float q[VEC];
@@ -347,7 +351,8 @@
     }
     FF_LTL(2);
     {
-        float* mine = sacc + (size_t)w * 2 * a.cols;
+        constexpr int NIMG = DXSUM ? 3 : 2;
+        float* mine = sacc + (size_t)w * NIMG * a.cols;
 #pragma unroll
         for (int i = 0; i < NCH; i++) {
             const int c = lane + 64 * i;
@@ -356,18 +361,20 @@
                 for (int e = 0; e < VEC; e += 4) {
                     *(f32x4*)(mine + c * VEC + e) = f32x4{accg[i][e], accg[i][e + 1], accg[i][e + 2], accg[i][e + 3]};
                     *(f32x4*)(mine + a.cols + c * VEC + e) = f32x4{accb[i][e], accb[i][e + 1], accb[i][e + 2], accb[i][e + 3]};
+                    if constexpr (DXSUM) *(f32x4*)(mine + 2 * a.cols + c * VEC + e) = f32x4{accx[i][e], accx[i][e + 1], accx[i][e + 2], accx[i][e + 3]};
                 }
             }
         }
     }
     __syncthreads();
     FF_LTL(3);
-    const long long P = 2LL * a.cols + 2;
+    constexpr int NIMG = DXSUM ? 3 : 2;
+    const long long P = (long long)NIMG * a.cols + 2;
     float* out = partial + (long long)blockIdx.x * P;
-    for (int i = threadIdx.x * 4; i < 2 * a.cols; i += 256 * 4) {
-        const f32x4 s0 = *(const f32x4*)(sacc + i), s1 = *(const f32x4*)(sacc + 2 * a.cols + i);
-        const f32x4 s2 = *(const f32x4*)(sacc + 4 * a.cols + i), s3 = *(const f32x4*)(sacc + 6 * a.cols + i);
-        float* o = out + i;
+    for (int i = threadIdx.x * 4; i < NIMG * a.cols; i += 256 * 4) {
+        const f32x4 s0 = *(const f32x4*)(sacc + i), s1 = *(const f32x4*)(sacc + NIMG * a.cols + i);
+        const f32x4 s2 = *(const f32x4*)(sacc + 2 * NIMG * a.cols + i), s3 = *(const f32x4*)(sacc + 3 * NIMG * a.cols + i);
+        float* o = out + i + (i >= 2 * a.cols ? 2 : 0);
         o[0] = (s0[0] + s1[0]) + (s2[0] + s3[0]); o[1] = (s0[1] + s1[1]) + (s2[1] + s3[1]);
         o[2] = (s0[2] + s1[2]) + (s2[2] + s3[2]); o[3] = (s0[3] + s1[3]) + (s2[3] + s3[3]);
     }
@@ -379,9 +386,10 @@
 
 template <typename T>
 FF_DEV void ln_final_body(int nblk, int cols, const float* __restrict__ partial, T* dgamma, T* dbeta, const T* alpha_a, T* out_a, const T* alpha_b,
-                          T* out_b) {
+                          T* out_b, int stride = 0) {
     __shared__ float red[16][17];
     const int P = 2 * cols + 2;
+    if (stride <= 0) stride = P;
     const int tx = threadIdx.x & 15, ty = threadIdx.x >> 4;
     const int idx = blockIdx.x * 16 + tx;
     float v[8] = {0.f, 0.f, 0.f, 0.f, 0.f, 0.f, 0.f, 0.f};
@@ -389,9 +397,9 @@
         int b = ty;
         for (; b + 7 * 16 < nblk; b += 8 * 16) {
 #pragma unroll
-            for (int u = 0; u < 8; u++) v[u] += partial[(long long)(b + 16 * u) * P + idx];
-        }
-        for (; b < nblk; b += 16) v[0] += partial[(long long)b * P + idx];
+            for (int u = 0; u < 8; u++) v[u] += partial[(long long)(b + 16 * u) * stride + idx];
+        }
+        for (; b < nblk; b += 16) v[0] += partial[(long long)b * stride + idx];
     }
     red[ty][tx] = ((v[0] + v[1]) + (v[2] + v[3])) + ((v[4] + v[5]) + (v[6] + v[7]));
     __syncthreads();
@@ -420,7 +428,34 @@
 __global__ __launch_bounds__(256) void ln_bwd_final_multi_kernel(const LnFinishTable t) {
     const LnPending& e = t.s[blockIdx.y];
     if ((int)blockIdx.x * 16 >= 2 * e.cols + 2) return;
-    ln_final_body<T>(e.nblk, e.cols, e.partial, (T*)e.dgamma, (T*)e.dbeta, (const T*)e.alpha_a, (T*)e.out_a, (const T*)e.alpha_b, (T*)e.out_b);
+    ln_final_body<T>(e.nblk, e.cols, e.partial, (T*)e.dgamma, (T*)e.dbeta, (const T*)e.alpha_a, (T*)e.out_a, (const T*)e.alpha_b, (T*)e.out_b, e.stride);
+}
+template <typename T>
+__global__ __launch_bounds__(256) void ln_bwd_colsum_final_kernel(int nsets, int nblk, int cols, const float* __restrict__ partial, long long set_stride, T* out) {
+    __shared__ float red[16][17];
+    const int stride = 3 * cols + 2;
+    const int tx = threadIdx.x & 15, ty = threadIdx.x >> 4;
+    const int idx = blockIdx.x * 16 + tx;
+    float v[8] = {0.f, 0.f, 0.f, 0.f, 0.f, 0.f, 0.f, 0.f};
+    if (idx < cols) {
+        for (int s = 0; s < nsets; s++) {
+            const float* p = partial + s * set_stride + 2 * cols + 2 + idx;
+            int b = ty;
+            for (; b + 7 * 16 < nblk; b += 8 * 16) {
+#pragma unroll
+                for (int u = 0; u < 8; u++) v[u] += p[(long long)(b + 16 * u) * stride];
+            }
+            for (; b < nblk; b += 16) v[0] += p[(long long)b * stride];
+        }
+    }
+    red[ty][tx] = ((v[0] + v[1]) + (v[2] + v[3])) + ((v[4] + v[5]) + (v[6] + v[7]));
+    __syncthreads();
+    if (ty == 0 && idx < cols) {
+        float s = 0.f;
+#pragma unroll
+        for (int u = 0; u < 16; u++) s += red[u][tx];
+        out[idx] = from_f32<T>(s);
+    }
 }
 
 struct ColReduceArgs {
@@ -630,6 +665,18 @@
     return ln_fused_blocks(rows, rpb);
 }
 size_t layernorm_bwd_partial_bytes(int rows, int cols) { return (size_t)layernorm_bwd_partial_blocks(rows) * (2 * (size_t)cols + 2) * sizeof(float); }
+bool layernorm_bwd_colsum_ok(int dtype, int cols) {
+    const int n = dtype == FF_DTYPE_BF16 ? 8 : 4;
+    return layernorm_bwd_deferrable(dtype, cols) && cdiv(cols / n, 64) <= 4 && (size_t)12 * cols * sizeof(float) <= 150 * 1024;
+}
+size_t layernorm_bwd_colsum_partial_bytes(int rows, int cols) { return (size_t)layernorm_bwd_partial_blocks(rows) * (3 * (size_t)cols + 2) * sizeof(float); }
+int layernorm_bwd_colsum_finish(int dtype, int nsets, int rows, int cols, const float* partial, long long set_stride, void* out, hipStream_t st_) {
+    FF_CHECK(nsets > 0 && rows > 0 && cols > 0 && partial && out, FF_ERR_SHAPE, "layernorm_bwd_colsum_finish: bad arguments");
+    const int nblk = layernorm_bwd_partial_blocks(rows);
+    if (dtype == FF_DTYPE_BF16) ln_bwd_colsum_final_kernel<bf16><<<dim3(cdiv(cols, 16)), dim3(256), 0, st_>>>(nsets, nblk, cols, partial, set_stride, (bf16*)out);
+    else ln_bwd_colsum_final_kernel<float><<<dim3(cdiv(cols, 16)), dim3(256), 0, st_>>>(nsets, nblk, cols, partial, set_stride, (float*)out);
+    return check_launch("ln_bwd_colsum_final");
+}
 
 template <typename T, int VEC>
 static int launch_ln_fused(const LnArgs& a, const void* dy, const void* x, const void* add, const void* gamma, const float* mean,
@@ -638,29 +685,35 @@
     int rpb;
     const int nblk = ln_fused_blocks(a.rows, rpb);
     const int nch = cdiv(a.cols / VEC, 64);
-    const size_t lds = (size_t)8 * a.cols * sizeof(float);
-#define FF_LN_LAUNCH(NCH)                                                                                                                 \
+    const size_t lds = (size_t)(a.dx_colsum ? 12 : 8) * a.cols * sizeof(float);
+#define FF_LN_LAUNCH(NCH) FF_LN_LAUNCH_(NCH, false)
+#define FF_LN_LAUNCH_(NCH, DXSUM)                                                                                                         \
     do {                                                                                                                                  \
         if (lds > 48 * 1024) {                                                                                                            \
             static bool attr[64] = {};                                                                                                    \
             int dev = 0;                                                                                                                  \
             (void)hipGetDevice(&dev);                                                                                                     \
             if (dev < 0 || dev >= 64 || !attr[dev]) {                                                                                     \
-                hipFuncSetAttribute((const void*)ln_bwd_fused_kernel<T, VEC, NCH>, hipFuncAttributeMaxDynamicSharedMemorySize, 150 * 1024); \
+                hipFuncSetAttribute((const void*)ln_bwd_fused_kernel<T, VEC, NCH, DXSUM>, hipFuncAttributeMaxDynamicSharedMemorySize, 150 * 1024); \
                 if (dev >= 0 && dev < 64) attr[dev] = true;                                                                               \
             }                                                                                                                             \
         }                                                                                                                                 \
-        ln_bwd_fused_kernel<T, VEC, NCH><<<dim3(nblk), dim3(256), lds, st_>>>(a, (const T*)dy, (const T*)x, (const T*)add, (const T*)gamma, \
+        ln_bwd_fused_kernel<T, VEC, NCH, DXSUM><<<dim3(nblk), dim3(256), lds, st_>>>(a, (const T*)dy, (const T*)x, (const T*)add, (const T*)gamma, \
                                                                               mean, rstd, (T*)dx, (const T*)dx_res, (const T*)dots.a,     \
                                                                               (const T*)dots.b, partial, rpb);                            \
     } while (0)
-    if (nch <= 2) FF_LN_LAUNCH(2);
+    if (a.dx_colsum) {
+        if (nch <= 2) FF_LN_LAUNCH_(2, true);
+        else FF_LN_LAUNCH_(4, true);
+    } else if (nch <= 2) FF_LN_LAUNCH(2);
     else if (nch <= 4) FF_LN_LAUNCH(4);
     else FF_LN_LAUNCH(8);
 #undef FF_LN_LAUNCH
+#undef FF_LN_LAUNCH_
     FF_TRY(check_launch("ln_bwd_fused"));
     if (pending) {
         pending->partial = partial; pending->nblk = nblk; pending->cols = a.cols; pending->dgamma = dgamma; pending->dbeta = dbeta;
+        pending->stride = a.dx_colsum ? 3 * a.cols + 2 : 0;
         pending->alpha_a = dots.alpha_a; pending->out_a = dots.out_a; pending->alpha_b = dots.alpha_b; pending->out_b = dots.out_b;
         return FF_OK;
     }
@@ -682,10 +735,12 @@
     const bool v = vec_ok(a.dtype, a.cols, {a.x_map, a.y_map, a.dx_map}, {x, add, gamma, dy, dx, dx_residual, dots.a, dots.b});
     FF_CHECK(a.dy_splits == 0 || (ln_fused_ok(a.dtype, a.cols, v) && (dgamma || dots.a || dots.b) && a.cols % 4 == 0), FF_ERR_UNSUPPORTED,
              "layernorm_bwd: summing split-K slabs needs the one-pass kernel");
+    FF_CHECK(!a.dx_colsum || (layernorm_bwd_colsum_ok(a.dtype, a.cols) && v && dgamma && pending && !dx && !dx_residual && !dots.a && !dots.b && !a.dy_splits),
+             FF_ERR_UNSUPPORTED, "layernorm_bwd: column sums of dx come from the one-pass kernel, postponed, without dx / residual / dots / slabs");
     if (ln_fused_ok(a.dtype, a.cols, v) && (dgamma || dots.a || dots.b)) {
         FF_CHECK(!dgamma == !dbeta, FF_ERR_SHAPE, "layernorm_bwd: dgamma and dbeta come together");
         int rpb;
-        const size_t need = (size_t)ln_fused_blocks(a.rows, rpb) * (2 * (size_t)a.cols + 2) * sizeof(float);
+        const size_t need = (size_t)ln_fused_blocks(a.rows, rpb) * ((a.dx_colsum ? 3 : 2) * (size_t)a.cols + 2) * sizeof(float);
         FF_CHECK(ws && ws_bytes >= need, FF_ERR_WORKSPACE, "layernorm_bwd workspace: need %zu have %zu", need, ws_bytes);
         if (a.dtype == FF_DTYPE_BF16) return launch_ln_fused<bf16, 8>(a, dy, x, add, gamma, mean, rstd, dx, dx_residual, dots, dgamma, dbeta, (float*)ws, st_, pending);
         return launch_ln_fused<float, 4>(a, dy, x, add, gamma, mean, rstd, dx, dx_residual, dots, dgamma, dbeta, (float*)ws, st_, pending);
```

Result: no change. 803.4, median of 6 (+0.3%).
